# shiinamiyuki/akari_render

Hardware: AMD Instinct MI355X
Metric: Msamples/s (whole node), 1080p path tracer, C2 (higher is better)
Workload: dtype f32

## Files before the change

akari_render_amd/capi.py:

```python
from __future__ import annotations

import ctypes as C
import os
from typing import Optional

import numpy as np

from . import abi
from .build import LIB, build

AKR_OK = 0
FILM_PLANE_RGB, FILM_PLANE_SPLAT, FILM_PLANE_WEIGHT, FILM_PLANES_PT, FILM_PLANES_ALL = 1, 2, 4, 5, 7
ERR_INVALID_ARGUMENT, ERR_HIP, ERR_NO_DEVICE, ERR_IO, ERR_PARSE, ERR_UNSUPPORTED, ERR_OOM, ERR_RENDER = -1, -2, -3, -4, -5, -6, -7, -8

(ARRAY_WOOP, ARRAY_TRI_GID, ARRAY_SHADE, ARRAY_INSTANCES, ARRAY_MATERIALS, ARRAY_BVH_NODES, ARRAY_LIGHT_ENTRIES,
 ARRAY_LIGHT_PDF, ARRAY_AREA_ENTRIES, ARRAY_AREA_PDF, ARRAY_INST_TRI_OFFSET, ARRAY_R2C, ARRAY_C2W,
 ARRAY_TEX_NODES, ARRAY_TEX_IMAGES, ARRAY_TEX_TEXELS, ARRAY_MAT_INPUTS,
 ARRAY_INST_LEAVES, ARRAY_MESH_TRIS, ARRAY_MESH_POS, ARRAY_MESH_META, ARRAY_MESH_NORMALS,
 ARRAY_ENV_MARGINAL_ENTRIES, ARRAY_ENV_MARGINAL_PDF, ARRAY_ENV_CONDITIONAL_ENTRIES, ARRAY_ENV_CONDITIONAL_PDF, ARRAY_ENV_TEXELS,
 ARRAY_PUNCTUAL_LIGHTS, ARRAY_LIGHT_TREE) = range(29)
ENV_LIGHT_INSTANCE = 0xFFFFFFFF
PUNCTUAL_LIGHT_INSTANCE = 0xFFFFFFFE
LIGHT_TREE_INSTANCE = 0xFFFFFFFD

EXPORTS = [
    "akr_last_error", "akr_version", "akr_struct_size", "akr_option_set", "akr_option_get", "akr_context_create",
    "akr_context_destroy", "akr_context_synchronize", "akr_context_device_info", "akr_scene_create", "akr_scene_load",
    "akr_scene_destroy", "akr_scene_set_resolution", "akr_scene_get_info", "akr_scene_get_light", "akr_scene_get_ggx_table",
    "akr_scene_get_desc_counts", "akr_scene_get_mesh", "akr_scene_get_instance", "akr_scene_get_material", "akr_scene_get_camera",
    "akr_scene_get_array", "akr_scene_get_image_count", "akr_scene_get_image", "akr_scene_get_material_graph", "akr_film_create",
    "akr_film_wrap", "akr_film_destroy", "akr_film_clear", "akr_film_read", "akr_film_write", "akr_film_resolve",
    "akr_film_device_ptr", "akr_pt_config_default", "akr_pt_config_from_json", "akr_pt_render", "akr_pt_begin", "akr_pt_passes",
    "akr_pt_begin_features", "akr_pt_render_features",
    "akr_pt_end", "akr_pt_get_stats", "akr_render_task", "akr_image_write", "akr_aov_config_default", "akr_aov_render",
    "akr_gpt_config_default", "akr_gpt_render", "akr_gpt_begin", "akr_gpt_sample", "akr_gpt_sums", "akr_gpt_sums_read",
    "akr_gpt_sums_write", "akr_gpt_finish", "akr_gpt_abort", "akr_gpt_reduce", "akr_mcmc_config_default", "akr_mcmc_render",
    "akr_film_set_splat_scale", "akr_film_get_splat_scale", "akr_pt_read_sampler_states", "akr_context_device_ordinal",
    "akr_device_count", "akr_comm_unique_id", "akr_comm_create", "akr_comm_wrap", "akr_comm_destroy", "akr_film_reduce",
    "akr_pt_kernel_info", "akr_scene_spec_source", "akr_host_spec_compile", "akr_host_spec_compile_text",
    "akr_film_reduce_planes", "akr_mcmc_render_shard", "akr_mcmc_combine_host", "akr_mcmc_combine",
    "akr_scene_set_environment", "akr_scene_get_environment", "akr_scene_set_lens", "akr_scene_get_lens",
    "akr_denoise_config_default", "akr_denoise", "akr_denoise_variance",
    "akr_pt_set_active_tiles", "akr_film_tile_error", "akr_adaptive_config_default", "akr_pt_adaptive_render",
    "akr_display_config_default", "akr_film_luminance_histogram", "akr_display_exposure", "akr_display_transform",
    "akr_scene_add_punctual_light", "akr_scene_clear_punctual_lights", "akr_scene_punctual_light_count", "akr_scene_get_punctual_light",
    "akr_scene_set_light_tree", "akr_scene_get_light_tree",
]
TEST_EXPORTS = [
    "akr_probe_material_inputs_host", "akr_host_stdrng_u64", "akr_host_chacha_block", "akr_host_pcg32_states",
    "akr_host_pcg_start", "akr_host_alias_table", "akr_probe_math", "akr_probe_bsdf", "akr_probe_intersect",
    "akr_probe_surface_interaction", "akr_probe_material_inputs", "akr_host_decode_png", "akr_host_decode_jpeg",
    "akr_host_decode_exr", "akr_host_decode_tiff", "akr_host_decode_dds", "akr_host_pmj02bn_tables",
    "akr_probe_material_folded_host", "akr_host_sobol_dim1", "akr_host_fastmod", "akr_host_tri_pretest",
    "akr_probe_env_sample", "akr_probe_env_pdf", "akr_host_lens_ray", "akr_probe_camera_rays",
    "akr_probe_div", "akr_probe_intersect_pair", "akr_probe_math2", "akr_host_denoise", "akr_probe_denoise_times",
    "akr_host_pt_launch_plan", "akr_host_denoise_variance", "akr_probe_denoise_variance_times",
    "akr_host_tile_error", "akr_host_half_bracket", "akr_probe_adapt_times",
    "akr_host_display_transform", "akr_host_luminance_histogram", "akr_probe_display_times",
    "akr_host_pt_features_plan", "akr_host_pcg_end_pass", "akr_probe_pcg_end_pass",
    "akr_host_light_sample", "akr_probe_light_sample", "akr_host_light_sample_soft", "akr_probe_light_sample_soft",
    "akr_host_light_tree_sample", "akr_probe_light_tree_sample", "akr_host_option_info",
    "akr_probe_pt_cost_order", "akr_probe_pt_cost_order_mode",
]


class OptionInfo(C.Structure):
    _fields_ = [("name", C.c_char_p), ("env", C.c_char_p), ("default_value", C.c_int32), ("ranged", C.c_int32), ("lo", C.c_int32), ("hi", C.c_int32)]


class RenderSession(C.Structure):

    _fields_ = [("save_intermediate", C.c_int32), ("save_stats", C.c_int32), ("name", C.c_char_p),
                ("override_sampler_independent", C.c_int32), ("verbose", C.c_int32)]


class AkariError(RuntimeError):
    def __init__(self, code: int, msg: str):
        super().__init__(f"akari_hip error {code}: {msg}")
        self.code = code


_lib: Optional[C.CDLL] = None


def lib() -> C.CDLL:
    global _lib
    if _lib is not None:
        return _lib
    if not os.path.exists(LIB):
        build()
    L = C.CDLL(os.environ.get("AKR_HIP_LIB") or LIB)
    vp, u32, u64, i32, f32 = C.c_void_p, C.c_uint32, C.c_uint64, C.c_int32, C.c_float
    fp, up, u64p, vpp = C.POINTER(C.c_float), C.POINTER(C.c_uint32), C.POINTER(C.c_uint64), C.POINTER(C.c_void_p)
    L.akr_last_error.restype = C.c_char_p
    L.akr_version.restype = C.c_char_p
    L.akr_struct_size.restype = C.c_uint32
    L.akr_struct_size.argtypes = [C.c_int32]
    for sid, cls in enumerate((abi.MeshDesc, abi.InstanceDesc, abi.MaterialDesc, abi.CameraDesc, abi.SceneDesc, abi.PtConfig, abi.PtStats, abi.SceneInfo,
                               abi.KernelInfo, abi.AovConfig, abi.GptConfig, abi.McmcConfig, abi.McmcResult, abi.McmcPartial,
                               abi.EnvironmentDesc, abi.LensDesc, abi.DenoiseConfig), start=1):
        if L.akr_struct_size(sid) != C.sizeof(cls):
            raise ImportError("libakari_hip.so and akari_render_amd/abi.py disagree on sizeof(%s): %d vs %d" % (cls.__name__, L.akr_struct_size(sid), C.sizeof(cls)))
    for sid, cls in ((19, abi.AdaptiveConfig), (20, abi.AdaptiveStats), (22, abi.DisplayConfig), (24, abi.PunctualLightDesc)):
        if L.akr_struct_size(sid) != C.sizeof(cls):
            raise ImportError("libakari_hip.so and akari_render_amd/abi.py disagree on sizeof(%s): %d vs %d" % (cls.__name__, L.akr_struct_size(sid), C.sizeof(cls)))

    def proto(name, *args):
        if name in TEST_EXPORTS and not hasattr(L, name):
            return
        fn = getattr(L, name)
        fn.restype = i32
        fn.argtypes = list(args)

    proto("akr_context_create", i32, vpp)
    proto("akr_context_destroy", vp)
    proto("akr_context_synchronize", vp)
    proto("akr_context_device_info", vp, C.c_char_p, u32, up, u64p)
    proto("akr_scene_create", vp, C.POINTER(abi.SceneDesc), vpp)
    proto("akr_scene_load", vp, C.c_char_p, u32, u32, vpp)
    proto("akr_scene_destroy", vp)
    proto("akr_scene_set_resolution", vp, u32, u32)
    proto("akr_scene_get_info", vp, C.POINTER(abi.SceneInfo))
    proto("akr_scene_get_light", vp, u32, up, fp, fp)
    proto("akr_scene_set_environment", vp, C.POINTER(abi.EnvironmentDesc))
    proto("akr_scene_get_environment", vp, C.POINTER(abi.EnvironmentDesc))
    proto("akr_scene_set_lens", vp, C.POINTER(abi.LensDesc))
    proto("akr_scene_get_lens", vp, C.POINTER(abi.LensDesc))
    proto("akr_scene_add_punctual_light", vp, C.POINTER(abi.PunctualLightDesc))
    proto("akr_scene_clear_punctual_lights", vp)
    proto("akr_scene_punctual_light_count", vp, up)
    proto("akr_scene_get_punctual_light", vp, u32, C.POINTER(abi.PunctualLightDesc))
    proto("akr_host_light_sample", vp, u32, fp, fp, up)
    proto("akr_probe_light_sample", vp, vp, u32, fp, fp, up)
    proto("akr_host_light_sample_soft", vp, u32, fp, fp, up)
    proto("akr_probe_light_sample_soft", vp, vp, u32, fp, fp, up)
    proto("akr_scene_set_light_tree", vp, u32)
    proto("akr_scene_get_light_tree", vp, up, up)
    proto("akr_host_light_tree_sample", vp, u32, fp, fp, up, up)
    proto("akr_probe_light_tree_sample", vp, vp, u32, fp, fp, up, up)
    proto("akr_host_lens_ray", vp, u32, f32, u32, up, fp, fp)
    proto("akr_probe_camera_rays", vp, vp, u32, f32, u32, up, fp, fp)
    proto("akr_host_pt_launch_plan", vp, C.POINTER(abi.PtConfig), i32, i32, i32, i32, C.POINTER(abi.PtLaunchPlan))
    proto("akr_host_pt_features_plan", vp, C.POINTER(abi.PtConfig), i32, i32, i32, i32, i32, i32, i32, C.POINTER(abi.PtFeaturesPlan))
    proto("akr_probe_env_sample", vp, vp, u32, fp, fp)
    proto("akr_probe_env_pdf", vp, vp, u32, fp, fp)
    proto("akr_scene_get_ggx_table", vp, fp)
    proto("akr_scene_get_desc_counts", vp, up, up, up)
    proto("akr_scene_get_mesh", vp, u32, C.POINTER(abi.MeshDesc))
    proto("akr_scene_get_instance", vp, u32, C.POINTER(abi.InstanceDesc))
    proto("akr_scene_get_material", vp, u32, C.POINTER(abi.MaterialDesc))
    proto("akr_scene_get_camera", vp, C.POINTER(abi.CameraDesc))
    proto("akr_scene_get_array", vp, i32, vpp, u64p)
    proto("akr_scene_get_image_count", vp, up)
    proto("akr_scene_get_image", vp, u32, C.POINTER(abi.ImageDesc))
    proto("akr_scene_get_material_graph", vp, u32, C.POINTER(abi.MaterialGraph))
    proto("akr_film_create", vp, u32, u32, vpp)
    proto("akr_film_wrap", vp, u32, u32, vp, vpp)
    proto("akr_film_destroy", vp)
    proto("akr_film_clear", vp)
    proto("akr_film_read", vp, fp)
    proto("akr_film_write", vp, fp)
    proto("akr_film_resolve", vp, fp)
    proto("akr_film_device_ptr", vp, vpp, u64p)
    proto("akr_pt_kernel_info", vp, C.POINTER(abi.KernelInfo))
    proto("akr_scene_spec_source", vp, C.c_char_p, u64, u64p)
    proto("akr_host_spec_compile", vp, u32, u32, C.c_char_p, u64p, C.c_char_p, u32)
    proto("akr_probe_material_folded_host", vp, u32, u32, fp, up, fp, fp)
    proto("akr_host_sobol_dim1", u32, up, up, up)
    proto("akr_host_fastmod", u32, up, up, up)
    proto("akr_host_tri_pretest", u32, fp, fp, f32, up, up, fp)
    proto("akr_host_spec_compile_text", C.c_char_p, u32, u32, C.c_char_p, C.c_char_p)
    proto("akr_context_device_ordinal", vp, C.POINTER(C.c_int32))
    proto("akr_device_count", C.POINTER(C.c_int32))
    proto("akr_option_set", C.c_char_p, i32)
    proto("akr_option_get", C.c_char_p, C.POINTER(C.c_int32))
    proto("akr_host_option_info", u32, C.POINTER(OptionInfo))
    proto("akr_probe_pt_cost_order", vp, up, up, up, u32, up, fp)
    proto("akr_probe_pt_cost_order_mode", i32, C.POINTER(C.c_int32))
    proto("akr_comm_unique_id", C.POINTER(C.c_uint8))
    proto("akr_comm_create", vp, C.POINTER(C.c_uint8), i32, i32, vpp)
    proto("akr_comm_wrap", vp, vp, i32, i32, vpp)
    proto("akr_comm_destroy", vp)
    proto("akr_film_reduce", vp, vp, i32, i32)
    proto("akr_film_reduce_planes", vp, vp, i32, i32, u32)
    proto("akr_mcmc_render_shard", vp, vp, C.POINTER(abi.McmcConfig), u32, u32, vp, C.POINTER(abi.McmcPartial), up, C.POINTER(abi.PtStats))
    proto("akr_mcmc_combine_host", vp, C.POINTER(abi.McmcPartial), u32, C.POINTER(abi.McmcResult))
    proto("akr_mcmc_combine", vp, vp, i32, C.POINTER(abi.McmcPartial), C.POINTER(abi.McmcResult))
    proto("akr_pt_config_default", C.POINTER(abi.PtConfig))
    proto("akr_aov_config_default", C.POINTER(abi.AovConfig))
    proto("akr_aov_render", vp, vp, C.POINTER(abi.AovConfig), vp, C.POINTER(abi.PtStats))
    proto("akr_gpt_config_default", C.POINTER(abi.GptConfig))
    proto("akr_gpt_render", vp, vp, C.POINTER(abi.GptConfig), vp, fp, C.POINTER(abi.PtStats))
    proto("akr_gpt_begin", vp, vp, C.POINTER(abi.GptConfig), vp, vp, vpp)
    proto("akr_gpt_sample", vp, u32, i32)
    proto("akr_gpt_sums", vp, C.POINTER(fp), u64p)
    proto("akr_gpt_sums_read", vp, fp)
    proto("akr_gpt_sums_write", vp, fp)
    proto("akr_gpt_finish", vp, fp, C.POINTER(abi.PtStats))
    proto("akr_gpt_abort", vp, C.POINTER(abi.PtStats))
    proto("akr_gpt_reduce", vp, vp, i32, i32)
    proto("akr_mcmc_config_default", C.POINTER(abi.McmcConfig))
    proto("akr_mcmc_render", vp, vp, C.POINTER(abi.McmcConfig), vp, C.POINTER(abi.McmcResult), up, C.POINTER(abi.PtStats))
    proto("akr_film_set_splat_scale", vp, C.c_float)
    proto("akr_film_get_splat_scale", vp, fp)
    proto("akr_pt_config_from_json", C.c_char_p, C.POINTER(abi.PtConfig), C.c_char_p, u32)
    proto("akr_pt_render", vp, vp, C.POINTER(abi.PtConfig), vp, C.POINTER(abi.PtStats))
    proto("akr_pt_begin", vp, vp, C.POINTER(abi.PtConfig), vp, vpp)
    proto("akr_pt_passes", vp, u32, i32, up)
    proto("akr_pt_begin_features", vp, vp, C.POINTER(abi.PtConfig), vp, vp, vp, vpp)
    proto("akr_pt_render_features", vp, vp, C.POINTER(abi.PtConfig), vp, vp, vp, C.POINTER(abi.PtStats))
    proto("akr_pt_end", vp, C.POINTER(abi.PtStats))
    proto("akr_pt_get_stats", vp, C.POINTER(abi.PtStats))
    proto("akr_render_task", vp, vp, C.c_char_p, C.POINTER(RenderSession), C.POINTER(abi.PtStats))
    proto("akr_image_write", C.c_char_p, fp, u32, u32)
    proto("akr_pt_read_sampler_states", vp, u64p)
    proto("akr_host_stdrng_u64", u64, u32, u64p)
    proto("akr_host_chacha_block", up, u64, u64, i32, up)
    proto("akr_host_pcg32_states", u64, u64, u64p)
    proto("akr_host_pcg_start", u64p, u64)
    proto("akr_host_pcg_end_pass", u64p, u64, u32)
    proto("akr_probe_pcg_end_pass", vp, u32, u64p, u64p, up, u64p, u64p)
    proto("akr_host_alias_table", fp, u32, up, fp, fp)
    proto("akr_probe_math", vp, u32, fp, fp, fp, fp)
    proto("akr_probe_math2", vp, u32, fp, fp)
    proto("akr_probe_bsdf", vp, C.POINTER(abi.MaterialDesc), fp, i32, fp, u32, fp, fp)
    proto("akr_probe_intersect", vp, vp, u32, fp, up, fp)
    proto("akr_probe_div", vp, u32, fp, fp, fp, fp)
    proto("akr_probe_intersect_pair", vp, vp, u32, fp, up, up, fp)
    proto("akr_probe_surface_interaction", vp, vp, u32, up, fp, fp)
    proto("akr_probe_material_inputs", vp, vp, u32, u32, fp, fp)
    proto("akr_probe_material_inputs_host", vp, u32, u32, u32, fp, fp)
    proto("akr_host_decode_png", C.c_char_p, u64, up, up, C.POINTER(C.c_uint8), u64)
    proto("akr_host_decode_jpeg", C.c_char_p, u64, up, up, C.POINTER(C.c_uint8), u64)
    proto("akr_host_decode_exr", C.c_char_p, u64, up, up, fp, u64)
    proto("akr_host_decode_tiff", C.c_char_p, u64, up, up, C.POINTER(C.c_uint8), u64)
    proto("akr_host_decode_dds", C.c_char_p, u64, up, up, C.POINTER(C.c_uint8), u64)
    proto("akr_host_pmj02bn_tables", up, C.POINTER(C.c_uint16))
    proto("akr_denoise_config_default", C.POINTER(abi.DenoiseConfig))
    proto("akr_denoise", vp, C.POINTER(abi.DenoiseConfig), vp, vp, vp, vp)
    proto("akr_host_denoise", C.POINTER(abi.DenoiseConfig), u32, u32, fp, f32, fp, f32, fp, f32, fp)
    proto("akr_probe_denoise_times", vp, C.POINTER(abi.DenoiseConfig), vp, vp, vp, vp, i32, fp)
    proto("akr_denoise_variance", vp, C.POINTER(abi.DenoiseConfig), vp, vp, vp, vp, vp)
    proto("akr_host_denoise_variance", C.POINTER(abi.DenoiseConfig), u32, u32, fp, f32, fp, fp, f32, fp, f32, fp)
    proto("akr_probe_denoise_variance_times", vp, C.POINTER(abi.DenoiseConfig), vp, vp, vp, vp, vp, i32, fp)
    proto("akr_pt_set_active_tiles", vp, up, u32)
    proto("akr_film_tile_error", vp, vp, vp, u32, u32, up, u32, fp)
    proto("akr_adaptive_config_default", C.POINTER(abi.AdaptiveConfig))
    proto("akr_display_config_default", C.POINTER(abi.DisplayConfig))
    proto("akr_film_luminance_histogram", vp, vp, up, up)
    proto("akr_display_exposure", C.POINTER(abi.DisplayConfig), up, fp)
    proto("akr_display_transform", vp, C.POINTER(abi.DisplayConfig), vp, vp, fp)
    proto("akr_host_display_transform", C.POINTER(abi.DisplayConfig), u32, u32, fp, f32, fp, fp)
    proto("akr_host_luminance_histogram", u32, u32, fp, f32, up, up)
    proto("akr_probe_display_times", vp, C.POINTER(abi.DisplayConfig), vp, vp, i32, fp)
    proto("akr_pt_adaptive_render", vp, vp, C.POINTER(abi.PtConfig), C.POINTER(abi.AdaptiveConfig), vp, vp, up, C.POINTER(abi.AdaptiveStats))
    proto("akr_host_tile_error", u32, u32, fp, fp, u32, u32, up, u32, fp)
    proto("akr_host_half_bracket", u32, u32, fp, fp, u32, u32, up, u32, i32)
    proto("akr_probe_adapt_times", vp, vp, vp, u32, u32, up, u32, fp)
    _lib = L
    return L


def check(rc: int) -> None:
    if rc != AKR_OK:
        raise AkariError(rc, lib().akr_last_error().decode("utf-8", "replace"))


def _fp(a: np.ndarray):
    return a.ctypes.data_as(C.POINTER(C.c_float))


def _up(a: np.ndarray):
    return a.ctypes.data_as(C.POINTER(C.c_uint32))


class Context:

    def __init__(self, device: int = 0):
        self.h = C.c_void_p()
        check(lib().akr_context_create(device, C.byref(self.h)))

    def close(self):
        if self.h:
            lib().akr_context_destroy(self.h)
            self.h = C.c_void_p()

    def __del__(self):
        try:
            self.close()
        except Exception:
            pass

    def synchronize(self):
        check(lib().akr_context_synchronize(self.h))

    def device_info(self):
        name = C.create_string_buffer(256)
        cus, mem = C.c_uint32(), C.c_uint64()
        check(lib().akr_context_device_info(self.h, name, 256, C.byref(cus), C.byref(mem)))
        return {"name": name.value.decode(), "compute_units": cus.value, "hbm_bytes": mem.value}


class Scene:

    def __init__(self, ctx: Optional[Context], source, width: int = 0, height: int = 0):
        self.ctx = ctx
        self.h = C.c_void_p()
        ch = ctx.h if ctx is not None else C.c_void_p()
        if isinstance(source, (str, os.PathLike)):
            check(lib().akr_scene_load(ch, os.fspath(source).encode(), width, height, C.byref(self.h)))
        else:
            desc, keep = source.to_desc()
            if width and height:
                desc.camera.width, desc.camera.height = width, height
            check(lib().akr_scene_create(ch, C.byref(desc), C.byref(self.h)))
            del keep
            env = getattr(source, "environment", None)
            if env is not None:
                self._set_environment_data(env)
            lens = getattr(source, "lens", None)
            if lens is not None:
                self.set_lens(lens.radius, lens.focal_distance)
            for light in getattr(source, "lights", None) or ():
                self.add_punctual_light(light)

    def close(self):
        if self.h:
            lib().akr_scene_destroy(self.h)
            self.h = C.c_void_p()

    def __del__(self):
        try:
            self.close()
        except Exception:
            pass

    def info(self) -> abi.SceneInfo:
        i = abi.SceneInfo()
        check(lib().akr_scene_get_info(self.h, C.byref(i)))
        return i

    def spec_source(self) -> str:
        n = C.c_uint64()
        check(lib().akr_scene_spec_source(self.h, None, 0, C.byref(n)))
        buf = C.create_string_buffer(n.value + 1)
        check(lib().akr_scene_spec_source(self.h, buf, n.value + 1, C.byref(n)))
        return buf.value.decode()

    def spec_compile(self, bvh: bool = False, pmj: bool = False, stage: bool = True, defer: bool = False, min_waves: int = 3, arch: str = "gfx950", inst: bool = False,
                     env: bool = False, lens: bool = False) -> int:
        nbytes = C.c_uint64()
        log = C.create_string_buffer(4096)
        flags = (1 if bvh else 0) | (2 if pmj else 0) | (4 if stage else 0) | (8 if defer else 0) | (16 if inst else 0) | (32 if env else 0) | (64 if lens else 0)
        check(lib().akr_host_spec_compile(self.h, flags, min_waves, arch.encode(), C.byref(nbytes), log, 4096))
        return nbytes.value

    def launch_plan(self, cfg: abi.PtConfig, defer_metal: int = -1, simple_kernels: int = 1, defer_on: int = 0, spec_waves: int = 0) -> dict:
        out = abi.PtLaunchPlan()
        check(lib().akr_host_pt_launch_plan(self.h, C.byref(cfg), defer_metal, simple_kernels, defer_on, spec_waves, C.byref(out)))
        return out.as_dict()

    def features_plan(self, cfg: abi.PtConfig, feat: bool = True, defer_metal: int = -1, simple_kernels: int = 1, defer_on: int = 0, spec_waves: int = 0,
                      wavefront: int = -1, arith: int = 0) -> dict:
        out = abi.PtFeaturesPlan()
        check(lib().akr_host_pt_features_plan(self.h, C.byref(cfg), defer_metal, simple_kernels, defer_on, spec_waves, 1 if feat else 0, wavefront, arith, C.byref(out)))
        return out.as_dict()

    def material_folded_host(self, material: int, uv: np.ndarray):
        uv = np.ascontiguousarray(uv, dtype=np.float32).reshape(-1, 2)
        n = uv.shape[0]
        out, alpha, em = np.zeros((n, 64), np.uint32), np.zeros(n, np.float32), np.zeros((n, 3), np.float32)
        check(lib().akr_probe_material_folded_host(self.h, material, n, _fp(uv), out.ctypes.data_as(C.POINTER(C.c_uint32)), _fp(alpha), _fp(em)))
        return out, alpha, em

    def _set_environment_data(self, env: Optional[abi.EnvironmentData]):
        if env is None:
            check(lib().akr_scene_set_environment(self.h, None))
            return
        d, keep = env.to_desc()
        check(lib().akr_scene_set_environment(self.h, C.byref(d)))
        del keep

    def set_environment(self, image=None, color=None, strength: float = 1.0, rotation=None, filter: int = abi.TEX_FILTER_LINEAR):
        if image is None and color is None:
            self._set_environment_data(None)
        else:
            self._set_environment_data(abi.EnvironmentData(image=image, color=color, strength=strength, rotation=rotation, filter=filter))

    def environment(self) -> Optional[abi.EnvironmentData]:
        d = abi.EnvironmentDesc()
        check(lib().akr_scene_get_environment(self.h, C.byref(d)))
        if d.strength == 0.0:
            return None
        rot = np.array(list(d.rotation), dtype=np.float32).reshape(3, 3)
        if d.width:
            n = d.width * d.height * 4
            im = np.ctypeslib.as_array(d.texels, shape=(n,)).astype(np.float32, copy=True).reshape(d.height, d.width, 4)
            return abi.EnvironmentData(image=im, strength=float(d.strength), rotation=rot, filter=int(d.filter))
        return abi.EnvironmentData(color=tuple(float(c) for c in d.color), strength=float(d.strength), rotation=rot)

    def add_punctual_light(self, light: Optional[abi.PunctualLightData] = None, **fields):
        if light is None:
            light = abi.PunctualLightData(**fields)
        d = light.to_desc()
        check(lib().akr_scene_add_punctual_light(self.h, C.byref(d)))

    def clear_punctual_lights(self):
        check(lib().akr_scene_clear_punctual_lights(self.h))

    def punctual_lights(self) -> list:
        n = C.c_uint32()
        check(lib().akr_scene_punctual_light_count(self.h, C.byref(n)))
        out = []
        for i in range(n.value):
            d = abi.PunctualLightDesc()
            check(lib().akr_scene_get_punctual_light(self.h, i, C.byref(d)))
            out.append(abi.PunctualLightData.from_desc(d))
        return out

    def _light_sample(self, fn, head, rows, cols=7):
        rows = np.ascontiguousarray(rows, dtype=np.float32).reshape(-1, cols)
        n = rows.shape[0]
        out, light = np.zeros((n, 13), np.float32), np.zeros(n, np.uint32)
        check(fn(*head, n, _fp(rows), _fp(out), _up(light)))
        return out, light

    def host_light_sample(self, rows):
        return self._light_sample(lib().akr_host_light_sample, (self.h,), rows)

    def probe_light_sample(self, rows):
        return self._light_sample(lib().akr_probe_light_sample, (self.ctx.h, self.h), rows)

    def host_light_sample_soft(self, rows):
        return self._light_sample(lib().akr_host_light_sample_soft, (self.h,), rows, 9)

    def probe_light_sample_soft(self, rows):
        return self._light_sample(lib().akr_probe_light_sample_soft, (self.ctx.h, self.h), rows, 9)

    def set_light_tree(self, on):
        check(lib().akr_scene_set_light_tree(self.h, 1 if on else 0))

    def light_tree(self):
        on, n = C.c_uint32(), C.c_uint32()
        check(lib().akr_scene_get_light_tree(self.h, C.byref(on), C.byref(n)))
        return on.value, n.value

    def _light_tree_sample(self, fn, head, rows):
        rows = np.ascontiguousarray(rows, dtype=np.float32).reshape(-1, 9)
        n = rows.shape[0]
        out, light, record = np.zeros((n, 13), np.float32), np.zeros(n, np.uint32), np.zeros(n, np.uint32)
        check(fn(*head, n, _fp(rows), _fp(out), _up(light), _up(record)))
        return out, light, record

    def host_light_tree_sample(self, rows):
        return self._light_tree_sample(lib().akr_host_light_tree_sample, (self.h,), rows)

    def probe_light_tree_sample(self, rows):
        return self._light_tree_sample(lib().akr_probe_light_tree_sample, (self.ctx.h, self.h), rows)

    def set_lens(self, radius: Optional[float] = None, focal_distance: float = 0.0):
        if radius is None:
            check(lib().akr_scene_set_lens(self.h, None))
            return
        d = abi.LensDesc(float(radius), float(focal_distance))
        check(lib().akr_scene_set_lens(self.h, C.byref(d)))

    def lens(self) -> Optional[abi.LensData]:
        d = abi.LensDesc()
        check(lib().akr_scene_get_lens(self.h, C.byref(d)))
        return abi.LensData(float(d.radius), float(d.focal_distance)) if d.radius > 0.0 else None

    def _camera_rays(self, fn, head, pixels, u_filter, u_lens, filter_type, filter_radius):
        px = np.ascontiguousarray(pixels, dtype=np.uint32).reshape(-1, 2)
        n = px.shape[0]
        u = np.ascontiguousarray(np.concatenate([np.asarray(u_filter, np.float32).reshape(n, 2), np.asarray(u_lens, np.float32).reshape(n, 2)], axis=1))
        out = np.zeros((n, 6), np.float32)
        check(fn(*head, int(filter_type), float(filter_radius), n, px.ctypes.data_as(C.POINTER(C.c_uint32)), _fp(u), _fp(out)))
        return out

    def host_lens_ray(self, pixels, u_filter, u_lens, filter_type: int = 0, filter_radius: float = 0.5) -> np.ndarray:
        return self._camera_rays(lib().akr_host_lens_ray, (self.h,), pixels, u_filter, u_lens, filter_type, filter_radius)

    def probe_camera_rays(self, pixels, u_filter, u_lens, filter_type: int = 0, filter_radius: float = 0.5) -> np.ndarray:
        return self._camera_rays(lib().akr_probe_camera_rays, (self.ctx.h, self.h), pixels, u_filter, u_lens, filter_type, filter_radius)

    def probe_env_sample(self, u: np.ndarray) -> np.ndarray:
        u = np.ascontiguousarray(u, dtype=np.float32).reshape(-1, 2)
        out = np.zeros((u.shape[0], 5), np.float32)
        check(lib().akr_probe_env_sample(self.ctx.h, self.h, u.shape[0], _fp(u), _fp(out)))
        return out

    def probe_env_pdf(self, d: np.ndarray) -> np.ndarray:
        d = np.ascontiguousarray(d, dtype=np.float32).reshape(-1, 3)
        out = np.zeros((d.shape[0], 4), np.float32)
        check(lib().akr_probe_env_pdf(self.ctx.h, self.h, d.shape[0], _fp(d), _fp(out)))
        return out

    def set_resolution(self, w: int, h: int):
        check(lib().akr_scene_set_resolution(self.h, w, h))

    def light(self, i: int):
        inst, power, pdf = C.c_uint32(), C.c_float(), C.c_float()
        check(lib().akr_scene_get_light(self.h, i, C.byref(inst), C.byref(power), C.byref(pdf)))
        return inst.value, power.value, pdf.value

    def ggx_table(self) -> np.ndarray:
        t = np.zeros(4096, dtype=np.float32)
        check(lib().akr_scene_get_ggx_table(self.h, _fp(t)))
# ... 284 lines not shown
        except Exception:
            pass


def pt_render(ctx: Context, scene: Scene, cfg: abi.PtConfig, film: Film) -> dict:
    st = abi.PtStats()
    c = cfg.copy()
    check(lib().akr_pt_render(ctx.h, scene.h, C.byref(c), film.h, C.byref(st)))
    return st.as_dict()


def pt_render_features(ctx: Context, scene: Scene, cfg: abi.PtConfig, film: Film, albedo: Film, normal: Film) -> dict:
    st = abi.PtStats()
    c = cfg.copy()
    check(lib().akr_pt_render_features(ctx.h if ctx is not None else None, scene.h, C.byref(c), film.h if film is not None else None,
                                       albedo.h if albedo is not None else None, normal.h if normal is not None else None, C.byref(st)))
    return st.as_dict()


def render_task(ctx: Context, scene: Scene, method_json: str, name: Optional[str] = None, save_intermediate: bool = False,
                save_stats: bool = False, override_sampler_independent: bool = False, verbose: bool = False) -> dict:
    ses = RenderSession(1 if save_intermediate else 0, 1 if save_stats else 0, name.encode() if name else None,
                        1 if override_sampler_independent else 0, 1 if verbose else 0)
    st = abi.PtStats()
    check(lib().akr_render_task(ctx.h, scene.h, method_json.encode(), C.byref(ses), C.byref(st)))
    return st.as_dict()


def image_write(path: str, rgb: np.ndarray) -> None:
    rgb = np.ascontiguousarray(rgb, dtype=np.float32)
    h, w = rgb.shape[0], rgb.shape[1]
    check(lib().akr_image_write(os.fspath(path).encode(), _fp(rgb), w, h))


def config_from_json(text: str):
    cfg = abi.PtConfig()
    out = C.create_string_buffer(1024)
    check(lib().akr_pt_config_from_json(text.encode(), C.byref(cfg), out, 1024))
    return cfg, out.value.decode()


def host_stdrng_u64(seed: int, n: int) -> np.ndarray:
    out = np.zeros(n, dtype=np.uint64)
    check(lib().akr_host_stdrng_u64(seed, n, out.ctypes.data_as(C.POINTER(C.c_uint64))))
    return out


def host_chacha_block(key, counter: int, stream: int, rounds: int) -> np.ndarray:
    key = np.ascontiguousarray(key, dtype=np.uint32)
    out = np.zeros(16, dtype=np.uint32)
    check(lib().akr_host_chacha_block(_up(key), counter, stream, rounds, _up(out)))
    return out


def host_pcg32_states(seed: int, n: int) -> np.ndarray:
    out = np.zeros(2 * n, dtype=np.uint64)
    check(lib().akr_host_pcg32_states(seed, n, out.ctypes.data_as(C.POINTER(C.c_uint64))))
    return out


def host_pcg_start(state: int, inc: int) -> int:
    s = C.c_uint64(state)
    check(lib().akr_host_pcg_start(C.byref(s), inc))
    return s.value


def host_pcg_end_pass(state: int, inc: int, dim: int) -> int:
    s = C.c_uint64(state)
    check(lib().akr_host_pcg_end_pass(C.byref(s), inc, dim))
    return s.value


def host_tri_pretest(rays8: np.ndarray, tris9: np.ndarray, plane_shift: float = 0.0):
    rays8 = np.ascontiguousarray(rays8, dtype=np.float32).reshape(-1, 8)
    tris9 = np.ascontiguousarray(tris9, dtype=np.float32).reshape(-1, 9)
    n = rays8.shape[0]
    may, exact, t = np.zeros(n, dtype=np.uint32), np.zeros(n, dtype=np.uint32), np.zeros(n, dtype=np.float32)
    check(lib().akr_host_tri_pretest(n, _fp(rays8), _fp(tris9), C.c_float(plane_shift), _up(may), _up(exact), _fp(t)))
    return may.astype(bool), exact.astype(bool), t


def host_alias_table(weights):
    w = np.ascontiguousarray(weights, dtype=np.float32)
    j = np.zeros(w.size, dtype=np.uint32)
    t = np.zeros(w.size, dtype=np.float32)
    pdf = np.zeros(w.size, dtype=np.float32)
    check(lib().akr_host_alias_table(_fp(w), w.size, _up(j), _fp(t), _fp(pdf)))
    return j, t, pdf


def probe_math(ctx: Context, x: np.ndarray):
    x = np.ascontiguousarray(x, dtype=np.float32)
    s, c, l = (np.zeros_like(x) for _ in range(3))
    check(lib().akr_probe_math(ctx.h, x.size, _fp(x), _fp(s), _fp(c), _fp(l)))
    return s, c, l


def probe_math2(ctx: Context, x: np.ndarray, y: np.ndarray) -> np.ndarray:
    xy = np.ascontiguousarray(np.stack([np.asarray(x, dtype=np.float32), np.asarray(y, dtype=np.float32)], axis=1))
    out = np.zeros((xy.shape[0], 6), dtype=np.float32)
    check(lib().akr_probe_math2(ctx.h, xy.shape[0], _fp(xy), _fp(out)))
    return out


def probe_div(ctx: Context, a: np.ndarray, b: np.ndarray):
    a = np.ascontiguousarray(a, dtype=np.float32)
    b = np.ascontiguousarray(b, dtype=np.float32)
    assert a.shape == b.shape
    fast, ieee = np.zeros_like(a), np.zeros_like(a)
    check(lib().akr_probe_div(ctx.h, a.size, _fp(a), _fp(b), _fp(fast), _fp(ieee)))
    return fast, ieee


def probe_pcg_end_pass(ctx: Context, state: np.ndarray, inc: np.ndarray, dim: np.ndarray):
    state = np.ascontiguousarray(state, dtype=np.uint64)
    inc = np.ascontiguousarray(inc, dtype=np.uint64)
    dim = np.ascontiguousarray(dim, dtype=np.uint32)
    assert state.shape == inc.shape == dim.shape
    closed, loop = np.zeros_like(state), np.zeros_like(state)
    u64p = C.POINTER(C.c_uint64)
    check(lib().akr_probe_pcg_end_pass(ctx.h, state.size, state.ctypes.data_as(u64p), inc.ctypes.data_as(u64p), _up(dim),
                                       closed.ctypes.data_as(u64p), loop.ctypes.data_as(u64p)))
    return closed, loop


def probe_bsdf(ctx: Context, m: abi.MaterialData, mode: int, wo, data: np.ndarray, table: Optional[np.ndarray] = None) -> np.ndarray:
    ms = m.to_struct()
    wo = np.ascontiguousarray(wo, dtype=np.float32)
    data = np.ascontiguousarray(data, dtype=np.float32).reshape(-1, 3)
    out = np.zeros((data.shape[0], 4 if mode == 0 else 8), dtype=np.float32)
    tp = _fp(np.ascontiguousarray(table, dtype=np.float32)) if table is not None else C.POINTER(C.c_float)()
    check(lib().akr_probe_bsdf(ctx.h, C.byref(ms), tp, mode, _fp(wo), data.shape[0], _fp(data), _fp(out)))
    return out


def probe_intersect(ctx: Context, scene: Scene, rays: np.ndarray):
    rays = np.ascontiguousarray(rays, dtype=np.float32).reshape(-1, 8)
    out = np.zeros((rays.shape[0], 3), dtype=np.uint32)
    bary = np.zeros((rays.shape[0], 2), dtype=np.float32)
    check(lib().akr_probe_intersect(ctx.h, scene.h, rays.shape[0], _fp(rays), _up(out), _fp(bary)))
    return out, bary


def probe_intersect_pair(ctx: Context, scene: Scene, rays: np.ndarray, excl: np.ndarray):
    rays = np.ascontiguousarray(rays, dtype=np.float32).reshape(-1, 16)
    excl = np.ascontiguousarray(excl, dtype=np.uint32).reshape(-1, 3)
    assert rays.shape[0] == excl.shape[0]
    out = np.zeros((rays.shape[0], 4), dtype=np.uint32)
    tuv = np.zeros((rays.shape[0], 3), dtype=np.float32)
    check(lib().akr_probe_intersect_pair(ctx.h, scene.h, rays.shape[0], _fp(rays), _up(excl), _up(out), _fp(tuv)))
    return out, tuv


def probe_surface_interaction(ctx: Context, scene: Scene, inst_prim: np.ndarray, bary: np.ndarray) -> np.ndarray:
    ip = np.ascontiguousarray(inst_prim, dtype=np.uint32).reshape(-1, 2)
    b = np.ascontiguousarray(bary, dtype=np.float32).reshape(-1, 2)
    out = np.zeros((ip.shape[0], 19), dtype=np.float32)
    check(lib().akr_probe_surface_interaction(ctx.h, scene.h, ip.shape[0], _up(ip), _fp(b), _fp(out)))
    return out


def probe_material_inputs(ctx: Optional[Context], scene: Scene, material: int, uv: np.ndarray) -> np.ndarray:
    u = np.ascontiguousarray(uv, dtype=np.float32).reshape(-1, 2)
    out = np.zeros((u.shape[0], 26), dtype=np.float32)
    check(lib().akr_probe_material_inputs(ctx.h if ctx is not None else C.c_void_p(), scene.h, material, u.shape[0], _fp(u), _fp(out)))
    return out


def probe_material_inputs_host(scene: Scene, material: int, uv: np.ndarray, color: int = 0) -> np.ndarray:
    u = np.ascontiguousarray(uv, dtype=np.float32).reshape(-1, 2)
    out = np.zeros((u.shape[0], 26), dtype=np.float32)
    check(lib().akr_probe_material_inputs_host(scene.h, material, color, u.shape[0], _fp(u), _fp(out)))
    return out


def _host_decode(fn, data: bytes) -> np.ndarray:
    w, h = C.c_uint32(), C.c_uint32()
    check(fn(data, len(data), C.byref(w), C.byref(h), None, 0))
    out = np.zeros((h.value, w.value, 4), dtype=np.uint8)
    check(fn(data, len(data), C.byref(w), C.byref(h), out.ctypes.data_as(C.POINTER(C.c_uint8)), out.size))
    return out


def host_decode_png(data: bytes) -> np.ndarray:
    return _host_decode(lib().akr_host_decode_png, data)


def host_decode_jpeg(data: bytes) -> np.ndarray:
    return _host_decode(lib().akr_host_decode_jpeg, data)


def host_decode_tiff(data: bytes) -> np.ndarray:
    return _host_decode(lib().akr_host_decode_tiff, data)


def host_decode_dds(data: bytes) -> np.ndarray:
    return _host_decode(lib().akr_host_decode_dds, data)


def aov_render(ctx: Context, scene: Scene, cfg: abi.AovConfig, film: Film) -> dict:
    st = abi.PtStats()
    check(lib().akr_aov_render(ctx.h, scene.h, C.byref(cfg), film.h, C.byref(st)))
    return st.as_dict()


def denoise(ctx: Context, color: Film, albedo: Optional[Film], normal: Optional[Film], out: Film, cfg: Optional[abi.DenoiseConfig] = None) -> None:
    c = cfg if cfg is not None else abi.DenoiseConfig.default()
    check(lib().akr_denoise(ctx.h, C.byref(c), color.h, albedo.h if albedo is not None else None, normal.h if normal is not None else None, out.h))


def denoise_times(ctx: Context, color: Film, albedo: Optional[Film], normal: Optional[Film], out: Film, kernel: int, cfg: Optional[abi.DenoiseConfig] = None) -> dict:
    c = cfg if cfg is not None else abi.DenoiseConfig.default()
    t = np.zeros(11, dtype=np.float32)
    check(lib().akr_probe_denoise_times(ctx.h, C.byref(c), color.h, albedo.h if albedo is not None else None, normal.h if normal is not None else None, out.h, kernel, _fp(t)))
    return {"prepare": float(t[0]), "levels": [float(v) for v in t[1:1 + c.iterations]], "finish": float(t[9]), "total": float(t[10])}


def host_denoise(width: int, height: int, color: np.ndarray, albedo: Optional[np.ndarray] = None, normal: Optional[np.ndarray] = None,
                 cfg: Optional[abi.DenoiseConfig] = None, splat_scales=(1.0, 1.0, 1.0)) -> np.ndarray:
    c = cfg if cfg is not None else abi.DenoiseConfig.default()
    films = []
    for f in (color, albedo, normal):
        if f is not None:
            f = np.ascontiguousarray(f, dtype=np.float32).reshape(-1)
            assert f.size == 7 * width * height
        films.append(f)
    out = np.zeros(3 * width * height, dtype=np.float32)
    ptr = [_fp(f) if f is not None else None for f in films]
    check(lib().akr_host_denoise(C.byref(c), width, height, ptr[0], splat_scales[0], ptr[1], splat_scales[1], ptr[2], splat_scales[2], _fp(out)))
    return out.reshape(height, width, 3)


def denoise_variance(ctx: Context, color: Film, half: Film, albedo: Optional[Film], normal: Optional[Film], out: Film, cfg: Optional[abi.DenoiseConfig] = None) -> None:
    c = cfg if cfg is not None else abi.DenoiseConfig.default()
    check(lib().akr_denoise_variance(ctx.h, C.byref(c), color.h, half.h if half is not None else None, albedo.h if albedo is not None else None,
                                     normal.h if normal is not None else None, out.h))


def denoise_variance_times(ctx: Context, color: Film, half: Film, albedo: Optional[Film], normal: Optional[Film], out: Film, kernel: int,
                           cfg: Optional[abi.DenoiseConfig] = None) -> dict:
    c = cfg if cfg is not None else abi.DenoiseConfig.default()
    t = np.zeros(11, dtype=np.float32)
    check(lib().akr_probe_denoise_variance_times(ctx.h, C.byref(c), color.h, half.h, albedo.h if albedo is not None else None,
                                                 normal.h if normal is not None else None, out.h, kernel, _fp(t)))
    return {"prepare": float(t[0]), "levels": [float(v) for v in t[1:1 + c.iterations]], "finish": float(t[9]), "total": float(t[10])}


def host_denoise_variance(width: int, height: int, color: np.ndarray, half: np.ndarray, albedo: Optional[np.ndarray] = None, normal: Optional[np.ndarray] = None,
                          cfg: Optional[abi.DenoiseConfig] = None, splat_scales=(1.0, 1.0, 1.0)) -> np.ndarray:
    c = cfg if cfg is not None else abi.DenoiseConfig.default()
    films = []
    for f in (color, half, albedo, normal):
        if f is not None:
            f = np.ascontiguousarray(f, dtype=np.float32).reshape(-1)
            assert f.size == 7 * width * height
        films.append(f)
    out = np.zeros(3 * width * height, dtype=np.float32)
    ptr = [_fp(f) if f is not None else None for f in films]
    check(lib().akr_host_denoise_variance(C.byref(c), width, height, ptr[0], splat_scales[0], ptr[1], ptr[2], splat_scales[1], ptr[3], splat_scales[2], _fp(out)))
    return out.reshape(height, width, 3)


def film_tile_error(ctx: Context, film: Film, half: Film, tile_w: int, tile_h: int, tiles) -> np.ndarray:
    t = np.ascontiguousarray(tiles, dtype=np.uint32).reshape(-1)
    err = np.zeros(t.size, dtype=np.float32)
    check(lib().akr_film_tile_error(ctx.h, film.h, half.h if half is not None else None, tile_w, tile_h, _up(t), t.size, _fp(err)))
    return err


def host_tile_error(width: int, height: int, film: np.ndarray, half: np.ndarray, tile_w: int, tile_h: int, tiles) -> np.ndarray:
    film, half = np.ascontiguousarray(film, dtype=np.float32), np.ascontiguousarray(half, dtype=np.float32)
    assert film.size == half.size == 7 * width * height
    t = np.ascontiguousarray(tiles, dtype=np.uint32).reshape(-1)
    err = np.zeros(t.size, dtype=np.float32)
    check(lib().akr_host_tile_error(width, height, _fp(film), _fp(half), tile_w, tile_h, _up(t), t.size, _fp(err)))
    return err


def host_half_bracket(width: int, height: int, film: np.ndarray, half: np.ndarray, tile_w: int, tile_h: int, tiles, close: bool) -> np.ndarray:
    film = np.ascontiguousarray(film, dtype=np.float32)
    out = np.array(half, dtype=np.float32, copy=True)
    assert film.size == out.size == 7 * width * height
    t = np.ascontiguousarray(tiles, dtype=np.uint32).reshape(-1)
    check(lib().akr_host_half_bracket(width, height, _fp(film), _fp(out), tile_w, tile_h, _up(t), t.size, 1 if close else 0))
    return out


def adapt_times(ctx: Context, film: Film, half: Film, tile_w: int, tile_h: int, tiles) -> dict:
    t = np.ascontiguousarray(tiles, dtype=np.uint32).reshape(-1)
    ms = np.zeros(3, dtype=np.float32)
    check(lib().akr_probe_adapt_times(ctx.h, film.h, half.h, tile_w, tile_h, _up(t), t.size, _fp(ms)))
    return {"tile_error": float(ms[0]), "half_open": float(ms[1]), "half_close": float(ms[2])}


def pt_adaptive_render(ctx: Context, scene: Scene, cfg: abi.PtConfig, film: Film, acfg: Optional[abi.AdaptiveConfig] = None, half: Optional[Film] = None,
                       want_tile_spp: bool = True):
    c, a = cfg.copy(), (acfg if acfg is not None else abi.AdaptiveConfig.default())
    tw, th = c.tile_w or 32, c.tile_h or 32
    tiles_x, tiles_y = (film.width + tw - 1) // tw, (film.height + th - 1) // th
    tile_spp = np.zeros(tiles_x * tiles_y, dtype=np.uint32) if want_tile_spp else None
    st = abi.AdaptiveStats()
    check(lib().akr_pt_adaptive_render(ctx.h, scene.h, C.byref(c), C.byref(a), film.h, half.h if half is not None else None,
                                       _up(tile_spp) if tile_spp is not None else None, C.byref(st)))
    return st.as_dict(), (tile_spp.reshape(tiles_y, tiles_x) if tile_spp is not None else None)


# ... 148 lines not shown
```

akari_render_amd/csrc/device/disect.h:

```cpp
#pragma once
#include "drng.h"
#include "dscene.h"
#include "../kernels.h"

namespace akr {

template <bool V>
struct BoolTag {
    static constexpr bool value = V;
};

struct Hit {
    float t, u, v;
    uint32_t gid;
};

struct PlaneHit {
    float t, px, py, pz;
};
AKR_HD PlaneHit tri_plane(vec3 o, vec3 d, float4 r2) {
    float dz = __builtin_fmaf(r2.x, d.x, __builtin_fmaf(r2.y, d.y, r2.z * d.z));
    float oz = __builtin_fmaf(r2.x, o.x, __builtin_fmaf(r2.y, o.y, __builtin_fmaf(r2.z, o.z, r2.w)));
    PlaneHit h;
    h.t = div_f(-oz, dz);
    h.px = __builtin_fmaf(h.t, d.x, o.x);
    h.py = __builtin_fmaf(h.t, d.y, o.y);
    h.pz = __builtin_fmaf(h.t, d.z, o.z);
    return h;
}
AKR_HD void tri_uv(const PlaneHit& h, float4 r0, float4 r1, float& u, float& v) {
    u = __builtin_fmaf(r0.x, h.px, __builtin_fmaf(r0.y, h.py, __builtin_fmaf(r0.z, h.pz, r0.w)));
    v = __builtin_fmaf(r1.x, h.px, __builtin_fmaf(r1.y, h.py, __builtin_fmaf(r1.z, h.pz, r1.w)));
}
AKR_HD bool tri_test(vec3 o, vec3 d, float4 r0, float4 r1, float4 r2, float tmin, float tmax, float& t_out, float& u_out,
                     float& v_out) {
    PlaneHit h = tri_plane(o, d, r2);
    float u, v;
    tri_uv(h, r0, r1, u, v);
    t_out = h.t;
    u_out = u;
    v_out = v;
    return (h.t >= tmin) & (h.t <= tmax) & (u >= 0.0f) & (v >= 0.0f) & (u + v <= 1.0f);
}

AKR_D float textured_alpha(const DScene& sc, const float4* r, uint32_t material, float u, float v) {
    float w = 1.0f - u - v;
    vec2 uv = mk2((r[0].w * w + r[2].w * u) + r[4].w * v, (r[1].w * w + r[3].w * u) + r[5].w * v);
    return material_alpha_at(sc.tex, sc.materials[material], material, uv);
}
template <bool TEX>
AKR_D bool alpha_test(const DScene& sc, uint32_t gid, float u, float v) {
    const float4* r = sc.shade + (size_t)gid * SHADE_ROWS;
    float4 q6 = r[6];
    const DMaterial& m = sc.materials[f2u(q6.y)];
    float alpha = (m.kind == MAT_PRINCIPLED || m.kind == MAT_DIFFUSE) ? m.base_alpha : 1.0f;
    if (TEX) {
        if (m.flags & MF_ALPHA_TEXTURED)
            alpha = textured_alpha(sc, r, f2u(q6.y), u, v);
    }
    if (alpha >= 1.0f) return true;
    uint32_t inst = f2u(q6.z);
    uint32_t prim = gid - sc.inst_tri_offset[inst];
    float h = (float)xxhash32_4(inst, prim, f2u(u), f2u(v)) * 2.3283064365386963e-10f;
    return alpha > h;
}

AKR_D float next_up(float x) {
    uint32_t b = f2u(x);
    return x > 0.0f ? u2f(b + 1u) : (x < 0.0f ? u2f(b - 1u) : u2f(1u));
}
AKR_D float hit_margin(float t, float u, float v, float tmax) {
    return __builtin_fminf(__builtin_fminf(__builtin_fminf(u, v), 1.0f - (u + v)), __builtin_fminf(t, tmax - t));
}

template <bool ANY_HIT, bool TEX = false>
AKR_D bool trace_exhaustive(const DScene& sc, vec3 o, vec3 d, float tmin, float tmax, uint32_t ex0, uint32_t ex1, Hit& hit) {
    float best_t = next_up(tmax);
    uint32_t best = kInvalid;
    float best_u = 0.0f, best_v = 0.0f;
    const uint32_t n = sc.n_tris;
    typedef const float __attribute__((address_space(4))) * ConstF;
    ConstF recs = (ConstF)(uintptr_t)sc.woop;
    auto load_rec = [&](uint32_t k, float4& a, float4& b, float4& c) {
        ConstF r = recs + 12 * (size_t)k;
        a = make_float4(r[0], r[1], r[2], r[3]);
        b = make_float4(r[4], r[5], r[6], r[7]);
        c = make_float4(r[8], r[9], r[10], r[11]);
    };
    float4 n0, n1, n2;
    load_rec(0, n0, n1, n2);
    PlaneHit ph{0.0f, 0.0f, 0.0f, 0.0f};
    for (uint32_t k = 0; k < n; k++) {
        const float4 r0 = n0, r1 = n1, r2 = n2;
        load_rec(k + 1, n0, n1, n2);
        if (!((sc.plane_share_mask >> k) & 1ull)) ph = tri_plane(o, d, r2);
        float u, v;
        const float t = ph.t;
        tri_uv(ph, r0, r1, u, v);
        float m = __builtin_fminf(hit_margin(t, u, v, tmax), t - tmin);
        m = (k == ex0) ? -1.0f : m;
        m = (k == ex1) ? -1.0f : m;
        if (sc.has_alpha) {
            if (m >= 0.0f && !alpha_test<TEX>(sc, k, u, v)) m = -1.0f;
        }
        if (ANY_HIT) {
            if (m >= 0.0f) best = k;
            if (__builtin_amdgcn_ballot_w64(best == kInvalid) == 0) break;
        } else {
            const float tc = (m >= 0.0f) ? t : __builtin_inff();
            const bool better = tc < best_t;
            best_t = better ? tc : best_t;
            best_u = better ? u : best_u;
            best_v = better ? v : best_v;
            best = better ? k : best;
        }
    }
    hit.t = best != kInvalid ? best_t : tmax;
    hit.u = best_u;
    hit.v = best_v;
    hit.gid = best;
    return best != kInvalid;
}

typedef float v2f __attribute__((ext_vector_type(2)));
typedef float v4f __attribute__((ext_vector_type(4)));
AKR_D float min_raw(float a, float b) {
    float r;
    asm("v_min_f32 %0, %1, %2" : "=v"(r) : "v"(a), "v"(b));
    return r;
}
AKR_D float max_raw(float a, float b) {
    float r;
    asm("v_max_f32 %0, %1, %2" : "=v"(r) : "v"(a), "v"(b));
    return r;
}
AKR_D float min_abs_raw(float a, float b) {
    float r;
    asm("v_min_f32 %0, %1, |%2|" : "=v"(r) : "v"(a), "v"(b));
    return r;
}
AKR_D float max3_abs_raw(float a, float b, float c) {
    float r;
    asm("v_max3_f32 %0, |%1|, |%2|, |%3|" : "=v"(r) : "v"(a), "v"(b), "v"(c));
    return r;
}
AKR_D PlaneHit tri_plane_unscaled(vec3 o, vec3 d, float4 r2, float& lo) {
    float dz = __builtin_fmaf(r2.x, d.x, __builtin_fmaf(r2.y, d.y, r2.z * d.z));
    float oz = __builtin_fmaf(r2.x, o.x, __builtin_fmaf(r2.y, o.y, __builtin_fmaf(r2.z, o.z, r2.w)));
    lo = min_abs_raw(lo, oz);
    PlaneHit h;
    h.t = div_f_unscaled(-oz, dz);
    h.px = __builtin_fmaf(h.t, d.x, o.x);
    h.py = __builtin_fmaf(h.t, d.y, o.y);
    h.pz = __builtin_fmaf(h.t, d.z, o.z);
    return h;
}

template <bool DIV>
struct WalkOpt {
    static constexpr bool unscaled_div = DIV;
};
template <int V>
struct IntTag {
    static constexpr int value = V;
};

template <bool TEX = false, class OPT = WalkOpt<true>>
AKR_D void trace_pair_exhaustive(const DScene& sc, vec3 o, vec3 d, float tmax, uint32_t ex0, vec3 so, vec3 sd, float stmax,
                                 uint32_t sex0, uint32_t sex1, Hit& hit, bool& found, bool& occluded, const float4* lds_recs, uint32_t* took_ieee_walk = nullptr) {
    constexpr bool UNSCALED = OPT::unscaled_div && !AKR_RX;
    float best_t = next_up(tmax);
    uint32_t best = kInvalid;
    float best_u = 0.0f, best_v = 0.0f;
    float occ_margin = -1.0f;
    const uint32_t n = sc.n_tris;
    const v4f* lrec = (const v4f*)lds_recs;
    const bool has_alpha = __builtin_amdgcn_readfirstlane((int)sc.has_alpha) != 0;
    v2f T2 = {0.0f, 0.0f}, hx2 = {0.0f, 0.0f}, hy2 = {0.0f, 0.0f}, hz2 = {0.0f, 0.0f};
    float lo = __builtin_inff(), slo = __builtin_inff();
    auto record = [&](auto alpha_tag, auto div_tag, uint32_t k, const v4f& q0, const v4f& q1, const v4f& q2) {
        constexpr int ALPHA = decltype(alpha_tag)::value;
        constexpr bool FAST = decltype(div_tag)::value;
        if (!((sc.plane_share_mask >> k) & 1ull)) {
            const float4 r2 = make_float4(q2.x, q2.y, q2.z, q2.w);
            const PlaneHit a = FAST ? tri_plane_unscaled(o, d, r2, lo) : tri_plane(o, d, r2), b = FAST ? tri_plane_unscaled(so, sd, r2, slo) : tri_plane(so, sd, r2);
            T2 = (v2f){a.t, b.t};
            hx2 = (v2f){a.px, b.px}; hy2 = (v2f){a.py, b.py}; hz2 = (v2f){a.pz, b.pz};
        }
        float u, v, su, sv;
        tri_uv(PlaneHit{T2.x, hx2.x, hy2.x, hz2.x}, make_float4(q0.x, q0.y, q0.z, q0.w), make_float4(q1.x, q1.y, q1.z, q1.w), u, v);
        tri_uv(PlaneHit{T2.y, hx2.y, hy2.y, hz2.y}, make_float4(q0.x, q0.y, q0.z, q0.w), make_float4(q1.x, q1.y, q1.z, q1.w), su, sv);
        const v2f u2 = {u, su}, v2 = {v, sv};
        const v2f s2 = {1.0f - (u2.x + v2.x), 1.0f - (u2.y + v2.y)};
        const v2f w2 = {tmax - T2.x, stmax - T2.y};
        float m = min_raw(min_raw(min_raw(u2.x, v2.x), s2.x), min_raw(T2.x, w2.x));
        float sm = min_raw(min_raw(min_raw(u2.y, v2.y), s2.y), min_raw(T2.y, w2.y));
        m = (k == ex0) ? -1.0f : m;
        sm = (k == sex0) ? -1.0f : sm;
        sm = (k == sex1) ? -1.0f : sm;
        if (ALPHA == 1 || (ALPHA == 2 && has_alpha)) {
            const uint32_t ka = __builtin_amdgcn_readfirstlane(k);
            if (m >= 0.0f && !alpha_test<TEX>(sc, ka, u2.x, v2.x)) m = -1.0f;
            if (sm >= 0.0f && !alpha_test<TEX>(sc, ka, u2.y, v2.y)) sm = -1.0f;
        }
        const float tc = (m >= 0.0f) ? T2.x : __builtin_inff();
        const bool better = tc < best_t;
        best_t = better ? tc : best_t;
        best = better ? k : best;
        occ_margin = max_raw(occ_margin, sm);
    };
    auto walk = [&](auto alpha_tag) {
        const BoolTag<UNSCALED> div_tag{};
        v4f a0 = lrec[0], a1 = lrec[1], a2 = lrec[2], b0, b1, b2;
        uint32_t k = 0;
        for (; k + 1 < n; k += 2) {
            b0 = lrec[3 * (k + 1)]; b1 = lrec[3 * (k + 1) + 1]; b2 = lrec[3 * (k + 1) + 2];
            record(alpha_tag, div_tag, k, a0, a1, a2);
            a0 = lrec[3 * (k + 2)]; a1 = lrec[3 * (k + 2) + 1]; a2 = lrec[3 * (k + 2) + 2];
            record(alpha_tag, div_tag, k + 1, b0, b1, b2);
        }
        if (k < n) record(alpha_tag, div_tag, k, a0, a1, a2);
    };
    auto walk_ieee = [&] {
        best_t = next_up(tmax); best = kInvalid; occ_margin = -1.0f;
#pragma clang loop unroll(disable)
        for (uint32_t k = 0; k < n; k++) {
            record(IntTag<2>{}, BoolTag<false>{}, k, lrec[3 * k], lrec[3 * k + 1], lrec[3 * k + 2]);
        }
    };
    if (UNSCALED) {
        const float ob = lds_recs[3u * (n + 1u) + 2u].w;
        const bool pre_bad = ((tmax >= 0.0f) & !((max3_abs_raw(o.x, o.y, o.z) <= ob) & (max3_abs_raw(d.x, d.y, d.z) <= 2.0f) & (tmax <= 1e20f))) |
                             ((stmax >= 0.0f) & !((max3_abs_raw(so.x, so.y, so.z) <= ob) & (max3_abs_raw(sd.x, sd.y, sd.z) <= 2.0f) & (stmax <= 1e20f)));
        bool redo = __builtin_amdgcn_ballot_w64(pre_bad) != 0;
        if (!redo) {
            if (has_alpha) walk(IntTag<1>{});
            else walk(IntTag<0>{});
            const bool bad = ((tmax >= 0.0f) & (lo < 0x1p-47f)) | ((stmax >= 0.0f) & (slo < 0x1p-47f));
            redo = __builtin_amdgcn_ballot_w64(bad) != 0;
        }
        if (redo) walk_ieee();
        if (took_ieee_walk) *took_ieee_walk = redo ? 1u : 0u;
    } else {
        if (has_alpha) walk(IntTag<1>{});
        else walk(IntTag<0>{});
        if (took_ieee_walk) *took_ieee_walk = 0u;
    }
    if (best != kInvalid) {
        const v4f q0 = lrec[3 * best], q1 = lrec[3 * best + 1];
        const float px = __builtin_fmaf(best_t, d.x, o.x), py = __builtin_fmaf(best_t, d.y, o.y), pz = __builtin_fmaf(best_t, d.z, o.z);
        best_u = __builtin_fmaf(q0.x, px, __builtin_fmaf(q0.y, py, __builtin_fmaf(q0.z, pz, q0.w)));
        best_v = __builtin_fmaf(q1.x, px, __builtin_fmaf(q1.y, py, __builtin_fmaf(q1.z, pz, q1.w)));
    }
    found = best != kInvalid;
    hit.t = found ? best_t : tmax;
    hit.u = best_u;
    hit.v = best_v;
    hit.gid = best;
    occluded = occ_margin >= 0.0f;
}

constexpr uint32_t kBvhDone = 0xfffffffeu;

struct TraceCounters {
    uint32_t nodes, tris, overflow;
};

AKR_D float safe_inv(float d) {
    float a = abs_f(d) < 1e-20f ? __builtin_copysignf(1e-20f, d) : d;
    return __builtin_amdgcn_rcpf(a);
}
AKR_D uint32_t byte_of(uint32_t w, int i) { return (w >> (8 * i)) & 0xffu; }

struct Trav {
    vec3 o, d, inv, noi;
    float tmin, tmax, best_t, best_u, best_v;
    uint32_t ex0, ex1, best;
    uint32_t G, T, tbase, sp, octinv4;
    bool active;
};
AKR_D void trav_begin(Trav& s, vec3 o, vec3 d, float tmin, float tmax, uint32_t ex0, uint32_t ex1) {
    s.o = o; s.d = d;
    s.inv = mk3(safe_inv(d.x), safe_inv(d.y), safe_inv(d.z));
    s.noi = mk3(-o.x * s.inv.x, -o.y * s.inv.y, -o.z * s.inv.z);
    s.tmin = tmin; s.tmax = tmax;
    s.best_t = tmax; s.best_u = 0.0f; s.best_v = 0.0f; s.best = kInvalid;
    s.ex0 = ex0; s.ex1 = ex1;
    const uint32_t oi = (s.inv.x >= 0.0f ? 1u : 0u) | (s.inv.y >= 0.0f ? 2u : 0u) | (s.inv.z >= 0.0f ? 4u : 0u);
    s.octinv4 = oi * 0x01010101u;
    s.G = 1u << (24u + oi);
    s.T = 0; s.tbase = 0; s.sp = 0;
    s.active = tmax >= tmin;
}

AKR_D uint32_t node_pop(Trav& s, uint32_t* __restrict__ stack, uint32_t depth, TraceCounters& cnt) {
    const uint32_t j = 31u - (uint32_t)__builtin_clz(s.G);
    s.G &= ~(1u << j);
    if ((s.G >> 24) != 0) {
        if (s.sp < depth) {
            stack[s.sp * 256u] = s.G;
            s.sp++;
        } else {
            cnt.overflow = 1;
        }
    }
    const uint32_t slot = (j - 24u) ^ (s.octinv4 & 7u);
    return (s.G & 0xffffffu) + slot;
}
AKR_D void hit_commit(Trav& s, bool any_hit, uint32_t gid, float t, float u, float v) {
    if (any_hit) {
        s.best = gid;
        s.T = 0; s.G = 0; s.sp = 0;
    } else {
        const bool better = (s.best == kInvalid) | (t < s.best_t) | ((t == s.best_t) & (gid < s.best));
        if (better) { s.best_t = t; s.best_u = u; s.best_v = v; s.best = gid; }
    }
}
template <bool TEX>
AKR_D void hit_accept(const DScene& sc, Trav& s, bool any_hit, uint32_t gid, float t, float u, float v) {
    bool h = (gid != s.ex0) & (gid != s.ex1);
    if (h && sc.has_alpha) h = alpha_test<TEX>(sc, gid, u, v);
    if (h) hit_commit(s, any_hit, gid, t, u, v);
}

template <int MODE, bool TEX, bool TILE = false>
AKR_D void trav_step_staged(const DScene& sc, Trav& s, uint32_t* __restrict__ stack, TraceCounters& cnt, bool any_rt = false, const uint4* tile = nullptr) {
    const bool any_hit = MODE == 2 ? any_rt : (MODE == 1);
    if (s.T == 0) {
        if ((s.G >> 24) == 0) {
            s.sp--;
            s.G = stack[s.sp * 256u];
        }
        const uint32_t idx = node_pop(s, stack, sc.bvh_stack_depth, cnt);
        const uint4* p = sc.bvh_nodes + (size_t)idx * (kBvhNodeWords / 4);
        uint4 w0, w1, w2, w3;
        if (TILE && idx < sc.bvh_tile_nodes) {
            typedef const volatile uint32_t __attribute__((address_space(3))) * LdsW;
            typedef uint32_t u32x4 __attribute__((ext_vector_type(4)));
            typedef const volatile u32x4 __attribute__((address_space(3))) * LdsU4;
            LdsU4 pt = (LdsU4)((LdsW)(const uint32_t*)tile + idx * kBvhNodeWords);
            const u32x4 t0 = pt[0], t1 = pt[1], t2 = pt[2], t3 = pt[3];
            w0 = make_uint4(t0.x, t0.y, t0.z, t0.w); w1 = make_uint4(t1.x, t1.y, t1.z, t1.w); w2 = make_uint4(t2.x, t2.y, t2.z, t2.w);
            w3 = make_uint4(t3.x, t3.y, t3.z, t3.w);
        } else {
            w0 = p[0]; w1 = p[1]; w2 = p[2]; w3 = p[3];
        }
        cnt.nodes++;
        const float limit = s.best_t;
        const float bx = u2f((w0.w & 0xffu) << 23) * s.inv.x, by = u2f(((w0.w >> 8) & 0xffu) << 23) * s.inv.y, bz = u2f(((w0.w >> 16) & 0xffu) << 23) * s.inv.z;
        const float ax = __builtin_fmaf(u2f(w0.x), s.inv.x, s.noi.x), ay = __builtin_fmaf(u2f(w0.y), s.inv.y, s.noi.y), az = __builtin_fmaf(u2f(w0.z), s.inv.z, s.noi.z);
        const bool nx = s.inv.x < 0.0f, ny = s.inv.y < 0.0f, nz = s.inv.z < 0.0f;
        const uint32_t xb = nx ? ((w3.y >> 16) | (w3.y << 16)) : w3.y, yb = ny ? ((w3.z >> 16) | (w3.z << 16)) : w3.z, zb = nz ? ((w3.w >> 16) | (w3.w << 16)) : w3.w;
        const uint32_t qnx[2] = {nx ? w2.z : w1.w, xb}, qfx[2] = {nx ? w1.w : w2.z, xb >> 16};
        const uint32_t qny[2] = {ny ? w2.w : w2.x, yb}, qfy[2] = {ny ? w2.x : w2.w, yb >> 16};
        const uint32_t qnz[2] = {nz ? w3.x : w2.y, zb}, qfz[2] = {nz ? w2.y : w3.x, zb >> 16};
        uint32_t hitmask = 0;
#pragma unroll
        for (int h = 0; h < 2; h++) {
            const uint32_t meta4 = h ? (w1.x >> 16) : w1.y;
            const uint32_t is_inner4 = (meta4 & (meta4 << 1)) & 0x10101010u;
            const uint32_t inner_mask4 = (is_inner4 >> 4) * 0xffu;
            const uint32_t bit_index4 = (meta4 ^ (s.octinv4 & inner_mask4)) & 0x1f1f1f1fu;
            const uint32_t child_bits4 = (meta4 >> 5) & 0x07070707u;
#pragma unroll
            for (int i = 0; i < (h ? 2 : 4); i++) {
                const float tnx = __builtin_fmaf((float)byte_of(qnx[h], i), bx, ax), tfx = __builtin_fmaf((float)byte_of(qfx[h], i), bx, ax);
                const float tny = __builtin_fmaf((float)byte_of(qny[h], i), by, ay), tfy = __builtin_fmaf((float)byte_of(qfy[h], i), by, ay);
                const float tnz = __builtin_fmaf((float)byte_of(qnz[h], i), bz, az), tfz = __builtin_fmaf((float)byte_of(qfz[h], i), bz, az);
                const float tn = __builtin_fmaxf(__builtin_fmaxf(tnx, tny), __builtin_fmaxf(tnz, s.tmin));
                const float tf = __builtin_fminf(__builtin_fminf(tfx, tfy), __builtin_fminf(tfz, limit));
                if (tn <= tf) hitmask |= byte_of(child_bits4, i) << byte_of(bit_index4, i);
            }
        }
        s.G = ((w0.w >> 24) | ((w1.x & 0xffffu) << 8)) | (hitmask & 0xff000000u);
        s.T = hitmask & 0x00ffffffu;
        s.tbase = w1.z;
    }
    if (s.T != 0) {
        const uint32_t b = (uint32_t)__builtin_ctz(s.T);
        s.T &= s.T - 1u;
        const uint4* p = (const uint4*)sc.woop + (size_t)(s.tbase + b) * (kBvhTriWords / 4);
        const uint4 w0 = p[0], w1 = p[1], w2 = p[2], w3 = p[3];
        cnt.tris++;
        float t, u, v;
        bool h = tri_test(s.o, s.d, make_float4(u2f(w0.x), u2f(w0.y), u2f(w0.z), u2f(w0.w)), make_float4(u2f(w1.x), u2f(w1.y), u2f(w1.z), u2f(w1.w)),
                          make_float4(u2f(w2.x), u2f(w2.y), u2f(w2.z), u2f(w2.w)), s.tmin, s.tmax, t, u, v);
        if (h) hit_accept<TEX>(sc, s, any_hit, w3.x, t, u, v);
    }
    s.active = (s.T != 0) | ((s.G >> 24) != 0) | (s.sp != 0);
}
template <int MODE, bool TEX, bool TILE = false>
AKR_D void trav_step(const DScene& sc, Trav& s, uint32_t* __restrict__ stack, TraceCounters& cnt, bool any_rt = false, const uint4* tile = nullptr) {
    if constexpr (TEX) {
        trav_step_staged<MODE, TEX, TILE>(sc, s, stack, cnt, any_rt, tile);
        return;
    }
    const bool any_hit = MODE == 2 ? any_rt : (MODE == 1);
    const bool do_tri = s.T != 0;
    const uint4* p;
    bool in_tile = false;
    uint32_t tile_idx = 0;
    if (do_tri) {
        const uint32_t b = (uint32_t)__builtin_ctz(s.T);
        s.T &= s.T - 1u;
        p = (const uint4*)sc.woop + (size_t)(s.tbase + b) * (kBvhTriWords / 4);
    } else {
        if ((s.G >> 24) == 0) {
            s.sp--;
            s.G = stack[s.sp * 256u];
        }
        const uint32_t idx = node_pop(s, stack, sc.bvh_stack_depth, cnt);
        p = sc.bvh_nodes + (size_t)idx * (kBvhNodeWords / 4);
// ... 93 lines not shown
```

akari_render_amd/csrc/device/dscene.h:

```cpp
#pragma once
#include "dtex.h"

namespace akr {

constexpr uint32_t kInvalid = 0xffffffffu;

constexpr uint32_t kBvhNodeWords = 16;
constexpr uint32_t kBvhTriWords = 16;
constexpr uint32_t kBvhStackDepth = 24;
AKR_HD uint32_t walk_bound_word(uint32_t n_tris) { return 12u * (n_tris + 1u) + 11u; }

enum : uint32_t { SHADE_ROWS = 8, INST_ROWS = 8 };
enum : uint32_t { TRI_HAS_NORMALS = 1u, TRI_HAS_TANGENTS = 2u };

struct LightRec {
    uint32_t tri_offset, n_tris, first_gid, inst;
};

constexpr uint32_t kMeshPrimMask = 0x7fffffffu, kMeshTriShares = 0x80000000u;
struct DInst {
    const uint4* __restrict__ tlas_leaves;
    const float4* __restrict__ mesh_tris;
    const uint32_t* __restrict__ mesh_pos;
    const uint32_t* __restrict__ mesh_meta;
    const float4* __restrict__ mesh_normals;
    const uint32_t* __restrict__ inst_mats;
    const uint32_t* __restrict__ share_bits;
    uint32_t on, n_instances;
};

struct DEnv {
    const float4* __restrict__ texels;
    const AliasPacked* __restrict__ marginal;
    const AliasPacked* __restrict__ conditional;
    float rot[9];
    uint32_t w, h, filter, light;
};

enum : uint32_t { PUNCT_POINT = 0, PUNCT_SPOT = 1, PUNCT_SUN = 2 };
constexpr uint32_t kPunctInst = 0xfffffffeu;
constexpr uint32_t kPunctTreeInst = 0xfffffffdu;
struct DPunct {
    vec3 q;       uint32_t kind;
    vec3 a;       float cos_o;
    vec3 c;       float cos_i;
    float inv_span;
    float radius;
    float cos_max;
    float k;
};
static_assert(sizeof(DPunct) == 64, "DPunct layout");
constexpr uint32_t kPunctSoftBit = 0x80000000u;

struct DScene {
    const float4* __restrict__ woop;
    const uint32_t* __restrict__ tri_gid;
    const float4* __restrict__ shade;
    const float4* __restrict__ normals;
    const float4* __restrict__ inst;
    const DMaterial* __restrict__ materials;
    const float* __restrict__ ggx_table;
    const AliasEntry* __restrict__ light_entries;
    const float* __restrict__ light_pdf;
    const uint32_t* __restrict__ light_inst;
    const uint32_t* __restrict__ light_tri_offset;
    const DEnv* __restrict__ env;
    const AliasEntry* __restrict__ area_entries;
    const float* __restrict__ area_pdf;
    const uint32_t* __restrict__ inst_tri_offset;
    const AliasPacked* __restrict__ light_alias;
    const AliasPacked* __restrict__ area_alias;
    const LightRec* __restrict__ lights;
    const uint4* __restrict__ bvh_nodes;
    uint32_t n_tris, n_lights, n_nodes, has_alpha;
    uint32_t bvh_stack_depth;
    uint32_t bvh_tile_nodes;
    uint64_t plane_share_mask;
    TexScene tex;
    DInst in2;
    const DPunct* __restrict__ punct;
    uint32_t n_punct, punct_tree;
};

struct SurfacePoint {
    Frame frame;
    vec3 p, ng;
    float prim_area;
    uint32_t material;
    int32_t light;
    uint32_t inst;
    vec2 uv;
};

AKR_HD vec3 xyz(float4 v) { return mk3(v.x, v.y, v.z); }
AKR_HD vec3 interp3(vec2 b, vec3 a0, vec3 a1, vec3 a2) {
    float w = 1.0f - b.x - b.y;
    return (a0 * w + a1 * b.x) + a2 * b.y;
}
AKR_HD vec3 xf_point(vec3 c0, vec3 c1, vec3 c2, vec3 t, vec3 p) { return ((c0 * p.x + c1 * p.y) + c2 * p.z) + t; }
AKR_HD vec3 xf_vector(vec3 c0, vec3 c1, vec3 c2, vec3 v) { return (c0 * v.x + c1 * v.y) + c2 * v.z; }

AKR_D SurfacePoint surface_interaction_rows(const float4* m, float4 q0, float4 q1, float4 q2, float4 q3, float4 q4, float4 q5, float4 q6, float4 q7, bool has_normals,
                                            const float4* nr, vec2 bary) {
    SurfacePoint s;
    s.prim_area = q6.x;
    s.material = f2u(q6.y);
    s.inst = f2u(q6.z);
    s.light = (int32_t)f2u(q6.w);
    float4 c0 = m[0], c1 = m[1], c2 = m[2], t = m[3];
    vec3 p_local = interp3(bary, xyz(q0), xyz(q1), xyz(q2));
    s.p = xf_point(xyz(c0), xyz(c1), xyz(c2), xyz(t), p_local);
    s.ng = xyz(q3);
    s.frame = Frame{s.ng, xyz(q4), xyz(q5)};
    {
        float w = 1.0f - bary.x - bary.y;
        s.uv = mk2((q0.w * w + q2.w * bary.x) + q4.w * bary.y, (q1.w * w + q3.w * bary.x) + q5.w * bary.y);
    }
    if (has_normals) {
        const uint32_t tf = f2u(q7.w);
        if (tf & (TRI_HAS_NORMALS | TRI_HAS_TANGENTS)) {
            vec3 ns = s.ng;
            if (tf & TRI_HAS_NORMALS) {
                vec3 ns_local = interp3(bary, xyz(nr[0]), xyz(nr[1]), xyz(nr[2]));
                float4 k0 = m[4], k1 = m[5], k2 = m[6];
                vec3 rr = (xyz(k0) * ns_local.x + xyz(k1) * ns_local.y) + xyz(k2) * ns_local.z;
                ns = normalize(rr * k0.w);
            }
            vec3 tt = xyz(q7);
            if (tf & TRI_HAS_TANGENTS) {
                vec3 tt_local = normalize(interp3(bary, xyz(nr[3]), xyz(nr[4]), xyz(nr[5])));
                tt = xf_vector(xyz(c0), xyz(c1), xyz(c2), tt_local);
            }
            s.frame = (tt.x != 0.0f || tt.y != 0.0f || tt.z != 0.0f) ? frame_from_n_t(ns, tt) : frame_from_n(ns);
        }
    }
    return s;
}
AKR_D SurfacePoint surface_interaction(const DScene& sc, uint32_t gid, vec2 bary) {
    const float4* r = sc.shade + (size_t)gid * SHADE_ROWS;
    float4 q0 = r[0], q1 = r[1], q2 = r[2], q3 = r[3], q4 = r[4], q5 = r[5], q6 = r[6];
    const float4* m = sc.inst + (size_t)f2u(q6.z) * INST_ROWS;
    const bool has_normals = sc.normals != nullptr;
    float4 q7 = make_float4(0, 0, 0, 0);
    if (has_normals) q7 = r[7];
    return surface_interaction_rows(m, q0, q1, q2, q3, q4, q5, q6, q7, has_normals, has_normals ? sc.normals + (size_t)gid * 6 : nullptr, bary);
}

}
```

akari_render_amd/csrc/device/pt_pass.h:

```cpp
#pragma once
#include "dpath.h"

namespace akr {

#ifndef AKR_PT_MIN_WAVES
#define AKR_PT_MIN_WAVES 4
#endif
#ifndef AKR_PT_MIN_WAVES_BVH
#define AKR_PT_MIN_WAVES_BVH 4
#endif
#ifndef AKR_PT_MIN_WAVES_FD
#define AKR_PT_MIN_WAVES_FD 4
#endif
#ifndef AKR_PT_MIN_WAVES_TEX
#define AKR_PT_MIN_WAVES_TEX 3
#endif
#ifndef AKR_PT_MIN_WAVES_BVH_TEX
#define AKR_PT_MIN_WAVES_BVH_TEX 3
#endif
template <bool TEX>
using PairWalkOpt = WalkOpt<!TEX>;
template <bool BVH, bool FD, bool TEX, bool PMJ, bool STAGE, bool DEFER, uint32_t ABSENT = 0, bool INST = false, bool ENV = false, bool LENS = false, bool FEAT = false, bool PUNCT = false, bool LTREE = false>
AKR_D void pt_pass_body(const PtParams& p) {
    extern __shared__ __attribute__((aligned(16))) uint32_t lds_stack[];
    TraceCtx tc;
    tc.stack = lds_stack + threadIdx.x;
    tc.cnt = TraceCounters{0, 0, 0};
    PtParams staged = p;
    if (STAGE) stage_scene_tables<BVH, TEX, !BVH && !FD && TEX>(p, lds_stack, staged);
    const PtParams& q = STAGE ? staged : p;
    const DScene& sc = q.sc;
    constexpr bool TILE = BVH && !TEX && !INST;
    constexpr uint32_t STRAG = BVH ? (INST ? AKR_PT_STRAGGLERS_INST : (TEX ? AKR_PT_STRAGGLERS_TEX : AKR_PT_STRAGGLERS)) : 0;
    const uint4* tile = (const uint4*)(lds_stack + p.tile_offset);
    if (TILE) {
        uint32_t* l = lds_stack + p.tile_offset;
        const uint32_t* g = (const uint32_t*)p.sc.bvh_nodes;
        for (uint32_t i = threadIdx.x; i < p.sc.bvh_tile_nodes * kBvhNodeWords; i += 256u) l[i] = g[i];
        __syncthreads();
    }
    const float4* lds_recs = nullptr;
    if (!BVH) {
        uint32_t* l = lds_stack + (p.stage_total >> 2);
        const uint32_t* g = (const uint32_t*)p.sc.woop;
        for (uint32_t i = threadIdx.x; i < (p.sc.n_tris + 2u) * 12u; i += 256u) l[i] = g[i];
        __syncthreads();
        lds_recs = (const float4*)l;
    }
    const uint32_t item = blockIdx.x * 256u + threadIdx.x;
    uint32_t px = 0, py = 0;
    bool in_frame;
    if (p.item_pixels != nullptr) {
        const uint32_t t = p.item_pixels[item];
        in_frame = t != kInvalid;
        if (in_frame) { py = t / p.width; px = t - py * p.width; }
    } else {
        in_frame = item < p.n_items && item_to_pixel(p, item, px, py);
    }
    const uint32_t pix = px + py * p.width;
    uint32_t sx, sy;
    shifted_pixel(p, px, py, sx, sy);
    if (PMJ && p.bn_offset != 0) pmj_bluenoise_stage(p, px, py);
    PathRegs r;
    path_regs_init<PMJ, LENS, FEAT>(r, q, in_frame, pix, sx, sy);
    constexpr bool PARK = !FD && TEX;
    uint32_t* park = lds_stack + p.park_offset + threadIdx.x;
    if (PARK) {
        park_put(park, PK_PIX, pix);
        park_put(park, PK_SX, sx);
        park_put(park, PK_SY, sy);
        if (FEAT) {
            park_put(park, PK_FEAT_A + 0, f2u(r.feat_a.x)); park_put(park, PK_FEAT_A + 1, f2u(r.feat_a.y)); park_put(park, PK_FEAT_A + 2, f2u(r.feat_a.z));
            park_put(park, PK_FEAT_N + 0, f2u(r.feat_n.x)); park_put(park, PK_FEAT_N + 1, f2u(r.feat_n.y)); park_put(park, PK_FEAT_N + 2, f2u(r.feat_n.z));
        }
    }

    uint32_t iteration = 0;
    while (__builtin_amdgcn_ballot_w64(r.active) != 0) {
        iteration++;
        if (r.active) {
            Hit hit;
            bool found = false, occluded = false;
            if (!(STRAG > 0 && r.carry)) {
                r.c_closest += r.has_ray ? 1u : 0u;
                r.c_shadow += r.has_shadow ? 1u : 0u;
            }
            if (BVH && INST) {
                trace_pair_inst<TEX, STRAG>(sc, r.has_ray, r.ro, r.rd, r.ray_ex0, r.has_shadow, r.s_o, r.s_d, r.s_tmax, r.s_ex0, r.s_ex1, r.carry, hit, found, occluded, tc.stack,
                                            lds_stack + p.carry_offset + threadIdx.x, tc.cnt);
            } else if (BVH && STRAG > 0) {
                uint32_t* cy = lds_stack + p.carry_offset + threadIdx.x;
                Trav s;
                uint32_t phase;
                hit.t = 1e20f; hit.u = 0.0f; hit.v = 0.0f; hit.gid = kInvalid;
                if (!r.carry) {
                    phase = r.has_ray ? 0u : (r.has_shadow ? 1u : 2u);
                    if (phase == 0) trav_begin(s, r.ro, r.rd, 0.0f, 1e20f, r.ray_ex0, kInvalid);
                    else trav_begin(s, r.s_o, r.s_d, 0.0f, phase == 1 ? r.s_tmax : -1.0f, r.s_ex0, r.s_ex1);
                } else {
                    phase = cy[CY_PHASE * 256];
                    if (phase == 0) trav_begin(s, r.ro, r.rd, 0.0f, 1e20f, r.ray_ex0, kInvalid);
                    else {
                        trav_begin(s, r.s_o, r.s_d, 0.0f, r.s_tmax, r.s_ex0, r.s_ex1);
                        hit.t = u2f(cy[CY_HIT_T * 256]); hit.u = u2f(cy[CY_HIT_U * 256]); hit.v = u2f(cy[CY_HIT_V * 256]); hit.gid = cy[CY_HIT_GID * 256];
                        found = hit.gid != kInvalid;
                    }
                    s.best_t = u2f(cy[CY_BEST_T * 256]); s.best_u = u2f(cy[CY_BEST_U * 256]); s.best_v = u2f(cy[CY_BEST_V * 256]); s.best = cy[CY_BEST * 256];
                    s.G = cy[CY_G * 256]; s.T = cy[CY_T * 256]; s.tbase = cy[CY_TBASE * 256]; s.sp = cy[CY_SP * 256];
                    s.active = true;
                }
                const uint32_t n_in = (uint32_t)__builtin_popcountll(__builtin_amdgcn_ballot_w64(phase != 2u));
                const uint32_t n_leave = n_in / (STRAG > 0 ? STRAG : 1u);
                while (true) {
                    const uint32_t n_now = (uint32_t)__builtin_popcountll(__builtin_amdgcn_ballot_w64(phase != 2u));
                    if (n_now <= n_leave) break;
                    if (phase != 2u) {
                        if (s.active) trav_step<2, TEX, TILE>(sc, s, tc.stack, tc.cnt, phase == 1u, tile);
                        if (!s.active) {
                            if (phase == 0u) {
                                found = s.best != kInvalid;
                                hit.t = s.best_t; hit.u = s.best_u; hit.v = s.best_v; hit.gid = s.best;
                                phase = r.has_shadow ? 1u : 2u;
                                if (r.has_shadow) trav_begin(s, r.s_o, r.s_d, 0.0f, r.s_tmax, r.s_ex0, r.s_ex1);
                            } else {
                                occluded = s.best != kInvalid;
                                phase = 2u;
                            }
                        }
                    }
                }
                r.carry = phase != 2u;
                if (r.carry) {
                    cy[CY_BEST_T * 256] = f2u(s.best_t); cy[CY_BEST_U * 256] = f2u(s.best_u); cy[CY_BEST_V * 256] = f2u(s.best_v); cy[CY_BEST * 256] = s.best;
                    cy[CY_G * 256] = s.G; cy[CY_T * 256] = s.T; cy[CY_TBASE * 256] = s.tbase; cy[CY_SP * 256] = s.sp;
                    cy[CY_PHASE * 256] = phase;
                    if (phase == 1u) { cy[CY_HIT_T * 256] = f2u(hit.t); cy[CY_HIT_U * 256] = f2u(hit.u); cy[CY_HIT_V * 256] = f2u(hit.v); cy[CY_HIT_GID * 256] = hit.gid; }
                }
            } else if (BVH) {
                Trav s;
                uint32_t phase = r.has_ray ? 0u : (r.has_shadow ? 1u : 2u);
                if (phase == 0) trav_begin(s, r.ro, r.rd, 0.0f, 1e20f, r.ray_ex0, kInvalid);
                else trav_begin(s, r.s_o, r.s_d, 0.0f, phase == 1 ? r.s_tmax : -1.0f, r.s_ex0, r.s_ex1);
                hit.t = 1e20f; hit.u = 0.0f; hit.v = 0.0f; hit.gid = kInvalid;
                while (phase != 2u) {
                    if (s.active) trav_step<2, TEX, TILE>(sc, s, tc.stack, tc.cnt, phase == 1u, tile);
                    if (!s.active) {
                        if (phase == 0u) {
                            found = s.best != kInvalid;
                            hit.t = s.best_t; hit.u = s.best_u; hit.v = s.best_v; hit.gid = s.best;
                            phase = r.has_shadow ? 1u : 2u;
                            if (r.has_shadow) trav_begin(s, r.s_o, r.s_d, 0.0f, r.s_tmax, r.s_ex0, r.s_ex1);
                        } else {
                            occluded = s.best != kInvalid;
                            phase = 2u;
                        }
                    }
                }
            } else {
                trace_pair_exhaustive<TEX, PairWalkOpt<TEX>>(sc, r.ro, r.rd, r.has_ray ? 1e20f : -1.0f, r.ray_ex0, r.s_o, r.s_d, r.has_shadow ? r.s_tmax : -1.0f, r.s_ex0, r.s_ex1, hit, found,
                                           occluded, lds_recs);
            }
            if (DEFER) {
                if (r.deferred) {
                    hit.gid = r.d_gid; hit.u = r.d_u; hit.v = r.d_v; hit.t = 0.0f;
                    found = true;
                    r.has_ray = true;
                    r.deferred = false;
                } else if (r.has_ray && found && (iteration & q.defer_metal)) {
                    const uint32_t mat = f2u(sc.shade[(size_t)hit.gid * SHADE_ROWS + 6].y);
                    if (sc.materials[mat].flags & q.defer_flags) {
                        r.d_gid = hit.gid; r.d_u = hit.u; r.d_v = hit.v;
                        r.deferred = true;
                        r.has_ray = false;
                    }
// ... 17 lines not shown
```

akari_render_amd/csrc/host/api_probe.cpp:

```cpp
#if defined(AKR_TEST_HOOKS) && AKR_TEST_HOOKS
#include "api_internal.h"
#include "../../../include/akari_hip_test.h"
#include "../device/dinst.h"
#include "../device/disect.h"
#include "../device/dpath.h"

extern "C" {

AKR_TEST_API int32_t akr_host_stdrng_u64(uint64_t seed, uint32_t n, uint64_t* out) {
    if (!out) return fail(AKR_ERR_INVALID_ARGUMENT, "out is NULL");
    StdRng rng(seed);
    for (uint32_t i = 0; i < n; i++) out[i] = rng.next_u64();
    return AKR_OK;
}
AKR_TEST_API int32_t akr_host_chacha_block(const uint32_t* key8, uint64_t counter, uint64_t stream, int32_t rounds, uint32_t* out16) {
    if (!key8 || !out16) return fail(AKR_ERR_INVALID_ARGUMENT, "NULL argument");
    StdRng::chacha_block(key8, counter, stream, rounds, out16);
    return AKR_OK;
}
AKR_TEST_API int32_t akr_host_pcg32_states(uint64_t seed, uint64_t n, uint64_t* out2n) {
    if (!out2n) return fail(AKR_ERR_INVALID_ARGUMENT, "out is NULL");
    StdRng rng(seed);
    for (uint64_t i = 0; i < n; i++) {
        Pcg32 p = pcg_new_seq_offset(i, rng.next_u64());
// ... 31 lines not shown
        out[k] = fastmod_u32(a[k], fastmod_magic(d[k]), d[k]);
    }
    return AKR_OK;
}
AKR_TEST_API int32_t akr_host_tri_pretest(uint32_t n, const float* rays8, const float* tris9, float plane_shift, uint32_t* may, uint32_t* exact, float* out_t) {
    if (!rays8 || !tris9 || !may || !exact) return fail(AKR_ERR_INVALID_ARGUMENT, "akr_host_tri_pretest: NULL argument");
    for (uint32_t k = 0; k < n; k++) {
        const float* r = rays8 + 8ull * k;
        const float* t = tris9 + 9ull * k;
        const vec3 o = mk3(r[0], r[1], r[2]), d = mk3(r[3], r[4], r[5]), A = mk3(t[0], t[1], t[2]), B = mk3(t[3], t[4], t[5]), C = mk3(t[6], t[7], t[8]);
        may[k] = tri_may_hit(o, d, A, B, C, r[6], r[7], plane_shift) ? 1u : 0u;
        float w[12], tt, u, v;
        woop_precompute(A, B, C, w);
        exact[k] = tri_test(o, d, make_float4(w[0], w[1], w[2], w[3]), make_float4(w[4], w[5], w[6], w[7]), make_float4(w[8], w[9], w[10], w[11]), r[6], r[7], tt, u, v) ? 1u : 0u;
        if (out_t) out_t[k] = tt;
    }
    return AKR_OK;
}
AKR_TEST_API int32_t akr_host_alias_table(const float* weights, uint32_t n, uint32_t* j, float* t, float* pdf) {
    if (!weights || !j || !t || !pdf || n == 0) return fail(AKR_ERR_INVALID_ARGUMENT, "akr_host_alias_table: bad argument");
    return guarded([&] {
        std::vector<float> w(weights, weights + n), p;
        std::vector<AliasEntry> e;
        build_alias_table(w, e, p);
        for (uint32_t i = 0; i < n; i++) { j[i] = e[i].j; t[i] = e[i].t; pdf[i] = p[i]; }
    });
}

AKR_TEST_API int32_t akr_probe_math(akr_context* ctx, uint32_t n, const float* x, float* s, float* c, float* l) {
    if (!ctx || !x || !s || !c || !l) return fail(AKR_ERR_INVALID_ARGUMENT, "akr_probe_math: NULL argument");
    return guarded([&] {
        ctx->bind();
        DevBuf dx, ds, dc, dl;
        std::vector<float> xv(x, x + n);
        dx.upload(xv);
        ds.alloc(n * 4); dc.alloc(n * 4); dl.alloc(n * 4);
        if (n) HIP_CHECK(launch_probe_math(n, dx.as<float>(), ds.as<float>(), dc.as<float>(), dl.as<float>(), ctx->stream));
        HIP_CHECK(hipStreamSynchronize(ctx->stream));
        if (n) {
            HIP_CHECK(hipMemcpy(s, ds.p, n * 4, hipMemcpyDeviceToHost));
            HIP_CHECK(hipMemcpy(c, dc.p, n * 4, hipMemcpyDeviceToHost));
            HIP_CHECK(hipMemcpy(l, dl.p, n * 4, hipMemcpyDeviceToHost));
        }
    });
}
AKR_TEST_API int32_t akr_probe_math2(akr_context* ctx, uint32_t n, const float* xy, float* out6) {
    if (!ctx || !xy || !out6) return fail(AKR_ERR_INVALID_ARGUMENT, "akr_probe_math2: NULL argument");
    return guarded([&] {
        ctx->bind();
        DevBuf dxy, dout;
        dxy.upload(std::vector<float>(xy, xy + 2ull * n));
        dout.alloc(6ull * n * 4);
        if (n) HIP_CHECK(launch_probe_math2(n, dxy.as<float>(), dout.as<float>(), ctx->stream));
        HIP_CHECK(hipStreamSynchronize(ctx->stream));
        if (n) HIP_CHECK(hipMemcpy(out6, dout.p, 6ull * n * 4, hipMemcpyDeviceToHost));
    });
}
AKR_TEST_API int32_t akr_probe_div(akr_context* ctx, uint32_t n, const float* a, const float* b, float* out_fast, float* out_ieee) {
    if (!ctx || !a || !b || !out_fast || !out_ieee) return fail(AKR_ERR_INVALID_ARGUMENT, "akr_probe_div: NULL argument");
    return guarded([&] {
        ctx->bind();
        DevBuf da, db, df, di;
        da.upload(std::vector<float>(a, a + n));
        db.upload(std::vector<float>(b, b + n));
        df.alloc((size_t)n * 4); di.alloc((size_t)n * 4);
        if (n) HIP_CHECK(launch_probe_div(n, da.as<float>(), db.as<float>(), df.as<float>(), di.as<float>(), ctx->stream));
        HIP_CHECK(hipStreamSynchronize(ctx->stream));
        if (n) {
            HIP_CHECK(hipMemcpy(out_fast, df.p, (size_t)n * 4, hipMemcpyDeviceToHost));
            HIP_CHECK(hipMemcpy(out_ieee, di.p, (size_t)n * 4, hipMemcpyDeviceToHost));
        }
    });
}
AKR_TEST_API int32_t akr_probe_pcg_end_pass(akr_context* ctx, uint32_t n, const uint64_t* state, const uint64_t* inc, const uint32_t* dim, uint64_t* out_closed, uint64_t* out_loop) {
    if (!ctx || !state || !inc || !dim || !out_closed || !out_loop) return fail(AKR_ERR_INVALID_ARGUMENT, "akr_probe_pcg_end_pass: NULL argument");
    return guarded([&] {
        ctx->bind();
        DevBuf ds, di, dd, dc, dl;
        ds.upload(std::vector<uint64_t>(state, state + n));
        di.upload(std::vector<uint64_t>(inc, inc + n));
        dd.upload(std::vector<uint32_t>(dim, dim + n));
        dc.alloc((size_t)n * 8); dl.alloc((size_t)n * 8);
        if (n) HIP_CHECK(launch_probe_pcg_end_pass(n, ds.as<uint64_t>(), di.as<uint64_t>(), dd.as<uint32_t>(), dc.as<uint64_t>(), dl.as<uint64_t>(), ctx->stream));
        HIP_CHECK(hipStreamSynchronize(ctx->stream));
        if (n) {
            HIP_CHECK(hipMemcpy(out_closed, dc.p, (size_t)n * 8, hipMemcpyDeviceToHost));
            HIP_CHECK(hipMemcpy(out_loop, dl.p, (size_t)n * 8, hipMemcpyDeviceToHost));
        }
    });
}
AKR_TEST_API int32_t akr_probe_bsdf(akr_context* ctx, const akr_material_desc* m, const float* table, int32_t mode, const float* wo, uint32_t n,
                               const float* in, float* out) {
    if (!ctx || !m || !wo || !in || !out) return fail(AKR_ERR_INVALID_ARGUMENT, "akr_probe_bsdf: NULL argument");
    return guarded([&] {
        ctx->bind();
        std::vector<DMaterial> dm(1, fold_material(*m));
        DevBuf dmat, dtab, din, dout;
        dmat.upload(dm);
        std::vector<float> tab(4096, 0.0f);
        if (table) tab.assign(table, table + 4096);
        dtab.upload(tab);
        std::vector<float> inv(in, in + 3ull * n);
        din.upload(inv);
        size_t out_n = (mode == 0 ? 4ull : 8ull) * n;
        dout.alloc(out_n * 4);
        if (n) HIP_CHECK(launch_probe_bsdf(dmat.as<DMaterial>(), dtab.as<float>(), mode, wo, n, din.as<float>(), dout.as<float>(), ctx->stream));
        HIP_CHECK(hipStreamSynchronize(ctx->stream));
        if (n) HIP_CHECK(hipMemcpy(out, dout.p, out_n * 4, hipMemcpyDeviceToHost));
    });
}
static PtParams probe_params(akr_scene* s) {
    PtParams p;
    std::memset(&p, 0, sizeof p);
    p.sc = s->dscene;
    p.tex_slots = s->cs.has_textures ? s->cs.tex_slots : 0;
    return p;
}
AKR_TEST_API int32_t akr_probe_intersect(akr_context* ctx, akr_scene* scene, uint32_t n, const float* rays, uint32_t* hit_inst_prim, float* bary) {
    if (!ctx || !scene || !rays || !hit_inst_prim || !bary) return fail(AKR_ERR_INVALID_ARGUMENT, "akr_probe_intersect: NULL argument");
    return guarded([&] {
        ctx->bind();
        DevBuf dr, dout, db;
        std::vector<float> rv(rays, rays + 8ull * n);
        dr.upload(rv);
        dout.alloc(3ull * n * 4);
        db.alloc(2ull * n * 4);
        if (n) HIP_CHECK(launch_probe_intersect(probe_params(scene), n, dr.as<float>(), dout.as<uint32_t>(), db.as<float>(), ctx->stream));
        HIP_CHECK(hipStreamSynchronize(ctx->stream));
        if (n) {
            HIP_CHECK(hipMemcpy(hit_inst_prim, dout.p, 3ull * n * 4, hipMemcpyDeviceToHost));
            HIP_CHECK(hipMemcpy(bary, db.p, 2ull * n * 4, hipMemcpyDeviceToHost));
        }
    });
}
AKR_TEST_API int32_t akr_probe_intersect_pair(akr_context* ctx, akr_scene* scene, uint32_t n, const float* rays16, const uint32_t* excl3, uint32_t* out4, float* tuv3) {
    if (!ctx || !scene || !rays16 || !excl3 || !out4 || !tuv3) return fail(AKR_ERR_INVALID_ARGUMENT, "akr_probe_intersect_pair: NULL argument");
    if (scene->ctx != ctx) return fail(AKR_ERR_INVALID_ARGUMENT, "akr_probe_intersect_pair: scene belongs to another context");
    if (scene->dscene.bvh_nodes || scene->dscene.in2.on || scene->dscene.n_tris > 64)
        return fail(AKR_ERR_INVALID_ARGUMENT, "akr_probe_intersect_pair: the pair walk serves scenes of at most 64 triangles");
    return guarded([&] {
        ctx->bind();
        DevBuf dr, de, dout, dt;
        dr.upload(std::vector<float>(rays16, rays16 + 16ull * n));
        de.upload(std::vector<uint32_t>(excl3, excl3 + 3ull * n));
        dout.alloc(4ull * n * 4);
        dt.alloc(3ull * n * 4);
        if (n) HIP_CHECK(launch_probe_intersect_pair(probe_params(scene), n, dr.as<float>(), de.as<uint32_t>(), dout.as<uint32_t>(), dt.as<float>(), ctx->stream));
        HIP_CHECK(hipStreamSynchronize(ctx->stream));
        if (n) {
            HIP_CHECK(hipMemcpy(out4, dout.p, 4ull * n * 4, hipMemcpyDeviceToHost));
            HIP_CHECK(hipMemcpy(tuv3, dt.p, 3ull * n * 4, hipMemcpyDeviceToHost));
        }
    });
}
static int32_t probe_env(akr_context* ctx, akr_scene* scene, uint32_t mode, uint32_t n, const float* in, float* out, const char* name) {
    if (!ctx || !scene || !in || !out) return fail(AKR_ERR_INVALID_ARGUMENT, std::string(name) + ": NULL argument");
    if (scene->ctx != ctx || !scene->cs.env.on) return fail(AKR_ERR_INVALID_ARGUMENT, std::string(name) + ": the scene has no environment light on this context");
    return guarded([&] {
        ctx->bind();
        const size_t n_in = (mode == 0 ? 2ull : 3ull) * n, n_out = (mode == 0 ? 5ull : 4ull) * n;
        DevBuf din, dout;
        din.upload(std::vector<float>(in, in + n_in));
        dout.alloc(n_out * 4);
        if (n) HIP_CHECK(launch_probe_env(probe_params(scene), mode, n, din.as<float>(), dout.as<float>(), ctx->stream));
        HIP_CHECK(hipStreamSynchronize(ctx->stream));
        if (n) HIP_CHECK(hipMemcpy(out, dout.p, n_out * 4, hipMemcpyDeviceToHost));
    });
}
AKR_TEST_API int32_t akr_probe_env_sample(akr_context* ctx, akr_scene* scene, uint32_t n, const float* u2, float* out5) {
    return probe_env(ctx, scene, 0, n, u2, out5, "akr_probe_env_sample");
}
AKR_TEST_API int32_t akr_probe_env_pdf(akr_context* ctx, akr_scene* scene, uint32_t n, const float* dirs3, float* out4) {
    return probe_env(ctx, scene, 1, n, dirs3, out4, "akr_probe_env_pdf");
}
static std::vector<float> rows9_of_rows7(uint32_t n, const float* rows7) {
    std::vector<float> r(9ull * n);
    for (uint32_t i = 0; i < n; i++) {
        for (int k = 0; k < 7; k++) r[9ull * i + k] = rows7[7ull * i + k];
        r[9ull * i + 7] = r[9ull * i + 8] = 0.5f;
    }
    return r;
}
AKR_TEST_API int32_t akr_host_light_sample_soft(const akr_scene* scene, uint32_t n, const float* rows9, float* out13, uint32_t* light) {
    if (!scene || !rows9 || !out13 || !light) return fail(AKR_ERR_INVALID_ARGUMENT, "akr_host_light_sample_soft: NULL argument");
    return guarded([&] {
        std::vector<AliasPacked> la, aa;
        std::vector<LightRec> lr;
        packed_light_tables(scene->cs, la, aa, lr);
        for (uint32_t i = 0; i < n; i++) punct_probe_row(la.data(), lr.data(), scene->cs.punct.data(), scene->cs.n_lights, rows9 + 9ull * i, out13 + 13ull * i, light + i);
    });
}
AKR_TEST_API int32_t akr_host_light_sample(const akr_scene* scene, uint32_t n, const float* rows7, float* out13, uint32_t* light) {
    if (!scene || !rows7 || !out13 || !light) return fail(AKR_ERR_INVALID_ARGUMENT, "akr_host_light_sample: NULL argument");
    return akr_host_light_sample_soft(scene, n, rows9_of_rows7(n, rows7).data(), out13, light);
}
AKR_TEST_API int32_t akr_probe_light_sample_soft(akr_context* ctx, akr_scene* scene, uint32_t n, const float* rows9, float* out13, uint32_t* light) {
    if (!ctx || !scene || !rows9 || !out13 || !light) return fail(AKR_ERR_INVALID_ARGUMENT, "akr_probe_light_sample_soft: NULL argument");
    if (scene->ctx != ctx) return fail(AKR_ERR_INVALID_ARGUMENT, "akr_probe_light_sample_soft: the scene was not created on this context");
    return guarded([&] {
        ctx->bind();
        DevBuf din, dout, dl;
        din.upload(std::vector<float>(rows9, rows9 + 9ull * n));
        dout.alloc(13ull * n * 4);
        dl.alloc(4ull * n);
        if (n) HIP_CHECK(launch_probe_light_sample(probe_params(scene), n, din.as<float>(), dout.as<float>(), dl.as<uint32_t>(), ctx->stream));
        HIP_CHECK(hipStreamSynchronize(ctx->stream));
        if (n) {
            HIP_CHECK(hipMemcpy(out13, dout.p, 13ull * n * 4, hipMemcpyDeviceToHost));
            HIP_CHECK(hipMemcpy(light, dl.p, 4ull * n, hipMemcpyDeviceToHost));
        }
    });
}
AKR_TEST_API int32_t akr_probe_light_sample(akr_context* ctx, akr_scene* scene, uint32_t n, const float* rows7, float* out13, uint32_t* light) {
    if (!ctx || !scene || !rows7 || !out13 || !light) return fail(AKR_ERR_INVALID_ARGUMENT, "akr_probe_light_sample: NULL argument");
    return akr_probe_light_sample_soft(ctx, scene, n, rows9_of_rows7(n, rows7).data(), out13, light);
}
AKR_TEST_API int32_t akr_host_light_tree_sample(const akr_scene* scene, uint32_t n, const float* rows9, float* out13, uint32_t* light, uint32_t* record) {
    if (!scene || !rows9 || !out13 || !light || !record) return fail(AKR_ERR_INVALID_ARGUMENT, "akr_host_light_tree_sample: NULL argument");
    return guarded([&] {
        std::vector<AliasPacked> la, aa;
        std::vector<LightRec> lr;
        packed_light_tables(scene->cs, la, aa, lr);
        const std::vector<DPunct> recs = punctual_device_records(scene->cs.punct, scene->cs.punct_tree);
        const uint32_t tree = scene->cs.punct_tree.empty() ? 0u : (uint32_t)scene->cs.punct.size();
        for (uint32_t i = 0; i < n; i++) light_tree_probe_row(la.data(), lr.data(), recs.data(), tree, scene->cs.n_lights, rows9 + 9ull * i, out13 + 13ull * i, light + i, record + i);
    });
}
AKR_TEST_API int32_t akr_probe_light_tree_sample(akr_context* ctx, akr_scene* scene, uint32_t n, const float* rows9, float* out13, uint32_t* light, uint32_t* record) {
    if (!ctx || !scene || !rows9 || !out13 || !light || !record) return fail(AKR_ERR_INVALID_ARGUMENT, "akr_probe_light_tree_sample: NULL argument");
    if (scene->ctx != ctx) return fail(AKR_ERR_INVALID_ARGUMENT, "akr_probe_light_tree_sample: the scene was not created on this context");
    return guarded([&] {
        ctx->bind();
        DevBuf din, dout, dl, dr;
        din.upload(std::vector<float>(rows9, rows9 + 9ull * n));
        dout.alloc(13ull * n * 4);
        dl.alloc(4ull * n);
        dr.alloc(4ull * n);
        if (n) HIP_CHECK(launch_probe_light_tree_sample(probe_params(scene), n, din.as<float>(), dout.as<float>(), dl.as<uint32_t>(), dr.as<uint32_t>(), ctx->stream));
        HIP_CHECK(hipStreamSynchronize(ctx->stream));
        if (n) {
            HIP_CHECK(hipMemcpy(out13, dout.p, 13ull * n * 4, hipMemcpyDeviceToHost));
            HIP_CHECK(hipMemcpy(light, dl.p, 4ull * n, hipMemcpyDeviceToHost));
            HIP_CHECK(hipMemcpy(record, dr.p, 4ull * n, hipMemcpyDeviceToHost));
        }
    });
}
static PtParams probe_camera_params(const akr_scene* s, uint32_t filter_type, float filter_radius) {
    PtParams p;
    std::memset(&p, 0, sizeof p);
    camera_params(p, s, filter_type, filter_radius);
    return p;
}
AKR_TEST_API int32_t akr_host_lens_ray(const akr_scene* scene, uint32_t filter_type, float filter_radius, uint32_t n, const uint32_t* pixels2, const float* u4, float* out6) {
    if (!scene || !pixels2 || !u4 || !out6) return fail(AKR_ERR_INVALID_ARGUMENT, "akr_host_lens_ray: NULL argument");
    if (filter_type > AKR_FILTER_GAUSSIAN) return fail(AKR_ERR_INVALID_ARGUMENT, "akr_host_lens_ray: unknown filter_type");
    const PtParams p = probe_camera_params(scene, filter_type, filter_radius);
    for (uint32_t i = 0; i < n; i++) {
        const float* u = u4 + 4ull * i;
        vec3 o, d;
        if (p.lens_radius > 0.0f) generate_ray_lens_from(p, pixels2[2ull * i], pixels2[2ull * i + 1], mk2(u[0], u[1]), mk2(u[2], u[3]), o, d);
        else generate_ray_from(p, pixels2[2ull * i], pixels2[2ull * i + 1], mk2(u[0], u[1]), o, d);
        float* r = out6 + 6ull * i;
        r[0] = o.x; r[1] = o.y; r[2] = o.z; r[3] = d.x; r[4] = d.y; r[5] = d.z;
    }
    return AKR_OK;
}
static std::pair<PtVariant, PtLdsLayout> fill_launch_plan(akr_scene* scene, const akr_pt_config* cfg, const TuningOptions& opt, bool feat, akr_pt_launch_plan* out) {
        const CompiledScene& cs = scene->cs;
        const TileGrid grid = tile_grid(cfg->tile_w, cfg->tile_h, scene->flat.camera.width, scene->flat.camera.height, cfg->shard_rank, cfg->shard_count);
        const PtRoute route = pt_route(scene, *cfg, opt, grid, feat, 1);
        if (!route.refusal.empty()) throw Unsupported(route.refusal);
        const PtPlan& pl = route.plan;
        const PtVariant& v = pl.v;
        const PtLdsSizes sizes{scene_stack_depth(cs), cs.n_tris, scene_n_nodes(cs), pl.tex_slots, pl.stage_total, cfg->sampler_type == AKR_SAMPLER_PMJ02BN};
        const PtLdsLayout L = pt_lds_layout(v, sizes);
        std::memset(out, 0, sizeof *out);
        const bool flags[10] = {v.bvh, v.fd, v.tex, v.pmj, v.stage, v.defer, v.simple, v.inst, v.env, v.lens};
        for (int i = 0; i < 10; i++) out->variant[i] = flags[i] ? 1u : 0u;
        out->simple_scene = pl.simple_scene; out->defer_metal = pl.defer_metal; out->defer_flags = pl.defer_flags;
        std::memcpy(out->stage_bytes, pl.stage_bytes, sizeof out->stage_bytes);
        out->stage_total = pl.stage_total;
        out->tile_offset = L.tile_offset; out->bvh_tile_nodes = L.tile_nodes; out->park_offset = L.park_offset; out->carry_offset = L.carry_offset;
        out->bn_offset = L.bn_offset; out->val_offset_words = L.val_offset_words;
        out->lds_bytes = (uint32_t)L.total_bytes;
        out->blocks = (grid.n_items + 255u) / 256u;
        out->specialised = route.spec ? 1u : 0u;
        out->punct = v.punct ? 1u : 0u;
        if (route.spec) std::snprintf(out->wrapper, sizeof out->wrapper, "%s", spec_wrapper_source(v, route.spec_waves).c_str());
        return {v, L};
}
static TuningOptions plan_options(int32_t defer_metal, int32_t simple_kernels, int32_t defer_on, int32_t spec_waves) {
    TuningOptions t;
    t.defer_metal = defer_metal;
    t.simple_kernels = simple_kernels;
    t.defer_on = defer_on;
    t.specialise = spec_waves != 0 ? 1 : 0;
    t.specialise_waves = spec_waves;
    return t;
}
AKR_TEST_API int32_t akr_host_pt_launch_plan(akr_scene* scene, const akr_pt_config* cfg, int32_t defer_metal, int32_t simple_kernels, int32_t defer_on, int32_t spec_waves,
                                             akr_pt_launch_plan* out) {
    if (!scene || !cfg || !out) return fail(AKR_ERR_INVALID_ARGUMENT, "akr_host_pt_launch_plan: NULL argument");
    return guarded([&] { fill_launch_plan(scene, cfg, plan_options(defer_metal, simple_kernels, defer_on, spec_waves), false, out); });
}
AKR_TEST_API int32_t akr_host_pt_features_plan(akr_scene* scene, const akr_pt_config* cfg, int32_t defer_metal, int32_t simple_kernels, int32_t defer_on, int32_t spec_waves, int32_t feat,
                                               int32_t wavefront, int32_t arith, akr_pt_features_plan* out) {
// ... 237 lines not shown
```

akari_render_amd/csrc/host/api_scene.cpp:

```cpp
#include "api_internal.h"

static void ensure_ggx_table(akr_scene* s) {
    akr_context* ctx = s->ctx;
    if (!s->flat.ggx_table.empty()) {
        s->ggx_host = s->flat.ggx_table;
    } else if (s->cs.needs_ggx_table) {
        std::lock_guard<std::mutex> lock(ctx->ggx_mutex);
        if (!ctx->ggx_cache.empty()) {
            s->ggx_host = ctx->ggx_cache;
            s->ggx_table.upload(s->ggx_host);
            return;
        }
        std::vector<uint64_t> seeds(4096);
        StdRng rng(0);
        for (auto& v : seeds) v = rng.next_u64();
        DevBuf dseeds;
        dseeds.upload(seeds);
        s->ggx_table.alloc(4096 * sizeof(float));
        HIP_CHECK(launch_ggx_table(dseeds.as<uint64_t>(), s->ggx_table.as<float>(), 1u << 20, ctx->stream));
        HIP_CHECK(hipStreamSynchronize(ctx->stream));
        s->ggx_host.resize(4096);
        HIP_CHECK(hipMemcpy(s->ggx_host.data(), s->ggx_table.p, 4096 * sizeof(float), hipMemcpyDeviceToHost));
        ctx->ggx_cache = s->ggx_host;
        return;
// ... 63 lines not shown
            DEnv rec;
            std::memset(&rec, 0, sizeof rec);
            rec.texels = s->env_texels.as<float4>();
            rec.marginal = s->env_marginal.as<AliasPacked>();
            rec.conditional = s->env_conditional.as<AliasPacked>();
            for (int k = 0; k < 9; k++) rec.rot[k] = cs.env.rot_t[k];
            rec.w = cs.env.w;
            rec.h = cs.env.h;
            rec.filter = cs.env.filter;
            rec.light = cs.n_lights - 1;
            s->env_rec.alloc(sizeof rec);
            HIP_CHECK(hipMemcpy(s->env_rec.p, &rec, sizeof rec, hipMemcpyHostToDevice));
        } else {
            s->env_texels.release();
            s->env_marginal.release();
            s->env_conditional.release();
            s->env_rec.release();
        }
    }
    DScene& d = s->dscene;
    d.light_entries = s->light_entries.as<AliasEntry>();
    d.light_pdf = s->light_pdf.as<float>();
    d.light_inst = s->light_inst.as<uint32_t>();
    d.light_tri_offset = s->light_tri_offset.as<uint32_t>();
    d.light_alias = s->light_alias.as<AliasPacked>();
    d.area_alias = s->area_alias.as<AliasPacked>();
    d.lights = s->lights.as<LightRec>();
    d.n_lights = cs.n_lights;
    d.env = cs.env.on ? s->env_rec.as<DEnv>() : nullptr;
    d.punct = s->punct.as<DPunct>();
    d.n_punct = (uint32_t)cs.punct.size();
    for (const DPunct& r : cs.punct)
        if (r.radius != 0.0f || r.cos_max != 0.0f) d.n_punct |= kPunctSoftBit;
    d.punct_tree = cs.punct_tree.empty() ? 0u : (uint32_t)cs.punct.size();
}
static void count_device_bytes(akr_scene* s) {
    s->device_bytes = 0;
    for (const DevBuf* b : {&s->woop, &s->tri_gid, &s->shade, &s->normals, &s->inst, &s->materials, &s->ggx_table, &s->light_entries,
                            &s->light_pdf, &s->light_inst, &s->light_tri_offset, &s->light_n_tris, &s->area_entries, &s->area_pdf,
                            &s->inst_tri_offset, &s->light_alias, &s->area_alias, &s->lights, &s->bvh_nodes, &s->tex_nodes, &s->tex_images, &s->tex_texels, &s->tex_mat_inputs,
                            &s->in2_tlas_leaves, &s->in2_mesh_tris, &s->in2_mesh_pos, &s->in2_mesh_meta, &s->in2_mesh_normals, &s->in2_inst_mats, &s->in2_share_bits,
                            &s->env_texels, &s->env_marginal, &s->env_conditional, &s->env_rec, &s->punct})
        s->device_bytes += b->bytes;
}

static float walk_origin_bound(const std::vector<float>& woop, uint32_t n) {
    double s_max = 0.0, w_max = 0.0;
    for (uint32_t k = 0; k < n; k++) {
        const float* r = &woop[12ull * k + 8];
        if (!(std::isfinite(r[0]) && std::isfinite(r[1]) && std::isfinite(r[2]) && std::isfinite(r[3]))) return -1.0f;
        s_max = std::max(s_max, std::fabs((double)r[0]) + std::fabs((double)r[1]) + std::fabs((double)r[2]));
        w_max = std::max(w_max, std::fabs((double)r[3]));
    }
    const double limit = 0x1p45;
    if (!(2.0 * s_max <= limit && w_max < limit)) return -1.0f;
    double b = 0x1p40;
    while (b >= 0x1p-40 && s_max * b + w_max > limit) b *= 0.5;
    return b >= 0x1p-40 ? (float)b : -1.0f;
}

static void check_lens_reach(const akr_scene* s, const HostLens& lens) {
    const CompiledScene& cs = s->cs;
    if (lens.radius == 0.0f || (cs.bvh_nodes.empty() && !cs.instanced.on)) return;
    const float* c2w = s->flat.camera.c2w;
    float bound[3], moved[16];
    lens_origin_bound(c2w, lens.radius, bound);
    std::memcpy(moved, c2w, sizeof moved);
    bool inside = true;
    for (int a = 0; a < 3; a++) {
        const float m = std::max(std::max(std::fabs(cs.scene_lo[a]), std::fabs(cs.scene_hi[a])), std::fabs(c2w[12 + a]));
        if (bound[a] > m) inside = false;
        moved[12 + a] = bound[a];
    }
    if (inside || (!cs.instanced.on && bvh_box_padding(cs.scene_lo, cs.scene_hi, moved) == bvh_box_padding(cs.scene_lo, cs.scene_hi, c2w))) return;
    char msg[320];
    std::snprintf(msg, sizeof msg, "lens: a lens of radius %g puts ray origins at coordinates up to (%g, %g, %g), beyond the magnitude the scene's acceleration "
                  "structure was padded for (its box and the camera position); use a smaller radius", lens.radius, bound[0], bound[1], bound[2]);
    throw std::invalid_argument(msg);
}

void akr_api::scene_finish(akr_scene* s, const TuningOptions& opt) {
    akr_context* ctx = s->ctx;
    compile_scene(s->flat, opt, s->cs);
    compile_punctual(s->flat, s->cs);
    compile_environment(s->flat, s->cs);
    check_lens_reach(s, s->flat.lens);
    CompiledScene& cs = s->cs;
    camera_matrices(s->flat.camera, s->r2c, s->c2w, &s->c2w_identity);
    if (!ctx) {
        s->ggx_host = s->flat.ggx_table.empty() ? std::vector<float>(4096, 0.0f) : s->flat.ggx_table;
        std::memset(&s->dscene, 0, sizeof s->dscene);
        return;
    }
    ctx->bind();
    if (cs.bvh_nodes.empty() && !cs.instanced.on && cs.woop.size() > walk_bound_word(cs.n_tris))
        cs.woop[walk_bound_word(cs.n_tris)] = walk_origin_bound(cs.woop, cs.n_tris);
    s->woop.upload(cs.woop);
    s->tri_gid.upload(cs.tri_gid);
    s->shade.upload(cs.shade);
    s->normals.upload(cs.normals);
    s->inst.upload(cs.inst);
    s->materials.upload(cs.materials);
    s->area_entries.upload(cs.area_entries);
    s->area_pdf.upload(cs.area_pdf);
    s->inst_tri_offset.upload(cs.inst_tri_offset);
    s->bvh_nodes.upload(cs.instanced.on ? cs.instanced.nodes : cs.bvh_nodes);
    if (cs.instanced.on) {
        s->in2_tlas_leaves.upload(cs.instanced.tlas_leaves);
        s->in2_mesh_tris.upload(cs.instanced.mesh_tris);
        s->in2_mesh_pos.upload(cs.instanced.mesh_pos);
        s->in2_mesh_meta.upload(cs.instanced.mesh_meta);
        s->in2_mesh_normals.upload(cs.instanced.mesh_normals);
        s->in2_inst_mats.upload(cs.instanced.inst_mats);
    }
    if (cs.has_textures) {
        s->tex_nodes.upload(cs.tex_nodes);
        s->tex_images.upload(cs.images);
        s->tex_texels.upload(cs.texels);
        s->tex_mat_inputs.upload(cs.mat_inputs);
    }
    ensure_ggx_table(s);
    DScene& d = s->dscene;
    std::memset(&d, 0, sizeof d);
    d.woop = s->woop.as<float4>();
    d.tri_gid = s->tri_gid.as<uint32_t>();
    d.shade = s->shade.as<float4>();
    d.normals = s->normals.as<float4>();
    d.inst = s->inst.as<float4>();
    d.materials = s->materials.as<DMaterial>();
    d.ggx_table = s->ggx_table.as<float>();
    d.area_entries = s->area_entries.as<AliasEntry>();
    d.area_pdf = s->area_pdf.as<float>();
    d.inst_tri_offset = s->inst_tri_offset.as<uint32_t>();
    upload_lights(s);
    d.bvh_nodes = s->bvh_nodes.as<uint4>();
    d.n_tris = cs.n_tris;
    d.n_nodes = scene_n_nodes(cs);
    d.has_alpha = cs.has_alpha ? 1u : 0u;
    d.bvh_stack_depth = scene_stack_depth(cs);
    if (cs.instanced.on) {
        d.in2.tlas_leaves = s->in2_tlas_leaves.as<uint4>();
        d.in2.mesh_tris = s->in2_mesh_tris.as<float4>();
        d.in2.mesh_pos = s->in2_mesh_pos.as<uint32_t>();
        d.in2.mesh_meta = s->in2_mesh_meta.as<uint32_t>();
        d.in2.mesh_normals = s->in2_mesh_normals.as<float4>();
        d.in2.inst_mats = s->in2_inst_mats.as<uint32_t>();
        d.in2.on = 1u;
        d.in2.n_instances = (uint32_t)s->flat.instances.size();
    }
    d.plane_share_mask = 0;
    if (cs.bvh_nodes.empty() && !cs.instanced.on)
        for (uint32_t k = 1; k < d.n_tris && k < 64; k++)
            if (std::memcmp(&cs.woop[12ull * k + 8], &cs.woop[12ull * (k - 1) + 8], 16) == 0) d.plane_share_mask |= 1ull << k;
    if (cs.has_textures) {
        d.tex.nodes = s->tex_nodes.as<DNode>();
        d.tex.images = s->tex_images.as<DImage>();
        d.tex.texels = s->tex_texels.as<uint32_t>();
        d.tex.mat_inputs = s->tex_mat_inputs.as<MatInputs>();
    }
    if (cs.instanced.on) {
        const size_t words = ((size_t)cs.n_tris + 31u) / 32u;
        s->in2_share_bits.alloc(std::max<size_t>(words, 1u) * 4u);
        HIP_CHECK(hipMemsetAsync(s->in2_share_bits.p, 0, s->in2_share_bits.bytes, ctx->stream));
        HIP_CHECK(launch_inst_share_bits(d, s->in2_share_bits.as<uint32_t>(), s->in2_mesh_tris.as<uint32_t>(), ctx->stream));
        HIP_CHECK(hipStreamSynchronize(ctx->stream));
        d.in2.share_bits = s->in2_share_bits.as<uint32_t>();
    }
    count_device_bytes(s);
}

static uint64_t compiled_scene_bytes(const CompiledScene& cs) {
    auto b = [](const auto& v) { return (uint64_t)v.size() * sizeof(v[0]); };
    uint64_t n = b(cs.woop) + b(cs.tri_gid) + b(cs.shade) + b(cs.normals) + b(cs.inst) + b(cs.materials) + b(cs.light_entries) + b(cs.light_pdf) +
                 b(cs.light_inst) + b(cs.light_tri_offset) + b(cs.light_n_tris) + b(cs.area_entries) + b(cs.area_pdf) + b(cs.inst_tri_offset) +
                 16ull * (cs.light_entries.size() + cs.area_entries.size() + cs.n_lights) + b(cs.bvh_nodes) + b(cs.tex_nodes) + b(cs.images) + b(cs.texels) +
                 b(cs.mat_inputs);
    n += (uint64_t)punctual_device_records(cs.punct, cs.punct_tree).size() * sizeof(DPunct);
    n += b(cs.env.texels) + 16ull * (cs.env.marginal_entries.size() + cs.env.conditional_entries.size()) + (cs.env.on ? sizeof(DEnv) : 0u);
    const CompiledScene::Instanced& is = cs.instanced;
    return n + b(is.nodes) + b(is.tlas_leaves) + b(is.mesh_tris) + b(is.mesh_pos) + b(is.mesh_meta) + b(is.mesh_normals) + b(is.inst_mats) + (is.on ? std::max<uint64_t>(((uint64_t)cs.n_tris + 31u) / 32u, 1u) * 4u : 0u);
}

extern "C" {

AKR_API int32_t akr_scene_create(akr_context* ctx, const akr_scene_desc* desc, akr_scene** out) {
    if (!desc || !out) return fail(AKR_ERR_INVALID_ARGUMENT, "akr_scene_create: NULL argument");
    *out = nullptr;
    return guarded([&] {
        auto s = std::make_unique<akr_scene>();
        s->ctx = ctx;
        const TuningOptions opt = tuning();
        s->flat = FlatScene::from_desc(*desc);
        s->flat.light_tree = opt.light_tree;
        scene_finish(s.get(), opt);
        *out = s.release();
    });
}
AKR_API int32_t akr_scene_load(akr_context* ctx, const char* path, uint32_t width, uint32_t height, akr_scene** out) {
    if (!path || !out) return fail(AKR_ERR_INVALID_ARGUMENT, "akr_scene_load: NULL argument");
    *out = nullptr;
    return guarded([&] {
        auto s = std::make_unique<akr_scene>();
        s->ctx = ctx;
        const TuningOptions opt = tuning();
        s->flat = load_scene_json(path, opt);
        s->flat.light_tree = opt.light_tree;
        if (width && height) {
            s->flat.camera.width = width;
            s->flat.camera.height = height;
        }
        scene_finish(s.get(), opt);
        *out = s.release();
    });
}
AKR_API int32_t akr_scene_destroy(akr_scene* scene) {
    if (!scene) return AKR_OK;
    return guarded([&] {
        if (scene->ctx) (void)hipSetDevice(scene->ctx->device);
        delete scene;
    });
}
AKR_API int32_t akr_scene_set_resolution(akr_scene* s, uint32_t width, uint32_t height) {
    if (!s || !width || !height) return fail(AKR_ERR_INVALID_ARGUMENT, "akr_scene_set_resolution: bad argument");
    if (s->sessions.load() != 0) return fail(AKR_ERR_INVALID_ARGUMENT, "akr_scene_set_resolution: a session holds the scene (end it first)");
    s->flat.camera.width = width;
    s->flat.camera.height = height;
    camera_matrices(s->flat.camera, s->r2c, s->c2w, &s->c2w_identity);
    return AKR_OK;
}
AKR_API int32_t akr_scene_get_info(const akr_scene* s, akr_scene_info* info) {
    if (!s || !info) return fail(AKR_ERR_INVALID_ARGUMENT, "akr_scene_get_info: NULL argument");
    info->width = s->flat.camera.width;
    info->height = s->flat.camera.height;
    info->n_instances = (uint32_t)s->flat.instances.size();
    info->n_triangles = s->cs.n_tris;
    info->n_materials = (uint32_t)s->flat.materials.size();
    info->n_lights = s->cs.n_lights;
    info->n_bvh_nodes = (uint32_t)((s->cs.instanced.on ? s->cs.instanced.nodes.size() : s->cs.bvh_nodes.size()) / kBvhNodeWords);
    info->uses_bvh = (s->cs.bvh_nodes.empty() && !s->cs.instanced.on) ? 0u : (s->cs.instanced.on ? 2u : 1u);
    info->device_bytes = s->device_bytes ? s->device_bytes : compiled_scene_bytes(s->cs);
    info->node_bytes = (s->cs.bvh_nodes.empty() && !s->cs.instanced.on) ? 0u : kBvhNodeWords * 4u;
    info->node_stride_bytes = (s->cs.bvh_nodes.empty() && !s->cs.instanced.on) ? 0u : kBvhNodeWords * 4u;
    info->tri_bytes = (s->cs.bvh_nodes.empty() && !s->cs.instanced.on) ? 48u : kBvhTriWords * 4u;
    info->bvh_depth = s->cs.bvh_depth;
    return AKR_OK;
}
AKR_API int32_t akr_scene_set_environment(akr_scene* s, const akr_environment_desc* desc) {
    if (!s) return fail(AKR_ERR_INVALID_ARGUMENT, "akr_scene_set_environment: scene is NULL");
    return guarded([&] {
        if (s->sessions.load() != 0) throw std::invalid_argument("akr_scene_set_environment: a session holds the scene (end it first)");
        HostEnvironment env;
        if (desc) env = environment_from_desc(*desc);
        std::swap(s->flat.env, env);
        try {
            compile_environment(s->flat, s->cs);
        } catch (...) {
            std::swap(s->flat.env, env);
            throw;
        }
        if (s->ctx) {
            s->ctx->bind();
            upload_lights(s);
            count_device_bytes(s);
        }
    });
}
AKR_API int32_t akr_scene_get_environment(const akr_scene* s, akr_environment_desc* out) {
    if (!s || !out) return fail(AKR_ERR_INVALID_ARGUMENT, "akr_scene_get_environment: NULL argument");
    const HostEnvironment& e = s->flat.env;
    std::memset(out, 0, sizeof *out);
    for (int k = 0; k < 9; k++) out->rotation[k] = e.rotation[k];
    if (!e.set) return AKR_OK;
    out->width = e.width;
    out->height = e.height;
    out->filter = e.filter;
    out->texels = e.texels.empty() ? nullptr : e.texels.data();
    for (int c = 0; c < 3; c++) out->color[c] = e.color[c];
    out->strength = e.strength;
    return AKR_OK;
}
static void punctual_lights_changed(akr_scene* s, std::vector<akr_punctual_light_desc>& before) {
    try {
        compile_punctual(s->flat, s->cs);
    } catch (...) {
        std::swap(s->flat.punct, before);
        throw;
    }
    if (s->ctx) {
        s->ctx->bind();
        upload_lights(s);
        count_device_bytes(s);
        std::lock_guard<std::mutex> lock(s->color_sets_mutex);
        for (auto& kv : s->color_sets) kv.second->punct.release();
    }
}
AKR_API int32_t akr_scene_add_punctual_light(akr_scene* s, const akr_punctual_light_desc* desc) {
    if (!s || !desc) return fail(AKR_ERR_INVALID_ARGUMENT, "akr_scene_add_punctual_light: NULL argument");
    return guarded([&] {
        if (s->sessions.load() != 0) throw std::invalid_argument("akr_scene_add_punctual_light: a session holds the scene (end it first)");
        akr_punctual_light_desc checked;
        if (!punctual_from_desc(*desc, checked)) return;
        std::vector<akr_punctual_light_desc> before = s->flat.punct;
        s->flat.punct.push_back(checked);
        punctual_lights_changed(s, before);
    });
}
// ... 230 lines not shown
```

akari_render_amd/csrc/host/scene_build.cpp:

```cpp
#include "scene_build.h"
#include "../device/dinst.h"
#include "host_parallel.h"

#include <chrono>
#include <cstdio>
#include <cmath>
#include <cstdlib>
#include <cstring>
#include <deque>
#include <stdexcept>

#include "../device/dgeom.h"

namespace akr {

FlatScene FlatScene::from_desc(const akr_scene_desc& d) {
    FlatScene s;
    if ((d.n_meshes && !d.meshes) || (d.n_instances && !d.instances) || (d.n_materials && !d.materials))
        throw std::invalid_argument("akr_scene_desc: null array with non-zero count");
    s.meshes.resize(d.n_meshes);
    for (uint32_t i = 0; i < d.n_meshes; i++) {
        const akr_mesh_desc& m = d.meshes[i];
        if (!m.vertices || !m.indices || m.n_triangles == 0) throw std::invalid_argument("akr_mesh_desc: empty mesh");
        HostMesh& h = s.meshes[i];
// ... 375 lines not shown
    out.tex_nodes.clear();
    out.tex_nodes_ssa.clear();
    out.shader_kinds.clear();
    out.mat_inputs.clear();
    out.has_textures = false;
    out.tex_slots = 0;
    descs = flat.materials;
    for (size_t mi = 0; mi < flat.materials.size(); mi++) {
        DMaterial d;
        if (!flat.graphs.empty() && !flat.graphs[mi].nodes.empty()) {
            compile_graph(flat.graphs[mi], flat.images, color, (uint32_t)mi, descs[mi], d, out);
        } else {
            d = fold_material(descs[mi], color);
            MatInputs in;
            std::memcpy(&in, &descs[mi], sizeof in);
            const bool fed[4] = {false, false, false, false};
            convert_color_inputs(in, descs[mi].kind, color, fed);
            in.kind = descs[mi].kind & MAT_KIND_MASK;
            std::memcpy(&descs[mi], &in, sizeof in);
        }
        const bool tex = (d.flags & MF_TEXTURED) != 0;
        if ((d.kind == MAT_PRINCIPLED || d.kind == MAT_DIFFUSE) && (d.base_alpha < 1.0f || (d.flags & MF_ALPHA_TEXTURED))) out.has_alpha = true;
        if (d.kind == MAT_PRINCIPLED && ((d.flags & (MF_SPEC | MF_COAT)) || tex)) out.needs_ggx_table = true;
        out.materials.push_back(d);
    }
    if (out.has_textures) {
        out.mat_inputs.resize(descs.size());
        std::memcpy(out.mat_inputs.data(), descs.data(), descs.size() * sizeof(MatInputs));
    }
    uint32_t absent = AB_COAT | AB_TRANSMISSION | AB_NORMAL_MAP | AB_GLASS | AB_METAL;
    for (const DMaterial& m : out.materials) {
        auto fed = [&](uint32_t k) { return (m.flags & MF_TEXTURED) && m.tex_input[k] != kNodeNone; };
        if (m.kind == MAT_GLASS) absent &= ~(uint32_t)AB_GLASS;
        if (m.kind != MAT_PRINCIPLED) continue;
        if (m.coat_weight != 0.0f || (m.flags & MF_COAT) || fed(IN_COAT_WEIGHT)) absent &= ~(uint32_t)AB_COAT;
        if (m.transmission != 0.0f || (m.flags & MF_EVAL_DIEL) || fed(IN_TRANSMISSION_WEIGHT)) absent &= ~(uint32_t)AB_TRANSMISSION;
        if ((m.flags & MF_NORMAL_MAP) || fed(IN_NORMAL)) absent &= ~(uint32_t)AB_NORMAL_MAP;
        if (m.metallic != 0.0f || (m.flags & MF_EVAL_METAL) || fed(IN_METALLIC)) absent &= ~(uint32_t)AB_METAL;
    }
    out.absent = absent;
}

float triangle_emission_power(const CompiledScene& out, const TexScene& host_tex, uint32_t material, uint32_t prim, vec2 uv0, vec2 uv1, vec2 uv2, float area) {
    const DMaterial& dm = out.materials[material];
    vec3 e = (dm.kind == MAT_PRINCIPLED || dm.kind == MAT_EMISSION) ? dm.emission : mk3(0, 0, 0);
    float acc = 0.0f;
    const bool tex_emission = (dm.flags & MF_TEXTURED) && (dm.kind == MAT_PRINCIPLED || dm.kind == MAT_EMISSION) &&
                              (dm.tex_input[IN_EMISSION_COLOR] != kNodeNone || dm.tex_input[IN_EMISSION_STRENGTH] != kNodeNone);
    if (tex_emission) {
        Pcg32 rng = pcg_new_seq((uint64_t)prim);
        for (int k = 0; k < 16; k++) {
            float u0 = pcg_next_1d(rng), u1 = pcg_next_1d(rng);
            vec2 bary = uniform_sample_triangle(mk2(u0, u1));
            (void)pcg_next_1d(rng);
            (void)pcg_next_1d(rng);
            float w = 1.0f - bary.x - bary.y;
            vec2 uv = mk2((uv0.x * w + uv1.x * bary.x) + uv2.x * bary.y, (uv0.y * w + uv1.y * bary.x) + uv2.y * bary.y);
            DMaterial at = dm;
            material_at(host_tex, material, uv, at);
            acc += max3(at.emission) * area;
        }
    } else {
        for (int k = 0; k < 16; k++) acc += max3(e) * area;
    }
    return acc / 16.0f;
}
bool instance_may_emit(const CompiledScene& out, const std::vector<akr_material_desc>& descs, const HostInstance& in) {
    bool any = false;
    for (uint32_t mi : in.materials) {
        const akr_material_desc& m = descs[mi];
        if (m.kind != AKR_MAT_PRINCIPLED && m.kind != AKR_MAT_EMISSION) { any = true; continue; }
        const DMaterial& dm = out.materials[mi];
        if ((dm.flags & MF_TEXTURED) && (dm.tex_input[IN_EMISSION_COLOR] != kNodeNone || dm.tex_input[IN_EMISSION_STRENGTH] != kNodeNone)) {
            any = true;
            continue;
        }
        float power = max_f(max_f(m.emission_color[0], m.emission_color[1]), m.emission_color[2]);
        if (!(power * m.emission_strength == 0.0f)) any = true;
    }
    return any;
}

namespace {
struct PhaseTimer {
    bool on = std::getenv("AKR_TIMING") != nullptr;
    std::chrono::steady_clock::time_point t = std::chrono::steady_clock::now();
    void lap(const char* what) {
        if (!on) return;
        auto n = std::chrono::steady_clock::now();
        std::fprintf(stderr, "[akari_hip] compile_scene: %-28s %.3f s\n", what, std::chrono::duration<double>(n - t).count());
        t = n;
    }
};
}
void compile_scene(const FlatScene& flat, const TuningOptions& tune, CompiledScene& out) {
    PhaseTimer phase;
    const size_t n_inst = flat.instances.size();
    out = CompiledScene();
    out.materials.reserve(flat.materials.size());
    if (!flat.graphs.empty() && flat.graphs.size() != flat.materials.size())
        throw std::invalid_argument("material graphs: one per material expected");
    for (const HostImage& im : flat.images) {
        while (im.format == AKR_IMAGE_RGBA32F && (out.texels.size() & 3u)) out.texels.push_back(0u);
        DImage d{};
        uint64_t off = out.texels.size();
        d.offset_lo = (uint32_t)off; d.offset_hi = (uint32_t)(off >> 32);
        d.width = im.width; d.height = im.height; d.format = im.format; d.filter = im.filter; d.address = im.address;
        out.images.push_back(d);
        out.texels.insert(out.texels.end(), im.words.begin(), im.words.end());
    }
    std::vector<akr_material_desc> descs;
    compile_materials(flat, 0, out, descs);
    const TexScene host_tex{out.tex_nodes.data(), out.images.data(), out.texels.data(), out.mat_inputs.data(), 0, 0};
    std::vector<InstXf> xf(n_inst);
    out.inst.assign(32 * n_inst, 0.0f);
    out.inst_tri_offset.resize(n_inst + 1);
    uint32_t n_tris = 0;
    bool any_normals = false;
    {
        uint64_t total = 0;
        for (const HostInstance& in : flat.instances)
            if (in.mesh < flat.meshes.size()) total += flat.meshes[in.mesh].n_triangles();
        if (total >= 0xffffffffull)
            throw std::runtime_error("unsupported: " + std::to_string(total) + " instance-triangles; global triangle ids are 32 bits");
    }
    for (size_t i = 0; i < n_inst; i++) {
        const HostInstance& in = flat.instances[i];
        xf[i] = make_xform(in.transform);
        const InstXf& x = xf[i];
        float* r = &out.inst[32 * i];
        r[0] = x.c0.x; r[1] = x.c0.y; r[2] = x.c0.z; r[3] = x.det;
        r[4] = x.c1.x; r[5] = x.c1.y; r[6] = x.c1.z;
        r[8] = x.c2.x; r[9] = x.c2.y; r[10] = x.c2.z;
        r[12] = x.t.x; r[13] = x.t.y; r[14] = x.t.z;
        r[16] = x.k0.x; r[17] = x.k0.y; r[18] = x.k0.z; r[19] = x.inv_det;
        r[20] = x.k1.x; r[21] = x.k1.y; r[22] = x.k1.z;
        r[24] = x.k2.x; r[25] = x.k2.y; r[26] = x.k2.z;
        out.inst_tri_offset[i] = n_tris;
        n_tris += flat.meshes[in.mesh].n_triangles();
        if (!flat.meshes[in.mesh].normals.empty() || !flat.meshes[in.mesh].tangents.empty()) any_normals = true;
    }
    out.inst_tri_offset[n_inst] = n_tris;
    out.n_tris = n_tris;
    if (want_instancing(flat, tune)) {
        compile_instanced_geometry(flat, tune, xf, descs, out);
        phase.lap("instanced geometry");
        return;
    }
    out.woop.assign(12ull * n_tris, 0.0f);
    out.shade.assign(32ull * n_tris, 0.0f);
    if (any_normals) out.normals.assign(24ull * n_tris, 0.0f);
    std::vector<float> bounds(6ull * n_tris);
    std::vector<float> tri_power(n_tris, 0.0f);
    std::vector<float> tri_cond(3ull * n_tris, 0.0f);
    for (int a = 0; a < 3; a++) { out.scene_lo[a] = INFINITY; out.scene_hi[a] = -INFINITY; }

    struct TriChunk { size_t inst; uint32_t first, last; float lo[3], hi[3]; std::string error; bool bad_slot = false; };
    std::vector<TriChunk> chunks;
    {
        const uint32_t kChunk = 1u << 16;
        for (size_t i = 0; i < n_inst; i++) {
            const uint32_t nt = flat.meshes[flat.instances[i].mesh].n_triangles();
            for (uint32_t f = 0; f < nt; f += kChunk) {
                TriChunk c;
                c.inst = i; c.first = f; c.last = std::min(nt, f + kChunk);
                for (int a = 0; a < 3; a++) { c.lo[a] = INFINITY; c.hi[a] = -INFINITY; }
                chunks.push_back(c);
            }
        }
    }
    parallel_chunks((unsigned)chunks.size(), n_tris > (1u << 17) ? host_threads() : 1u, [&](unsigned ci) {
        TriChunk& chunk = chunks[ci];
        const size_t i = chunk.inst;
        const HostInstance& in = flat.instances[i];
        const HostMesh& g = flat.meshes[in.mesh];
        const InstXf& x = xf[i];
        for (uint32_t prim = chunk.first; prim < chunk.last; prim++) {
            const uint32_t gid = out.inst_tri_offset[i] + prim;
            uint32_t slot = (g.slots.size() > 1) ? g.slots[prim] : 0;
            if (slot >= in.materials.size()) { chunk.bad_slot = true; return; }
            uint32_t material = in.materials[slot];
            vec3 v0 = ld3(g.vertices, g.indices[3 * prim]), v1 = ld3(g.vertices, g.indices[3 * prim + 1]), v2 = ld3(g.vertices, g.indices[3 * prim + 2]);
            vec2 uv0, uv1, uv2;
            tri_default_uvs(uv0, uv1, uv2);
            if (!g.uvs.empty()) {
                uv0 = mk2(g.uvs[6 * prim + 0], g.uvs[6 * prim + 1]);
                uv1 = mk2(g.uvs[6 * prim + 2], g.uvs[6 * prim + 3]);
                uv2 = mk2(g.uvs[6 * prim + 4], g.uvs[6 * prim + 5]);
            }
            const TriWorld tw = tri_world(x, v0, v1, v2, uv0, uv1, uv2);
            const vec3 ng_local = tw.ng_local, tt = tw.tt, ng = tw.ng;
            const float area = tw.area;
            const Frame fr = tw.frame;
            uint32_t tri_flags = 0;
            bool tangents_ok = false;
            if (!g.tangents.empty()) {
                tangents_ok = true;
                for (int k = 0; k < 9; k++) tangents_ok = tangents_ok && is_finite(g.tangents[9 * prim + k]);
            }
            if (!g.normals.empty()) tri_flags |= TRI_HAS_NORMALS;
            if (tangents_ok) tri_flags |= 2u;
            float* r = &out.shade[32ull * gid];
            r[0] = v0.x; r[1] = v0.y; r[2] = v0.z; r[3] = uv0.x;
            r[4] = v1.x; r[5] = v1.y; r[6] = v1.z; r[7] = uv0.y;
            r[8] = v2.x; r[9] = v2.y; r[10] = v2.z; r[11] = uv1.x;
            r[12] = ng.x; r[13] = ng.y; r[14] = ng.z; r[15] = uv1.y;
            r[16] = fr.t.x; r[17] = fr.t.y; r[18] = fr.t.z; r[19] = uv2.x;
            r[20] = fr.s.x; r[21] = fr.s.y; r[22] = fr.s.z; r[23] = uv2.y;
            r[24] = area; r[25] = u2f(material); r[26] = u2f((uint32_t)i); r[27] = u2f(0xffffffffu);
            r[28] = tt.x; r[29] = tt.y; r[30] = tt.z; r[31] = u2f(tri_flags);
            if (any_normals) {
                float* nr = &out.normals[24ull * gid];
                for (int k = 0; k < 3; k++) {
                    vec3 nk = g.normals.empty() ? ng_local : mk3(g.normals[9 * prim + 3 * k], g.normals[9 * prim + 3 * k + 1], g.normals[9 * prim + 3 * k + 2]);
                    nr[4 * k] = nk.x; nr[4 * k + 1] = nk.y; nr[4 * k + 2] = nk.z;
                    if (tangents_ok) {
                        nr[12 + 4 * k] = g.tangents[9 * prim + 3 * k]; nr[12 + 4 * k + 1] = g.tangents[9 * prim + 3 * k + 1];
                        nr[12 + 4 * k + 2] = g.tangents[9 * prim + 3 * k + 2];
                    }
                }
            }
            vec3 A = xf_point(x.c0, x.c1, x.c2, x.t, v0), B = xf_point(x.c0, x.c1, x.c2, x.t, v1), C = xf_point(x.c0, x.c1, x.c2, x.t, v2);
            woop_precompute(A, B, C, &out.woop[12ull * gid]);
            if (prim & 1u) {
                const vec3 vb[3] = {A, B, C};
                share_plane_row(&out.woop[12ull * (gid - 1) + 8], &out.woop[12ull * gid + 8], vb);
            }
            float* bb = &bounds[6ull * gid];
            bb[0] = min_f(min_f(A.x, B.x), C.x); bb[1] = min_f(min_f(A.y, B.y), C.y); bb[2] = min_f(min_f(A.z, B.z), C.z);
            bb[3] = max_f(max_f(A.x, B.x), C.x); bb[4] = max_f(max_f(A.y, B.y), C.y); bb[5] = max_f(max_f(A.z, B.z), C.z);
            {
                const double Ad[3] = {A.x, A.y, A.z}, Bd[3] = {B.x, B.y, B.z}, Cd[3] = {C.x, C.y, C.z};
                tri_conditioning(Ad, Bd, Cd, &tri_cond[3ull * gid]);
            }
            if (!(is_finite(A.x) && is_finite(A.y) && is_finite(A.z) && is_finite(B.x) && is_finite(B.y) && is_finite(B.z) && is_finite(C.x) &&
                  is_finite(C.y) && is_finite(C.z)))
            {
                chunk.error = "instance " + std::to_string(i) + ", triangle " + std::to_string(prim) + ": non-finite vertex position after the instance transform";
                return;
            }
            for (int a = 0; a < 3; a++) {
                chunk.lo[a] = min_f(chunk.lo[a], bb[a]);
                chunk.hi[a] = max_f(chunk.hi[a], bb[3 + a]);
            }
            tri_power[gid] = triangle_emission_power(out, host_tex, material, prim, uv0, uv1, uv2, area);
        }
    });
    for (const TriChunk& c : chunks) {
        if (c.bad_slot) throw std::invalid_argument("material slot out of range for instance");
        if (!c.error.empty()) throw std::invalid_argument(c.error);
        for (int a = 0; a < 3; a++) {
            out.scene_lo[a] = min_f(out.scene_lo[a], c.lo[a]);
            out.scene_hi[a] = max_f(out.scene_hi[a], c.hi[a]);
        }
    }
    phase.lap("triangle records");
    std::vector<float> light_weights;
    for (size_t i = 0; i < n_inst; i++) {
        const HostInstance& in = flat.instances[i];
        const bool any = instance_may_emit(out, descs, in);
        if (!any) continue;
        uint32_t first = out.inst_tri_offset[i], count = out.inst_tri_offset[i + 1] - first;
        std::vector<float> powers(tri_power.begin() + first, tri_power.begin() + first + count);
        float total = 0.0f;
        for (float pw : powers) total += pw;
        if (total > 1e-4f) {
            uint32_t light_id = (uint32_t)out.light_inst.size();
            out.light_inst.push_back((uint32_t)i);
            out.light_power.push_back(total);
            light_weights.push_back(total);
            std::vector<AliasEntry> ent;
            std::vector<float> pdf;
            build_alias_table(powers, ent, pdf);
            out.light_tri_offset.push_back((uint32_t)out.area_entries.size());
            out.light_n_tris.push_back(count);
            out.area_entries.insert(out.area_entries.end(), ent.begin(), ent.end());
            out.area_pdf.insert(out.area_pdf.end(), pdf.begin(), pdf.end());
            for (uint32_t k = 0; k < count; k++) out.shade[32ull * (first + k) + 27] = u2f(light_id);
        }
    }
    out.n_lights = (uint32_t)out.light_inst.size();
    if (out.n_lights > 0) build_alias_table(light_weights, out.light_entries, out.light_pdf);

    phase.lap("light tables");
    const uint32_t kExhaustiveMax = tune.force_bvh ? 0u : 64u;
    const size_t stage = exhaustive_stage_bytes(out, out.n_lights);
    if (n_tris > kExhaustiveMax || stage > kStageMaxBytes) {
        const float pad_scale = 0.01f * (float)tune.pad_percent;
        const float pad = pad_scale * bvh_box_padding(out.scene_lo, out.scene_hi, flat.camera.c2w);
        {
            const unsigned nc = n_tris > (1u << 17) ? host_threads() * 4 : 1;
            parallel_chunks(nc, host_threads(), [&](unsigned c) {
                const uint32_t lo = (uint32_t)((uint64_t)n_tris * c / nc), hi = (uint32_t)((uint64_t)n_tris * (c + 1) / nc);
                for (uint32_t g = lo; g < hi; g++) {
                    const float* k = &tri_cond[3ull * g];
                    float* bb = &bounds[6ull * g];
                    const float mag = box_magnitude(bb, bb + 3);
                    for (int a = 0; a < 3; a++) {
                        const float extra = pad_scale * tri_cond_extra(k[a], mag, pad / pad_scale);
                        if (extra > 0.0f) {
                            bb[a] -= extra;
                            bb[3 + a] += extra;
                        }
                    }
                }
            });
        }
        std::vector<float>().swap(tri_cond);
        std::vector<uint32_t> order;
        const bool force_balanced = tune.bvh_balanced != 0;
        build_bvh8(bounds, n_tris, pad, kBvhNodeWords, force_balanced, order, out.bvh_nodes, out.bvh_depth);
        if (out.bvh_depth > kBvhStackDepth) build_bvh8(bounds, n_tris, pad, kBvhNodeWords, true, order, out.bvh_nodes, out.bvh_depth);
        if (out.bvh_depth > kBvhStackDepth)
            throw std::runtime_error("unsupported: BVH depth " + std::to_string(out.bvh_depth) + " exceeds the traversal stack (" +
                                     std::to_string(kBvhStackDepth) + " levels)");
        phase.lap("BVH build");
        std::vector<float> rec((size_t)kBvhTriWords * n_tris, 0.0f);
        {
            const unsigned nc = n_tris > (1u << 17) ? host_threads() * 4 : 1;
            parallel_chunks(nc, host_threads(), [&](unsigned c) {
                const uint32_t lo = (uint32_t)((uint64_t)n_tris * c / nc), hi = (uint32_t)((uint64_t)n_tris * (c + 1) / nc);
                for (uint32_t k = lo; k < hi; k++) {
                    std::memcpy(&rec[(size_t)kBvhTriWords * k], &out.woop[12ull * order[k]], 48);
                    rec[(size_t)kBvhTriWords * k + 12] = u2f(order[k]);
                }
            });
        }
        out.woop.swap(rec);
        out.tri_gid = order;
        phase.lap("records in traversal order");
    }
    out.woop.resize(out.woop.size() + 32, 0.0f);
}

size_t exhaustive_stage_bytes(const CompiledScene& out, size_t n_lights) {
    size_t stage = 0;
    for (size_t b : {out.shade.size() * 4, out.normals.size() * 4, out.inst.size() * 4, out.materials.size() * sizeof(DMaterial),
                     n_lights * 32 , out.area_entries.size() * 16, n_lights * 4, out.area_pdf.size() * 4,
                     out.tex_nodes.size() * sizeof(DNode), out.images.size() * sizeof(DImage), out.mat_inputs.size() * sizeof(MatInputs)})
        stage += (b + 15) & ~(size_t)15;
    return stage;
}

}
```

akari_render_amd/csrc/host/scene_build.h:

```cpp
#pragma once
#include <cmath>
#include <stdint.h>

#include <string>
#include <vector>

#include "../../../include/akari_hip.h"
#include "../kernels.h"
#include "options.h"

namespace akr {

struct HostMesh {
    std::vector<float> vertices;
    std::vector<uint32_t> indices;
    std::vector<float> uvs;
    std::vector<float> normals;
    std::vector<float> tangents;
    std::vector<uint32_t> slots;
    uint32_t n_triangles() const { return (uint32_t)(indices.size() / 3); }
};
struct HostInstance {
    uint32_t mesh = 0;
    std::vector<uint32_t> materials;
    float transform[16];
};
struct HostImage {
    uint32_t width = 0, height = 0, format = 0, filter = 0, address = 0;
    std::vector<uint32_t> words;
};
struct HostGraph {
    std::vector<akr_shader_node> nodes;
    uint32_t input[AKR_IN_COUNT];
    HostGraph() { for (uint32_t& i : input) i = AKR_NODE_NONE; }
};
struct HostEnvironment {
    bool set = false;
    uint32_t width = 0, height = 0;
    uint32_t filter = 0;
    std::vector<float> texels;
    float color[3] = {0, 0, 0};
    float strength = 0.0f;
    float rotation[9] = {1, 0, 0, 0, 1, 0, 0, 0, 1};
};
struct HostLens {
    float radius = 0.0f, focal_distance = 0.0f;
};
inline HostLens lens_from_values(float radius, float focal_distance) {
    if (!std::isfinite(radius) || !std::isfinite(focal_distance) || radius < 0.0f || focal_distance < 0.0f)
        throw std::invalid_argument("lens: radius and focal_distance must be finite and >= 0");
    if (radius > 0.0f && !(focal_distance > 0.0f)) throw std::invalid_argument("lens: a radius > 0 needs a focal_distance > 0");
    HostLens l;
    if (radius > 0.0f) { l.radius = radius; l.focal_distance = focal_distance; }
    return l;
}
struct FlatScene {
    std::vector<HostMesh> meshes;
    std::vector<HostInstance> instances;
    std::vector<akr_material_desc> materials;
    akr_camera_desc camera;
    std::vector<float> ggx_table;
    std::vector<HostImage> images;
    std::vector<HostGraph> graphs;
    HostEnvironment env;
    std::vector<akr_punctual_light_desc> punct;
    int light_tree = 0;
    HostLens lens;
    static FlatScene from_desc(const akr_scene_desc& d);
};

struct CompiledScene {
    uint32_t n_tris = 0, n_lights = 0;
    std::vector<float> woop;
    std::vector<uint32_t> tri_gid;
    std::vector<float> shade;
    std::vector<float> normals;
    std::vector<float> inst;
    std::vector<DMaterial> materials;
    std::vector<uint32_t> inst_tri_offset;
    std::vector<AliasEntry> light_entries;
    std::vector<float> light_pdf, light_power;
    std::vector<uint32_t> light_inst, light_tri_offset, light_n_tris;
    std::vector<AliasEntry> area_entries;
    std::vector<float> area_pdf;
    std::vector<uint32_t> bvh_nodes;
    uint32_t bvh_depth = 0;
    std::vector<DNode> tex_nodes;
    std::vector<DImage> images;
    std::vector<uint32_t> texels;
    std::vector<MatInputs> mat_inputs;
    uint32_t tex_slots = 0;
    std::vector<akr_shader_node> tex_nodes_ssa;
    struct ShaderKind {
        std::string signature;
        uint32_t mat_kind = 0, n_nodes = 0;
        std::vector<uint32_t> materials;
    };
    std::vector<ShaderKind> shader_kinds;
    uint32_t absent = 0;
    struct Instanced {
        bool on = false;
        std::vector<uint32_t> nodes;
        std::vector<float> tlas_leaves;
        std::vector<float> mesh_tris;
        std::vector<uint32_t> mesh_pos;
        std::vector<uint32_t> mesh_meta;
        std::vector<float> mesh_normals;
        std::vector<uint32_t> inst_mats;
        std::vector<uint32_t> inst_light;
        uint32_t tlas_nodes = 0, tlas_depth = 0, blas_depth = 0, n_mesh_tris = 0;
        uint32_t n_padding_classes = 0;
    } instanced;
    struct Environment {
        bool on = false;
        uint32_t w = 0, h = 0, filter = 0;
        std::vector<float> texels;
        std::vector<AliasEntry> marginal_entries, conditional_entries;
        std::vector<float> marginal_pdf, conditional_pdf;
        float rot_t[9] = {1, 0, 0, 0, 1, 0, 0, 0, 1};
        float power = 0.0f;
    } env;
    std::vector<DPunct> punct;
    std::vector<uint32_t> punct_tree;
    bool has_textures = false;
    bool has_alpha = false;
    bool needs_ggx_table = false;
    float scene_lo[3], scene_hi[3];
    bool has_tree() const { return !bvh_nodes.empty() || instanced.on; }
};

inline float bvh_box_padding(const float lo[3], const float hi[3], const float* c2w ) {
    float diag2 = 0.0f, reach = 0.0f;
    for (int a = 0; a < 3; a++) {
        diag2 += (hi[a] - lo[a]) * (hi[a] - lo[a]);
        const float m = std::fabs(lo[a]) > std::fabs(hi[a]) ? std::fabs(lo[a]) : std::fabs(hi[a]);
        const float c = std::fabs(c2w[12 + a]);
        reach += m > c ? m : c;
    }
    const float diag = __builtin_sqrtf(diag2);
    return 4e-6f * (diag > reach ? diag : reach);
}
inline void lens_origin_bound(const float* c2w , float radius, float out[3]) {
    const double w = std::fabs((double)c2w[15]) > 0.0 ? std::fabs((double)c2w[15]) : 1.0;
    for (int a = 0; a < 3; a++)
        out[a] = (float)(((double)std::fabs(c2w[12 + a]) + (double)radius * std::sqrt((double)c2w[a] * c2w[a] + (double)c2w[4 + a] * c2w[4 + a])) / w * 1.000001);
}

constexpr float kTriCondEps = 10.0f * 5.9604645e-8f;
constexpr float kTriCondFree = 0.64f;
inline void tri_conditioning(const double A[3], const double B[3], const double C[3], float k[3]) {
    const double e1[3] = {B[0] - A[0], B[1] - A[1], B[2] - A[2]}, e2[3] = {C[0] - A[0], C[1] - A[1], C[2] - A[2]};
    const double n[3] = {e1[1] * e2[2] - e1[2] * e2[1], e1[2] * e2[0] - e1[0] * e2[2], e1[0] * e2[1] - e1[1] * e2[0]};
    const double nl = std::sqrt(n[0] * n[0] + n[1] * n[1] + n[2] * n[2]);
    const double l1 = std::sqrt(e1[0] * e1[0] + e1[1] * e1[1] + e1[2] * e1[2]), l2 = std::sqrt(e2[0] * e2[0] + e2[1] * e2[1] + e2[2] * e2[2]);
    for (int a = 0; a < 3; a++) {
        const double v = nl > 0.0 ? (l2 * std::fabs(e1[a]) + l1 * std::fabs(e2[a])) / nl : 0.0;
        k[a] = v < 1e30 ? (float)(v * 1.0001) : 1e30f;
    }
}
inline float tri_cond_extra(float k, float magnitude, float pad) {
    const float need = kTriCondEps * magnitude * k, have = kTriCondFree * pad;
    return need > have ? need - have : 0.0f;
}
inline float box_magnitude(const float lo[3], const float hi[3]) {
    float m2 = 0.0f;
    for (int a = 0; a < 3; a++) {
        const float m = std::fabs(lo[a]) > std::fabs(hi[a]) ? std::fabs(lo[a]) : std::fabs(hi[a]);
        m2 += m * m;
    }
    return __builtin_sqrtf(m2) * 1.0001f;
}
DMaterial fold_material(const akr_material_desc& m, uint32_t color = 0);
void compile_materials(const FlatScene& flat, uint32_t color, CompiledScene& out, std::vector<akr_material_desc>& descs);
void build_alias_table(const std::vector<float>& weights, std::vector<AliasEntry>& entries, std::vector<float>& pdf);
constexpr uint64_t kSpecAutoSamples = 1ull << 31;

void compile_scene(const FlatScene& flat, const TuningOptions& opt, CompiledScene& out);
size_t exhaustive_stage_bytes(const CompiledScene& out, size_t n_lights);
std::string punctual_light_name(const CompiledScene& cs);
constexpr uint32_t kEnvConstW = 32, kEnvConstH = 16;
void compile_environment(const FlatScene& flat, CompiledScene& out);
HostEnvironment environment_from_desc(const akr_environment_desc& d);
void rebuild_light_alias(CompiledScene& out);
bool punctual_from_desc(const akr_punctual_light_desc& d, akr_punctual_light_desc& out);
DPunct fold_punctual(const akr_punctual_light_desc& d, uint32_t color);
void compile_punctual(const FlatScene& flat, CompiledScene& out);
std::vector<uint32_t> build_light_tree(const std::vector<DPunct>& recs, const std::vector<float>& weights);
std::vector<DPunct> punctual_device_records(const std::vector<DPunct>& recs, const std::vector<uint32_t>& tree);
float triangle_emission_power(const CompiledScene& out, const TexScene& host_tex, uint32_t material, uint32_t prim, vec2 uv0, vec2 uv1, vec2 uv2, float area);
bool instance_may_emit(const CompiledScene& out, const std::vector<akr_material_desc>& descs, const HostInstance& in);
bool want_instancing(const FlatScene& flat, const TuningOptions& opt);
struct InstXf;
void compile_instanced_geometry(const FlatScene& flat, const TuningOptions& opt, const std::vector<InstXf>& xf, const std::vector<akr_material_desc>& descs, CompiledScene& out);
void camera_matrices(const akr_camera_desc& cam, float r2c[16], float c2w[16], uint32_t* c2w_identity);
PcgStartConsts pcg_start_constants();

FlatScene load_scene_json(const std::string& path, const TuningOptions& opt);
void parse_method_json(const std::string& text, akr_pt_config* cfg, std::string* film_out);
constexpr size_t kStageMaxBytes = 32 * 1024;
constexpr size_t kStageMaxBytesBvh = 12 * 1024;

struct ParsedTask {
    bool is_aov = false;
    akr_pt_config cfg;
    akr_aov_config aov;
    bool is_gpt = false;
    akr_gpt_config gpt;
    bool is_mcmc = false;
    akr_mcmc_config mcmc;
    std::string film_out;
};
std::vector<ParsedTask> parse_render_tasks(const std::string& text, bool allow_sampler_override);
void make_pmj02_sets(std::vector<uint32_t>& out);
void load_bluenoise(std::vector<uint16_t>& out);
void write_image(const std::string& path, const float* rgb, uint32_t w, uint32_t h);
void decode_png(const uint8_t* data, size_t n, uint32_t& w, uint32_t& h, std::vector<uint8_t>& rgba);
void decode_jpeg(const uint8_t* data, size_t n, uint32_t& w, uint32_t& h, std::vector<uint8_t>& rgba);
void decode_exr(const uint8_t* data, size_t n, uint32_t& w, uint32_t& h, std::vector<float>& rgba);
void decode_tiff(const uint8_t* data, size_t n, uint32_t& w, uint32_t& h, std::vector<uint8_t>& rgba);
void decode_dds(const uint8_t* data, size_t n, uint32_t& w, uint32_t& h, std::vector<uint8_t>& rgba);
std::vector<uint8_t> inflate_zlib_stream(const uint8_t* data, size_t n);

}
```

akari_render_amd/csrc/kernels.h:

```cpp
#pragma once
#if !defined(__HIPCC_RTC__)
#include <hip/hip_runtime.h>
#endif

#include "device/drng.h"
#include "device/dscene.h"

#if !defined(__HIPCC_RTC__)
#include <algorithm>
struct PtVariant {
    bool bvh = false, fd = false, tex = false, pmj = false, stage = false, defer = false, simple = false, inst = false, env = false, lens = false;
    bool feat = false;
    bool punct = false;
    bool ltree = false;
};
constexpr bool pt_variant_compiled(const PtVariant& v) {
    return (v.bvh || v.stage) && !(v.defer && (v.fd || (v.bvh && !v.tex))) && !(v.simple && (v.fd || v.tex)) && !((v.env || v.lens || v.feat || v.punct) && (v.defer || v.simple)) &&
           !(v.inst && !(v.bvh && !v.stage && !v.defer && !v.simple && !v.feat)) && !(v.punct && (v.feat || v.inst)) && !(v.ltree && !v.punct);
}
constexpr uint32_t pt_variant_bits(const PtVariant& v) {
    return (v.bvh ? 1u : 0u) | (v.pmj ? 2u : 0u) | (v.stage ? 4u : 0u) | (v.defer ? 8u : 0u) | (v.inst ? 16u : 0u) | (v.env ? 32u : 0u) | (v.lens ? 64u : 0u) |
           (v.feat ? 128u : 0u) | (v.punct ? 256u : 0u) | (v.ltree ? 512u : 0u);
}
constexpr PtVariant pt_variant_from_bits(uint32_t f) {
// ... 132 lines not shown
    uint32_t last_pass_spp;
    PcgStartConsts start;
    Pcg32* states;
    float* film;
    uint64_t* counters;
    uint32_t sampler;
    uint32_t smp_seed, smp_spp, smp_w;
    uint64_t smp_mod_magic;
    const uint32_t* pmj_sets;
    const uint16_t* bluenoise;
    uint32_t stage_bytes[13];
    uint32_t stage_total;
    uint32_t simple_scene;
    uint32_t defer_metal;
    uint32_t defer_flags;
    uint32_t tex_slots;
    uint32_t tile_offset;
    uint32_t park_offset;
    uint32_t carry_offset;
    uint32_t bn_offset;
    uint32_t wf_sort;
    float sort_lo[3], sort_scale[3];
    uint32_t n_items;
    uint32_t shard_rank, shard_count;
    uint32_t tile_w, tile_h, tiles_x, tiles_y;
    const uint32_t* owned_tiles;
    uint32_t* item_cost;
    const uint32_t* item_pixels;
    float lens_radius, lens_focal;
    float *feat_albedo, *feat_normal;
};

AKR_HD uint32_t morton_spread16(uint32_t x) {
    x &= 0xffffu;
    x = (x | (x << 8)) & 0x00ff00ffu;
    x = (x | (x << 4)) & 0x0f0f0f0fu;
    x = (x | (x << 2)) & 0x33333333u;
    x = (x | (x << 1)) & 0x55555555u;
    return x;
}
AKR_HD uint32_t tile_morton(uint32_t tx, uint32_t ty) { return morton_spread16(tx) | (morton_spread16(ty) << 1); }
AKR_HD uint32_t tile_owner(uint32_t tx, uint32_t ty, uint32_t count) { return tile_morton(tx, ty) % count; }

struct WfBuffers {
    float4 *ray_o, *ray_d;
    float4 *sh_o, *sh_d, *sh_c;
    float4* hit;
    float4 *beta, *rad, *base;
    float4* film;
    uint4 *rng, *misc;
    uint32_t* queue_closest[2];
    uint32_t* queue_shadow[2];
    uint32_t* key_closest[2];
    uint32_t* key_shadow[2];
    uint32_t* qcount;
    uint32_t* qhead;
    uint32_t* n_active;
    uint32_t* pend;
    uint32_t* carry;
    uint32_t carry_words, n_slots;
    uint32_t carry_queue;
    uint32_t carry_lanes, carry_steps;
    uint32_t slot_base, slot_end;
};

struct GptParams {
    float* own;
    float* shifted[4];
    float *acc_p, *acc_gx, *acc_gy, *sqr_p, *sqr_gx, *sqr_gy;
    uint32_t reconnect, stride, separate_weights, reconstruction;
    const uint32_t* item_pixels;
    uint32_t shard_rank, shard_count, tile_w, tile_h, tiles_x;
};

struct PssSample {
    float cur, backup;
    uint32_t last_modified, modified_backup;
};
struct MarkovState {
    uint32_t cur_pixel[2], chain_id;
    float cur_f, b;
    uint32_t b_cnt, n_accepted, n_mutations, cur_iter, last_large_iter;
};
struct McmcParams {
    PssSample* pss;
    MarkovState* states;
    float4* cur_colors;
    Pcg32* rngs;
    const Pcg32* seeds;
    float* fs;
    const uint32_t* resampled;
    float* film;
    uint32_t n_chains, n_bootstrap, dim, width, height;
    uint32_t chain_begin, chain_count;
    uint32_t exponential_mutation;
    float small_sigma, large_step_prob, image_mutation_prob, image_mutation_size;
};
#if !defined(__HIPCC_RTC__)
hipError_t launch_mcmc_bootstrap(const PtParams& p, const McmcParams& m, hipStream_t stream);
hipError_t launch_mcmc_init(const PtParams& p, const McmcParams& m, hipStream_t stream);
hipError_t launch_mcmc_advance(const PtParams& p, const McmcParams& m, uint32_t mutations_per_chain, float contribution, hipStream_t stream);
#endif

#if !defined(__HIPCC_RTC__)
inline PtLdsSizes pt_lds_sizes(const PtParams& p) {
    return PtLdsSizes{p.sc.bvh_stack_depth, p.sc.n_tris, p.sc.n_nodes, p.tex_slots, p.stage_total, p.sampler == 1u && p.bluenoise != nullptr};
}
inline PtParams pt_params_with_layout(const PtParams& p, const PtLdsLayout& L) {
    PtParams q = p;
    q.tile_offset = L.tile_offset; q.sc.bvh_tile_nodes = L.tile_nodes; q.park_offset = L.park_offset; q.carry_offset = L.carry_offset;
    q.bn_offset = L.bn_offset; q.sc.tex.val_offset_words = L.val_offset_words;
    return q;
}
#endif
inline PtParams with_tex_slots(const PtParams& p, size_t base_bytes, size_t& lds_bytes) {
    PtParams q = p;
    base_bytes = (base_bytes + 15) & ~(size_t)15;
    q.sc.tex.val_offset_words = (uint32_t)(base_bytes / 4);
    lds_bytes = base_bytes + (p.sc.tex.nodes != nullptr ? (size_t)p.tex_slots * kTexValStride * sizeof(TexVal) : 0);
    return q;
}
#if !defined(__HIPCC_RTC__)
hipError_t launch_inst_share_bits(const DScene& sc, uint32_t* bits, uint32_t* mesh_tri_words, hipStream_t stream);
hipError_t launch_probe_env(const PtParams& p, uint32_t mode, uint32_t n, const float* in, float* out, hipStream_t stream);
hipError_t launch_probe_light_sample(const PtParams& p, uint32_t n, const float* rows9, float* out13, uint32_t* light, hipStream_t stream);
hipError_t launch_probe_light_tree_sample(const PtParams& p, uint32_t n, const float* rows9, float* out13, uint32_t* light, uint32_t* record, hipStream_t stream);
hipError_t launch_probe_camera_rays(const PtParams& p, uint32_t n, const uint32_t* pixels2, const float* u4, float* out6, hipStream_t stream);
hipError_t launch_pt_pass(const PtParams& p, const PtVariant& v, hipStream_t stream, hipFunction_t spec_fn = nullptr, bool relaxed = false);
hipError_t launch_gpt_sample(const PtParams& p, const GptParams& g, hipStream_t stream);
hipError_t launch_gpt_update(const GptParams& g, uint32_t W, uint32_t H, float* film, hipStream_t stream);
hipError_t launch_gpt_recon_init(const GptParams& g, uint32_t W, uint32_t H, float* old, float spp, hipStream_t stream);
hipError_t launch_gpt_recon(const GptParams& g, uint32_t W, uint32_t H, const float* old, float* cur, float scaling, float spp, hipStream_t stream);
hipError_t launch_aov(const PtParams& p, uint32_t spp, uint32_t aov, uint32_t remap, hipStream_t stream);
hipError_t launch_wf_init(const PtParams& p, const WfBuffers& wf, hipStream_t stream);
hipError_t launch_wf_shade(const PtParams& p, const WfBuffers& wf, uint32_t q_out, hipStream_t stream);
uint32_t wf_trace_blocks_per_cu(const PtParams& p);
hipError_t launch_wf_trace(const PtParams& p, const WfBuffers& wf, uint32_t q_in, uint32_t n_blocks, hipStream_t stream);
size_t wf_sort_temp_bytes(uint32_t n);
hipError_t wf_sort_pairs(void* temp, size_t temp_bytes, const uint32_t* keys_in, uint32_t* keys_out, const uint32_t* vals_in, uint32_t* vals_out, uint32_t n, hipStream_t stream);
size_t cost_order_temp_bytes(uint32_t n_padded);
hipError_t launch_cost_order(const PtParams& p, uint32_t n_padded, uint64_t* keys, uint64_t* keys_sorted, void* temp, size_t temp_bytes, uint32_t* table, hipStream_t stream);
hipError_t launch_cost_to_pixels(const PtParams& p, const uint32_t* item_cost, uint32_t* pixel_cost, hipStream_t stream);
hipError_t launch_probe_material(const PtParams& p, uint32_t material, uint32_t n, const float* uv, uint32_t* out, hipStream_t stream);
hipError_t launch_init_pcg32(const uint64_t* seeds, void* states, uint64_t n, hipStream_t stream);
hipError_t launch_film_resolve(const float* film, uint64_t n, float splat_scale, float* rgb, hipStream_t stream);
hipError_t launch_ggx_table(const uint64_t* seeds, float* table, uint32_t samples, hipStream_t stream);
hipError_t launch_probe_math(uint32_t n, const float* x, float* s, float* c, float* l, hipStream_t stream);
hipError_t launch_probe_math2(uint32_t n, const float* xy, float* out, hipStream_t stream);
hipError_t launch_probe_bsdf(const DMaterial* m, const float* table, int mode, const float* wo, uint32_t n, const float* in, float* out,
                             hipStream_t stream);
hipError_t launch_probe_div(uint32_t n, const float* a, const float* b, float* out_fast, float* out_ieee, hipStream_t stream);
hipError_t launch_probe_pcg_end_pass(uint32_t n, const uint64_t* state, const uint64_t* inc, const uint32_t* dim, uint64_t* out_closed, uint64_t* out_loop, hipStream_t stream);
hipError_t launch_probe_intersect_pair(const PtParams& p, uint32_t n, const float* rays, const uint32_t* excl, uint32_t* out, float* out_tuv, hipStream_t stream);
hipError_t launch_probe_intersect(const PtParams& p, uint32_t n, const float* rays, uint32_t* out, float* bary, hipStream_t stream);
hipError_t launch_probe_si(const PtParams& p, uint32_t n, const uint32_t* inst_prim, const float* bary, float* out, hipStream_t stream);
#endif

}
```

akari_render_amd/csrc/probe_kernels.hip:

```cpp
#include "device/pt_pass.h"
#include "launch.h"

namespace akr {

__global__ void k_probe_math(uint32_t n, const float* __restrict__ x, float* s, float* c, float* l) {
    uint32_t i = blockIdx.x * blockDim.x + threadIdx.x;
    if (i >= n) return;
    float sv, cv;
    sincos_f(x[i], sv, cv);
    s[i] = sv;
    c[i] = cv;
    l[i] = log_f(x[i]);
}
__global__ void k_probe_math2(uint32_t n, const float* __restrict__ xy, float* __restrict__ out) {
    uint32_t i = blockIdx.x * blockDim.x + threadIdx.x;
    if (i >= n) return;
    const float x = xy[2 * (size_t)i], y = xy[2 * (size_t)i + 1];
    float* o = out + 6 * (size_t)i;
    o[0] = exp_f(x);
    o[1] = pow_f(x, y);
    o[2] = atan2_f(y, x);
    o[3] = sqrt_f(x);
    o[4] = rcp_f(x);
    o[5] = srgb_to_linear1(x);
}
__global__ void k_probe_div(uint32_t n, const float* __restrict__ a, const float* __restrict__ b, float* __restrict__ out_fast, float* __restrict__ out_ieee) {
    uint32_t i = blockIdx.x * blockDim.x + threadIdx.x;
    if (i >= n) return;
    out_fast[i] = div_f_unscaled(a[i], b[i]);
    out_ieee[i] = div_f(a[i], b[i]);
}
__global__ void k_probe_pcg_end_pass(uint32_t n, const uint64_t* __restrict__ state, const uint64_t* __restrict__ inc, const uint32_t* __restrict__ dim,
                                     uint64_t* __restrict__ out_closed, uint64_t* __restrict__ out_loop) {
    uint32_t i = blockIdx.x * blockDim.x + threadIdx.x;
    if (i >= n) return;
    Pcg32 a{state[i], inc[i]}, b = a;
    pcg_end_pass(a, dim[i]);
    pcg_advance(b, -(int64_t)dim[i]);
    out_closed[i] = a.state;
    out_loop[i] = b.state;
}
__global__ void k_probe_bsdf(const DMaterial* __restrict__ m, const float* __restrict__ table, int mode, vec3 wo, uint32_t n,
                             const float* __restrict__ in, float* __restrict__ out) {
    uint32_t i = blockIdx.x * blockDim.x + threadIdx.x;
    if (i >= n) return;
    ShadePoint sp;
    shade_point_init(sp, *m, frame_from_n(mk3(0, 0, 1)), mk3(0, 0, 1), false);
    if (mode == 0) {
        BsdfEval e = shade_evaluate(sp, *m, table, wo, mk3(in[3 * i], in[3 * i + 1], in[3 * i + 2]));
        out[4 * i + 0] = e.f.x;
        out[4 * i + 1] = e.f.y;
        out[4 * i + 2] = e.f.z;
        out[4 * i + 3] = e.pdf;
    } else {
        BsdfSample s = shade_sample(sp, *m, table, wo, in[3 * i], mk2(in[3 * i + 1], in[3 * i + 2]));
        float* o = out + 8 * (size_t)i;
        o[0] = s.wi.x; o[1] = s.wi.y; o[2] = s.wi.z;
        o[3] = s.color.x; o[4] = s.color.y; o[5] = s.color.z;
        o[6] = s.pdf;
        o[7] = s.valid ? 1.0f : 0.0f;
    }
}
template <bool BVH, bool INST = false>
__global__ __launch_bounds__(256) void k_probe_intersect(PtParams p, uint32_t n, const float* __restrict__ rays, uint32_t* __restrict__ out, float* __restrict__ bary) {
    extern __shared__ __attribute__((aligned(16))) uint32_t lds_stack[];
    TraceCtx tc;
    tc.stack = lds_stack + threadIdx.x;
    tc.cnt = TraceCounters{0, 0, 0};
    uint32_t i = blockIdx.x * blockDim.x + threadIdx.x;
    bool act = i < n;
    const float* r = rays + 8 * (size_t)(act ? i : 0);
    Hit h;
    bool found = INST ? trace_inst<false, false>(p.sc, mk3(r[0], r[1], r[2]), mk3(r[3], r[4], r[5]), r[6], r[7], kInvalid, kInvalid, h, tc.stack, tc.cnt)
                      : trace<BVH, false>(p, tc, mk3(r[0], r[1], r[2]), mk3(r[3], r[4], r[5]), r[6], r[7], kInvalid, kInvalid, h);
    if (!act) return;
    uint32_t inst = 0, prim = 0;
    if (found) {
        inst = INST ? inst_of_gid(p.sc, h.gid) : f2u(p.sc.shade[(size_t)h.gid * SHADE_ROWS + 6].z);
        prim = h.gid - p.sc.inst_tri_offset[inst];
    }
    out[3 * i + 0] = found ? 1u : 0u;
    out[3 * i + 1] = inst;
    out[3 * i + 2] = prim;
    bary[2 * i + 0] = found ? h.u : 0.0f;
    bary[2 * i + 1] = found ? h.v : 0.0f;
}
__global__ __launch_bounds__(256) void k_probe_intersect_pair(PtParams p, uint32_t n, const float* __restrict__ rays, const uint32_t* __restrict__ excl, uint32_t* __restrict__ out,
                                                              float* __restrict__ out_tuv) {
    extern __shared__ __attribute__((aligned(16))) uint32_t lds_stack[];
    const uint32_t* g = (const uint32_t*)p.sc.woop;
    for (uint32_t i = threadIdx.x; i < (p.sc.n_tris + 2u) * 12u; i += 256u) lds_stack[i] = g[i];
    __syncthreads();
    const uint32_t i = blockIdx.x * blockDim.x + threadIdx.x;
    const bool act = i < n;
    const float* r = rays + 16 * (size_t)(act ? i : 0);
    const uint32_t* e = excl + 3 * (size_t)(act ? i : 0);
    Hit h;
    bool found = false, occluded = false;
    uint32_t redo = 0;
    trace_pair_exhaustive<false>(p.sc, mk3(r[0], r[1], r[2]), mk3(r[3], r[4], r[5]), act ? r[6] : -1.0f, e[0], mk3(r[8], r[9], r[10]), mk3(r[11], r[12], r[13]),
                                 act ? r[14] : -1.0f, e[1], e[2], h, found, occluded, (const float4*)lds_stack, &redo);
    if (!act) return;
    out[4 * i + 0] = found ? 1u : 0u;
    out[4 * i + 1] = h.gid;
    out[4 * i + 2] = occluded ? 1u : 0u;
    out[4 * i + 3] = redo;
    out_tuv[3 * i + 0] = h.t;
    out_tuv[3 * i + 1] = h.u;
    out_tuv[3 * i + 2] = h.v;
}
template <bool INST>
__global__ void k_probe_si(PtParams p, uint32_t n, const uint32_t* __restrict__ inst_prim, const float* __restrict__ bary, float* __restrict__ out) {
    uint32_t i = blockIdx.x * blockDim.x + threadIdx.x;
    if (i >= n) return;
    uint32_t gid = p.sc.inst_tri_offset[inst_prim[2 * i]] + inst_prim[2 * i + 1];
    SurfacePoint s = surface_interaction_any<INST>(p.sc, gid, mk2(bary[2 * i], bary[2 * i + 1]));
    float* o = out + 19 * (size_t)i;
    o[0] = s.p.x; o[1] = s.p.y; o[2] = s.p.z;
    o[3] = s.ng.x; o[4] = s.ng.y; o[5] = s.ng.z;
    o[6] = s.frame.n.x; o[7] = s.frame.n.y; o[8] = s.frame.n.z;
    o[9] = s.frame.t.x; o[10] = s.frame.t.y; o[11] = s.frame.t.z;
    o[12] = s.frame.s.x; o[13] = s.frame.s.y; o[14] = s.frame.s.z;
    o[15] = s.uv.x;
    o[16] = s.uv.y;
    o[17] = s.prim_area;
    o[18] = (float)s.material;
}

__global__ void k_probe_material(PtParams p, uint32_t material, uint32_t n, const float* __restrict__ uv, uint32_t* __restrict__ out) {
    uint32_t i = blockIdx.x * blockDim.x + threadIdx.x;
    if (i >= n) return;
    const DMaterial& m = p.sc.materials[material];
    MatInputs in = p.sc.tex.mat_inputs[material];
    if (m.flags & MF_TEXTURED) {
        eval_material_graph(p.sc.tex, m.tex_first_node, m.tex_n_nodes & kTexCountMask, mk2(uv[2 * i], uv[2 * i + 1]), in);
    }
    const uint32_t* w = reinterpret_cast<const uint32_t*>(&in);
    for (uint32_t k = 0; k < 26; k++) out[26 * (size_t)i + k] = w[k];
}

hipError_t launch_probe_material(const PtParams& p, uint32_t material, uint32_t n, const float* uv, uint32_t* out, hipStream_t stream) {
    size_t lds;
    const PtParams q = with_tex_slots(p, 0, lds);
    hipLaunchKernelGGL(k_probe_material, dim3((n + 127) / 128), dim3(128), lds, stream, q, material, n, uv, out);
    return hipGetLastError();
}
hipError_t launch_probe_math(uint32_t n, const float* x, float* s, float* c, float* l, hipStream_t stream) {
    hipLaunchKernelGGL(k_probe_math, dim3((n + 255) / 256), dim3(256), 0, stream, n, x, s, c, l);
    return hipGetLastError();
}
hipError_t launch_probe_math2(uint32_t n, const float* xy, float* out, hipStream_t stream) {
    hipLaunchKernelGGL(k_probe_math2, dim3((n + 255) / 256), dim3(256), 0, stream, n, xy, out);
    return hipGetLastError();
}
hipError_t launch_probe_div(uint32_t n, const float* a, const float* b, float* out_fast, float* out_ieee, hipStream_t stream) {
    hipLaunchKernelGGL(k_probe_div, dim3((n + 255) / 256), dim3(256), 0, stream, n, a, b, out_fast, out_ieee);
    return hipGetLastError();
}
hipError_t launch_probe_pcg_end_pass(uint32_t n, const uint64_t* state, const uint64_t* inc, const uint32_t* dim, uint64_t* out_closed, uint64_t* out_loop, hipStream_t stream) {
    hipLaunchKernelGGL(k_probe_pcg_end_pass, dim3((n + 255) / 256), dim3(256), 0, stream, n, state, inc, dim, out_closed, out_loop);
    return hipGetLastError();
}
hipError_t launch_probe_intersect_pair(const PtParams& p, uint32_t n, const float* rays, const uint32_t* excl, uint32_t* out, float* out_tuv, hipStream_t stream) {
    launch_kernel(k_probe_intersect_pair, (n + 255) / 256, (p.sc.n_tris + 2u) * 48u, stream, p, n, rays, excl, out, out_tuv);
    return hipGetLastError();
}
hipError_t launch_probe_bsdf(const DMaterial* m, const float* table, int mode, const float* wo, uint32_t n, const float* in, float* out,
                             hipStream_t stream) {
    hipLaunchKernelGGL(k_probe_bsdf, dim3((n + 255) / 256), dim3(256), 0, stream, m, table, mode, mk3(wo[0], wo[1], wo[2]), n, in, out);
    return hipGetLastError();
}
hipError_t launch_probe_intersect(const PtParams& p, uint32_t n, const float* rays, uint32_t* out, float* bary, hipStream_t stream) {
    const bool bvh = p.sc.bvh_nodes != nullptr, inst = p.sc.in2.on != 0;
    dispatch_bools([&](auto B, auto I) {
        launch_kernel(k_probe_intersect<B() || I(), I()>, (n + 255) / 256, B() || I() ? p.sc.bvh_stack_depth * 256 * 4 : 0, stream, p, n, rays, out, bary);
    }, bvh, inst);
    return hipGetLastError();
}
hipError_t launch_probe_si(const PtParams& p, uint32_t n, const uint32_t* inst_prim, const float* bary, float* out, hipStream_t stream) {
    dispatch_bools([&](auto I) { launch_kernel(k_probe_si<I()>, (n + 255) / 256, 0, stream, p, n, inst_prim, bary, out); }, p.sc.in2.on != 0);
    return hipGetLastError();
}

__global__ void k_probe_env(const DEnv* __restrict__ env_p, uint32_t color, uint32_t mode, uint32_t n, const float* __restrict__ in, float* __restrict__ out) {
    const uint32_t i = blockIdx.x * blockDim.x + threadIdx.x;
    if (i >= n) return;
    const DEnv& env = *env_p;
    if (mode == 0) {
        vec3 wi;
        float pdf;
        const bool ok = env_sample(env, mk2(in[2 * (size_t)i], in[2 * (size_t)i + 1]), wi, pdf);
        float* o = out + 5 * (size_t)i;
        o[0] = wi.x; o[1] = wi.y; o[2] = wi.z; o[3] = pdf; o[4] = ok ? 1.0f : 0.0f;
    } else {
        const vec3 d = mk3(in[3 * (size_t)i], in[3 * (size_t)i + 1], in[3 * (size_t)i + 2]);
        const vec3 le = env_eval(env, color, d);
        float* o = out + 4 * (size_t)i;
        o[0] = env_pdf(env, d); o[1] = le.x; o[2] = le.y; o[3] = le.z;
    }
}
hipError_t launch_probe_env(const PtParams& p, uint32_t mode, uint32_t n, const float* in, float* out, hipStream_t stream) {
    if (!p.sc.env || mode > 1) return hipErrorInvalidValue;
    if (n == 0) return hipSuccess;
    hipLaunchKernelGGL(k_probe_env, dim3((n + 255) / 256), dim3(256), 0, stream, p.sc.env, p.color, mode, n, in, out);
    return hipGetLastError();
}

__global__ void k_probe_camera_rays(const PtParams p, uint32_t n, const uint32_t* __restrict__ pixels, const float* __restrict__ u, float* __restrict__ out) {
    const uint32_t i = blockIdx.x * blockDim.x + threadIdx.x;
    if (i >= n) return;
    const float* ui = u + 4 * (size_t)i;
    vec3 o, d;
    if (p.lens_radius > 0.0f) generate_ray_lens_from(p, pixels[2 * (size_t)i], pixels[2 * (size_t)i + 1], mk2(ui[0], ui[1]), mk2(ui[2], ui[3]), o, d);
    else generate_ray_from(p, pixels[2 * (size_t)i], pixels[2 * (size_t)i + 1], mk2(ui[0], ui[1]), o, d);
    float* r = out + 6 * (size_t)i;
    r[0] = o.x; r[1] = o.y; r[2] = o.z; r[3] = d.x; r[4] = d.y; r[5] = d.z;
}
hipError_t launch_probe_camera_rays(const PtParams& p, uint32_t n, const uint32_t* pixels2, const float* u4, float* out6, hipStream_t stream) {
    if (n == 0) return hipSuccess;
    hipLaunchKernelGGL(k_probe_camera_rays, dim3((n + 255) / 256), dim3(256), 0, stream, p, n, pixels2, u4, out6);
    return hipGetLastError();
}

__global__ void k_probe_light_sample(const AliasPacked* __restrict__ light_alias, const LightRec* __restrict__ lights, const DPunct* __restrict__ punct, uint32_t n_lights, uint32_t n,
                                     const float* __restrict__ rows9, float* __restrict__ out13, uint32_t* __restrict__ light) {
    const uint32_t i = blockIdx.x * blockDim.x + threadIdx.x;
    if (i >= n) return;
    punct_probe_row(light_alias, lights, punct, n_lights, rows9 + 9 * (size_t)i, out13 + 13 * (size_t)i, light + i);
}
hipError_t launch_probe_light_sample(const PtParams& p, uint32_t n, const float* rows9, float* out13, uint32_t* light, hipStream_t stream) {
    if (n == 0) return hipSuccess;
    hipLaunchKernelGGL(k_probe_light_sample, dim3((n + 255) / 256), dim3(256), 0, stream, p.sc.light_alias, p.sc.lights, p.sc.punct, p.sc.n_lights, n, rows9, out13, light);
    return hipGetLastError();
}

__global__ void k_probe_light_tree_sample(const AliasPacked* __restrict__ light_alias, const LightRec* __restrict__ lights, const DPunct* __restrict__ punct, uint32_t punct_tree,
                                          uint32_t n_lights, uint32_t n, const float* __restrict__ rows9, float* __restrict__ out13, uint32_t* __restrict__ light,
                                          uint32_t* __restrict__ record) {
    const uint32_t i = blockIdx.x * blockDim.x + threadIdx.x;
    if (i >= n) return;
    light_tree_probe_row(light_alias, lights, punct, punct_tree, n_lights, rows9 + 9 * (size_t)i, out13 + 13 * (size_t)i, light + i, record + i);
}
hipError_t launch_probe_light_tree_sample(const PtParams& p, uint32_t n, const float* rows9, float* out13, uint32_t* light, uint32_t* record, hipStream_t stream) {
    if (n == 0) return hipSuccess;
    hipLaunchKernelGGL(k_probe_light_tree_sample, dim3((n + 255) / 256), dim3(256), 0, stream, p.sc.light_alias, p.sc.lights, p.sc.punct, p.sc.punct_tree, p.sc.n_lights, n, rows9, out13,
                       light, record);
    return hipGetLastError();
}

}
```

Before: 3674.

## Skip shadow-ray triangle tests for boundary planes when whole wave is outside segment

At scene build time, mark triangle planes for which every scene vertex lies on one side (boundary planes such as the walls of a closed box). During the exhaustive pair walk, when such a plane's shadow-segment parameter is outside [0, stmax] for every lane in the wave (checked with a ballot), the shadow barycentric, alpha and occlusion work for that triangle is skipped. The shadow plane computation is also split so that hit-point components are only computed when needed. This adds a wave ballot per triangle and a per-scene mask, and relies on a tolerance-based convexity test being correct.

```diff
diff --git a/akari_render_amd/capi.py b/akari_render_amd/capi.py
--- a/akari_render_amd/capi.py
+++ b/akari_render_amd/capi.py
@@ -61,6 +61,7 @@
     "akr_host_light_sample", "akr_probe_light_sample", "akr_host_light_sample_soft", "akr_probe_light_sample_soft",
     "akr_host_light_tree_sample", "akr_probe_light_tree_sample", "akr_host_option_info",
     "akr_probe_pt_cost_order", "akr_probe_pt_cost_order_mode",
+    "akr_probe_intersect_pair_gate", "akr_host_shadow_gate_mask",
 ]
 
 
@@ -227,6 +228,8 @@
     proto("akr_probe_intersect", vp, vp, u32, fp, up, fp)
     proto("akr_probe_div", vp, u32, fp, fp, fp, fp)
     proto("akr_probe_intersect_pair", vp, vp, u32, fp, up, up, fp)
+    proto("akr_probe_intersect_pair_gate", vp, vp, i32, u32, fp, up, up, fp, C.POINTER(C.c_uint64))
+    proto("akr_host_shadow_gate_mask", vp, C.POINTER(C.c_uint64))
     proto("akr_probe_surface_interaction", vp, vp, u32, up, fp, fp)
     proto("akr_probe_material_inputs", vp, vp, u32, u32, fp, fp)
     proto("akr_probe_material_inputs_host", vp, u32, u32, u32, fp, fp)
@@ -354,6 +357,11 @@
         flags = (1 if bvh else 0) | (2 if pmj else 0) | (4 if stage else 0) | (8 if defer else 0) | (16 if inst else 0) | (32 if env else 0) | (64 if lens else 0)
         check(lib().akr_host_spec_compile(self.h, flags, min_waves, arch.encode(), C.byref(nbytes), log, 4096))
         return nbytes.value
+
+    def shadow_gate_mask(self) -> int:
+        m = C.c_uint64()
+        check(lib().akr_host_shadow_gate_mask(self.h, C.byref(m)))
+        return m.value
 
     def launch_plan(self, cfg: abi.PtConfig, defer_metal: int = -1, simple_kernels: int = 1, defer_on: int = 0, spec_waves: int = 0) -> dict:
         out = abi.PtLaunchPlan()
@@ -944,6 +952,18 @@
     return out, tuv
 
 
+def probe_intersect_pair_gate(ctx: Context, scene: Scene, rays: np.ndarray, excl: np.ndarray, gate: bool):
+    rays = np.ascontiguousarray(rays, dtype=np.float32).reshape(-1, 16)
+    excl = np.ascontiguousarray(excl, dtype=np.uint32).reshape(-1, 3)
+    assert rays.shape[0] == excl.shape[0]
+    out = np.zeros((rays.shape[0], 4), dtype=np.uint32)
+    tuv = np.zeros((rays.shape[0], 3), dtype=np.float32)
+    skipped = np.zeros(rays.shape[0], dtype=np.uint64)
+    check(lib().akr_probe_intersect_pair_gate(ctx.h, scene.h, 1 if gate else 0, rays.shape[0], _fp(rays), _up(excl), _up(out), _fp(tuv),
+                                              skipped.ctypes.data_as(C.POINTER(C.c_uint64))))
+    return out, tuv, skipped
+
+
 def probe_surface_interaction(ctx: Context, scene: Scene, inst_prim: np.ndarray, bary: np.ndarray) -> np.ndarray:
     ip = np.ascontiguousarray(inst_prim, dtype=np.uint32).reshape(-1, 2)
     b = np.ascontiguousarray(bary, dtype=np.float32).reshape(-1, 2)
diff --git a/akari_render_amd/csrc/device/disect.h b/akari_render_amd/csrc/device/disect.h
--- a/akari_render_amd/csrc/device/disect.h
+++ b/akari_render_amd/csrc/device/disect.h
@@ -144,21 +144,30 @@
     asm("v_max3_f32 %0, |%1|, |%2|, |%3|" : "=v"(r) : "v"(a), "v"(b), "v"(c));
     return r;
 }
-AKR_D PlaneHit tri_plane_unscaled(vec3 o, vec3 d, float4 r2, float& lo) {
+AKR_D float tri_plane_t_unscaled(vec3 o, vec3 d, float4 r2, float& lo) {
     float dz = __builtin_fmaf(r2.x, d.x, __builtin_fmaf(r2.y, d.y, r2.z * d.z));
     float oz = __builtin_fmaf(r2.x, o.x, __builtin_fmaf(r2.y, o.y, __builtin_fmaf(r2.z, o.z, r2.w)));
     lo = min_abs_raw(lo, oz);
+    return div_f_unscaled(-oz, dz);
+}
+AKR_HD float tri_plane_t(vec3 o, vec3 d, float4 r2) {
+    float dz = __builtin_fmaf(r2.x, d.x, __builtin_fmaf(r2.y, d.y, r2.z * d.z));
+    float oz = __builtin_fmaf(r2.x, o.x, __builtin_fmaf(r2.y, o.y, __builtin_fmaf(r2.z, o.z, r2.w)));
+    return div_f(-oz, dz);
+}
+AKR_D PlaneHit tri_plane_unscaled(vec3 o, vec3 d, float4 r2, float& lo) {
     PlaneHit h;
-    h.t = div_f_unscaled(-oz, dz);
+    h.t = tri_plane_t_unscaled(o, d, r2, lo);
     h.px = __builtin_fmaf(h.t, d.x, o.x);
     h.py = __builtin_fmaf(h.t, d.y, o.y);
     h.pz = __builtin_fmaf(h.t, d.z, o.z);
     return h;
 }
 
-template <bool DIV>
+template <bool DIV, bool GATE = false>
 struct WalkOpt {
     static constexpr bool unscaled_div = DIV;
+    static constexpr bool shadow_gate = GATE;
 };
 template <int V>
 struct IntTag {
@@ -167,8 +176,12 @@
 
 template <bool TEX = false, class OPT = WalkOpt<true>>
 AKR_D void trace_pair_exhaustive(const DScene& sc, vec3 o, vec3 d, float tmax, uint32_t ex0, vec3 so, vec3 sd, float stmax,
-                                 uint32_t sex0, uint32_t sex1, Hit& hit, bool& found, bool& occluded, const float4* lds_recs, uint32_t* took_ieee_walk = nullptr) {
+                                 uint32_t sex0, uint32_t sex1, Hit& hit, bool& found, bool& occluded, const float4* lds_recs, uint32_t* took_ieee_walk = nullptr,
+                                 uint64_t* gate_skipped = nullptr) {
     constexpr bool UNSCALED = OPT::unscaled_div && !AKR_RX;
+    constexpr bool GATE = OPT::shadow_gate;
+    uint64_t skipped = 0;
+    bool skip_shadow = false;
     float best_t = next_up(tmax);
     uint32_t best = kInvalid;
     float best_u = 0.0f, best_v = 0.0f;
@@ -177,55 +190,69 @@
     const v4f* lrec = (const v4f*)lds_recs;
     const bool has_alpha = __builtin_amdgcn_readfirstlane((int)sc.has_alpha) != 0;
     v2f T2 = {0.0f, 0.0f}, hx2 = {0.0f, 0.0f}, hy2 = {0.0f, 0.0f}, hz2 = {0.0f, 0.0f};
+    float sg = 0.0f;
     float lo = __builtin_inff(), slo = __builtin_inff();
-    auto record = [&](auto alpha_tag, auto div_tag, uint32_t k, const v4f& q0, const v4f& q1, const v4f& q2) {
+    auto record = [&](auto alpha_tag, auto div_tag, auto gate_tag, uint32_t k, const v4f& q0, const v4f& q1, const v4f& q2) {
         constexpr int ALPHA = decltype(alpha_tag)::value;
         constexpr bool FAST = decltype(div_tag)::value;
+        constexpr bool GATED = decltype(gate_tag)::value;
         if (!((sc.plane_share_mask >> k) & 1ull)) {
             const float4 r2 = make_float4(q2.x, q2.y, q2.z, q2.w);
-            const PlaneHit a = FAST ? tri_plane_unscaled(o, d, r2, lo) : tri_plane(o, d, r2), b = FAST ? tri_plane_unscaled(so, sd, r2, slo) : tri_plane(so, sd, r2);
-            T2 = (v2f){a.t, b.t};
-            hx2 = (v2f){a.px, b.px}; hy2 = (v2f){a.py, b.py}; hz2 = (v2f){a.pz, b.pz};
-        }
-        float u, v, su, sv;
+            const PlaneHit a = FAST ? tri_plane_unscaled(o, d, r2, lo) : tri_plane(o, d, r2);
+            const float st = FAST ? tri_plane_t_unscaled(so, sd, r2, slo) : tri_plane_t(so, sd, r2);
+            T2 = (v2f){a.t, st};
+            sg = min_raw(st, stmax - st);
+            hx2.x = a.px; hy2.x = a.py; hz2.x = a.pz;
+            if (GATED) {
+                skip_shadow = ((sc.shadow_gate_mask >> k) & 1ull) != 0 && __builtin_amdgcn_ballot_w64(sg >= 0.0f) == 0;
+                if (gate_skipped && skip_shadow) skipped |= 1ull << k;
+            }
+            if (!(GATED && skip_shadow)) {
+                hx2.y = __builtin_fmaf(st, sd.x, so.x); hy2.y = __builtin_fmaf(st, sd.y, so.y); hz2.y = __builtin_fmaf(st, sd.z, so.z);
+            }
+        }
+        float u, v;
         tri_uv(PlaneHit{T2.x, hx2.x, hy2.x, hz2.x}, make_float4(q0.x, q0.y, q0.z, q0.w), make_float4(q1.x, q1.y, q1.z, q1.w), u, v);
-        tri_uv(PlaneHit{T2.y, hx2.y, hy2.y, hz2.y}, make_float4(q0.x, q0.y, q0.z, q0.w), make_float4(q1.x, q1.y, q1.z, q1.w), su, sv);
-        const v2f u2 = {u, su}, v2 = {v, sv};
-        const v2f s2 = {1.0f - (u2.x + v2.x), 1.0f - (u2.y + v2.y)};
-        const v2f w2 = {tmax - T2.x, stmax - T2.y};
-        float m = min_raw(min_raw(min_raw(u2.x, v2.x), s2.x), min_raw(T2.x, w2.x));
-        float sm = min_raw(min_raw(min_raw(u2.y, v2.y), s2.y), min_raw(T2.y, w2.y));
+        float m = min_raw(min_raw(min_raw(u, v), 1.0f - (u + v)), min_raw(T2.x, tmax - T2.x));
         m = (k == ex0) ? -1.0f : m;
-        sm = (k == sex0) ? -1.0f : sm;
-        sm = (k == sex1) ? -1.0f : sm;
-        if (ALPHA == 1 || (ALPHA == 2 && has_alpha)) {
-            const uint32_t ka = __builtin_amdgcn_readfirstlane(k);
-            if (m >= 0.0f && !alpha_test<TEX>(sc, ka, u2.x, v2.x)) m = -1.0f;
-            if (sm >= 0.0f && !alpha_test<TEX>(sc, ka, u2.y, v2.y)) sm = -1.0f;
+        const bool alpha = ALPHA == 1 || (ALPHA == 2 && has_alpha);
+        if (alpha) {
+            if (m >= 0.0f && !alpha_test<TEX>(sc, __builtin_amdgcn_readfirstlane(k), u, v)) m = -1.0f;
         }
         const float tc = (m >= 0.0f) ? T2.x : __builtin_inff();
         const bool better = tc < best_t;
         best_t = better ? tc : best_t;
         best = better ? k : best;
-        occ_margin = max_raw(occ_margin, sm);
+        if (!(GATED && skip_shadow)) {
+            float su, sv;
+            tri_uv(PlaneHit{T2.y, hx2.y, hy2.y, hz2.y}, make_float4(q0.x, q0.y, q0.z, q0.w), make_float4(q1.x, q1.y, q1.z, q1.w), su, sv);
+            float sm = min_raw(min_raw(min_raw(su, sv), 1.0f - (su + sv)), sg);
+            sm = (k == sex0) ? -1.0f : sm;
+            sm = (k == sex1) ? -1.0f : sm;
+            if (alpha) {
+                if (sm >= 0.0f && !alpha_test<TEX>(sc, __builtin_amdgcn_readfirstlane(k), su, sv)) sm = -1.0f;
+            }
+            occ_margin = max_raw(occ_margin, sm);
+        }
     };
     auto walk = [&](auto alpha_tag) {
         const BoolTag<UNSCALED> div_tag{};
+        const BoolTag<GATE> gate_tag{};
         v4f a0 = lrec[0], a1 = lrec[1], a2 = lrec[2], b0, b1, b2;
         uint32_t k = 0;
         for (; k + 1 < n; k += 2) {
             b0 = lrec[3 * (k + 1)]; b1 = lrec[3 * (k + 1) + 1]; b2 = lrec[3 * (k + 1) + 2];
-            record(alpha_tag, div_tag, k, a0, a1, a2);
+            record(alpha_tag, div_tag, gate_tag, k, a0, a1, a2);
             a0 = lrec[3 * (k + 2)]; a1 = lrec[3 * (k + 2) + 1]; a2 = lrec[3 * (k + 2) + 2];
-            record(alpha_tag, div_tag, k + 1, b0, b1, b2);
-        }
-        if (k < n) record(alpha_tag, div_tag, k, a0, a1, a2);
+            record(alpha_tag, div_tag, gate_tag, k + 1, b0, b1, b2);
+        }
+        if (k < n) record(alpha_tag, div_tag, gate_tag, k, a0, a1, a2);
     };
     auto walk_ieee = [&] {
-        best_t = next_up(tmax); best = kInvalid; occ_margin = -1.0f;
+        best_t = next_up(tmax); best = kInvalid; occ_margin = -1.0f; skipped = 0;
 #pragma clang loop unroll(disable)
         for (uint32_t k = 0; k < n; k++) {
-            record(IntTag<2>{}, BoolTag<false>{}, k, lrec[3 * k], lrec[3 * k + 1], lrec[3 * k + 2]);
+            record(IntTag<2>{}, BoolTag<false>{}, BoolTag<false>{}, k, lrec[3 * k], lrec[3 * k + 1], lrec[3 * k + 2]);
         }
     };
     if (UNSCALED) {
@@ -258,6 +285,7 @@
     hit.v = best_v;
     hit.gid = best;
     occluded = occ_margin >= 0.0f;
+    if (gate_skipped) *gate_skipped = skipped;
 }
 
 constexpr uint32_t kBvhDone = 0xfffffffeu;
diff --git a/akari_render_amd/csrc/device/dscene.h b/akari_render_amd/csrc/device/dscene.h
--- a/akari_render_amd/csrc/device/dscene.h
+++ b/akari_render_amd/csrc/device/dscene.h
@@ -80,6 +80,7 @@
     DInst in2;
     const DPunct* __restrict__ punct;
     uint32_t n_punct, punct_tree;
+    uint64_t shadow_gate_mask;
 };
 
 struct SurfacePoint {
diff --git a/akari_render_amd/csrc/device/pt_pass.h b/akari_render_amd/csrc/device/pt_pass.h
--- a/akari_render_amd/csrc/device/pt_pass.h
+++ b/akari_render_amd/csrc/device/pt_pass.h
@@ -18,8 +18,11 @@
 #ifndef AKR_PT_MIN_WAVES_BVH_TEX
 #define AKR_PT_MIN_WAVES_BVH_TEX 3
 #endif
+#ifndef AKR_WALK_SHADOW_GATE
+#define AKR_WALK_SHADOW_GATE 1
+#endif
 template <bool TEX>
-using PairWalkOpt = WalkOpt<!TEX>;
+using PairWalkOpt = WalkOpt<!TEX, AKR_WALK_SHADOW_GATE == 2 || (AKR_WALK_SHADOW_GATE == 1 && !TEX)>;
 template <bool BVH, bool FD, bool TEX, bool PMJ, bool STAGE, bool DEFER, uint32_t ABSENT = 0, bool INST = false, bool ENV = false, bool LENS = false, bool FEAT = false, bool PUNCT = false, bool LTREE = false>
 AKR_D void pt_pass_body(const PtParams& p) {
     extern __shared__ __attribute__((aligned(16))) uint32_t lds_stack[];
diff --git a/akari_render_amd/csrc/host/api_probe.cpp b/akari_render_amd/csrc/host/api_probe.cpp
--- a/akari_render_amd/csrc/host/api_probe.cpp
+++ b/akari_render_amd/csrc/host/api_probe.cpp
@@ -207,6 +207,34 @@
             HIP_CHECK(hipMemcpy(tuv3, dt.p, 3ull * n * 4, hipMemcpyDeviceToHost));
         }
     });
+}
+AKR_TEST_API int32_t akr_probe_intersect_pair_gate(akr_context* ctx, akr_scene* scene, int32_t gate, uint32_t n, const float* rays16, const uint32_t* excl3, uint32_t* out4, float* tuv3,
+                                                   uint64_t* skipped) {
+    if (!ctx || !scene || !rays16 || !excl3 || !out4 || !tuv3 || !skipped) return fail(AKR_ERR_INVALID_ARGUMENT, "akr_probe_intersect_pair_gate: NULL argument");
+    if (scene->ctx != ctx) return fail(AKR_ERR_INVALID_ARGUMENT, "akr_probe_intersect_pair_gate: scene belongs to another context");
+    if (scene->dscene.bvh_nodes || scene->dscene.in2.on || scene->dscene.n_tris > 64)
+        return fail(AKR_ERR_INVALID_ARGUMENT, "akr_probe_intersect_pair_gate: the pair walk serves scenes of at most 64 triangles");
+    return guarded([&] {
+        ctx->bind();
+        DevBuf dr, de, dout, dt, ds;
+        dr.upload(std::vector<float>(rays16, rays16 + 16ull * n));
+        de.upload(std::vector<uint32_t>(excl3, excl3 + 3ull * n));
+        dout.alloc(4ull * n * 4);
+        dt.alloc(3ull * n * 4);
+        ds.alloc(8ull * n);
+        if (n) HIP_CHECK(launch_probe_intersect_pair_gate(probe_params(scene), gate != 0, n, dr.as<float>(), de.as<uint32_t>(), dout.as<uint32_t>(), dt.as<float>(), ds.as<uint64_t>(), ctx->stream));
+        HIP_CHECK(hipStreamSynchronize(ctx->stream));
+        if (n) {
+            HIP_CHECK(hipMemcpy(out4, dout.p, 4ull * n * 4, hipMemcpyDeviceToHost));
+            HIP_CHECK(hipMemcpy(tuv3, dt.p, 3ull * n * 4, hipMemcpyDeviceToHost));
+            HIP_CHECK(hipMemcpy(skipped, ds.p, 8ull * n, hipMemcpyDeviceToHost));
+        }
+    });
+}
+AKR_TEST_API int32_t akr_host_shadow_gate_mask(const akr_scene* scene, uint64_t* mask) {
+    if (!scene || !mask) return fail(AKR_ERR_INVALID_ARGUMENT, "akr_host_shadow_gate_mask: NULL argument");
+    *mask = scene->cs.shadow_gate_mask;
+    return AKR_OK;
 }
 static int32_t probe_env(akr_context* ctx, akr_scene* scene, uint32_t mode, uint32_t n, const float* in, float* out, const char* name) {
     if (!ctx || !scene || !in || !out) return fail(AKR_ERR_INVALID_ARGUMENT, std::string(name) + ": NULL argument");
diff --git a/akari_render_amd/csrc/host/api_scene.cpp b/akari_render_amd/csrc/host/api_scene.cpp
--- a/akari_render_amd/csrc/host/api_scene.cpp
+++ b/akari_render_amd/csrc/host/api_scene.cpp
@@ -239,6 +239,7 @@
     if (cs.bvh_nodes.empty() && !cs.instanced.on)
         for (uint32_t k = 1; k < d.n_tris && k < 64; k++)
             if (std::memcmp(&cs.woop[12ull * k + 8], &cs.woop[12ull * (k - 1) + 8], 16) == 0) d.plane_share_mask |= 1ull << k;
+    d.shadow_gate_mask = cs.shadow_gate_mask;
     if (cs.has_textures) {
         d.tex.nodes = s->tex_nodes.as<DNode>();
         d.tex.images = s->tex_images.as<DImage>();
diff --git a/akari_render_amd/csrc/host/scene_build.cpp b/akari_render_amd/csrc/host/scene_build.cpp
--- a/akari_render_amd/csrc/host/scene_build.cpp
+++ b/akari_render_amd/csrc/host/scene_build.cpp
@@ -551,6 +551,7 @@
     if (any_normals) out.normals.assign(24ull * n_tris, 0.0f);
     std::vector<float> bounds(6ull * n_tris);
     std::vector<float> tri_power(n_tris, 0.0f);
+    std::vector<float> world_v(n_tris <= 64u ? 9ull * n_tris : 0ull);
     std::vector<float> tri_cond(3ull * n_tris, 0.0f);
     for (int a = 0; a < 3; a++) { out.scene_lo[a] = INFINITY; out.scene_hi[a] = -INFINITY; }
 
@@ -621,6 +622,10 @@
             }
             vec3 A = xf_point(x.c0, x.c1, x.c2, x.t, v0), B = xf_point(x.c0, x.c1, x.c2, x.t, v1), C = xf_point(x.c0, x.c1, x.c2, x.t, v2);
             woop_precompute(A, B, C, &out.woop[12ull * gid]);
+            if (!world_v.empty()) {
+                const float w9[9] = {A.x, A.y, A.z, B.x, B.y, B.z, C.x, C.y, C.z};
+                std::memcpy(&world_v[9ull * gid], w9, sizeof w9);
+            }
             if (prim & 1u) {
                 const vec3 vb[3] = {A, B, C};
                 share_plane_row(&out.woop[12ull * (gid - 1) + 8], &out.woop[12ull * gid + 8], vb);
@@ -728,8 +733,31 @@
         out.woop.swap(rec);
         out.tri_gid = order;
         phase.lap("records in traversal order");
+    } else {
+        out.shadow_gate_mask = shadow_gate_planes(out.woop, world_v, n_tris);
     }
     out.woop.resize(out.woop.size() + 32, 0.0f);
+}
+
+uint64_t shadow_gate_planes(const std::vector<float>& woop, const std::vector<float>& world_v, uint32_t n_tris) {
+    if (n_tris > 64u || world_v.size() != 9ull * n_tris) return 0;
+    uint64_t mask = 0;
+    for (uint32_t k = 0; k < n_tris; k++) {
+        const float* r = &woop[12ull * k + 8];
+        if (k > 0 && std::memcmp(r, &woop[12ull * (k - 1) + 8], 16) == 0) continue;
+        double lo = 0.0, hi = 0.0, scale = 0.0;
+        for (size_t c = 0; c < 3ull * n_tris; c++) {
+            const float* p = &world_v[3 * c];
+            const double tx = (double)r[0] * p[0], ty = (double)r[1] * p[1], tz = (double)r[2] * p[2];
+            const double e = tx + ty + tz + (double)r[3];
+            lo = std::min(lo, e);
+            hi = std::max(hi, e);
+            scale = std::max(scale, std::fabs(tx) + std::fabs(ty) + std::fabs(tz) + std::fabs((double)r[3]));
+        }
+        const double tol = 1e-5 * scale;
+        if (std::isfinite(lo) && std::isfinite(hi) && scale > 0.0 && (lo >= -tol || hi <= tol)) mask |= 1ull << k;
+    }
+    return mask;
 }
 
 size_t exhaustive_stage_bytes(const CompiledScene& out, size_t n_lights) {
diff --git a/akari_render_amd/csrc/host/scene_build.h b/akari_render_amd/csrc/host/scene_build.h
--- a/akari_render_amd/csrc/host/scene_build.h
+++ b/akari_render_amd/csrc/host/scene_build.h
@@ -126,6 +126,7 @@
     bool has_alpha = false;
     bool needs_ggx_table = false;
     float scene_lo[3], scene_hi[3];
+    uint64_t shadow_gate_mask = 0;
     bool has_tree() const { return !bvh_nodes.empty() || instanced.on; }
 };
 
@@ -177,6 +178,7 @@
 
 void compile_scene(const FlatScene& flat, const TuningOptions& opt, CompiledScene& out);
 size_t exhaustive_stage_bytes(const CompiledScene& out, size_t n_lights);
+uint64_t shadow_gate_planes(const std::vector<float>& woop, const std::vector<float>& world_v, uint32_t n_tris);
 std::string punctual_light_name(const CompiledScene& cs);
 constexpr uint32_t kEnvConstW = 32, kEnvConstH = 16;
 void compile_environment(const FlatScene& flat, CompiledScene& out);
diff --git a/akari_render_amd/csrc/kernels.h b/akari_render_amd/csrc/kernels.h
--- a/akari_render_amd/csrc/kernels.h
+++ b/akari_render_amd/csrc/kernels.h
@@ -308,6 +308,7 @@
 hipError_t launch_probe_div(uint32_t n, const float* a, const float* b, float* out_fast, float* out_ieee, hipStream_t stream);
 hipError_t launch_probe_pcg_end_pass(uint32_t n, const uint64_t* state, const uint64_t* inc, const uint32_t* dim, uint64_t* out_closed, uint64_t* out_loop, hipStream_t stream);
 hipError_t launch_probe_intersect_pair(const PtParams& p, uint32_t n, const float* rays, const uint32_t* excl, uint32_t* out, float* out_tuv, hipStream_t stream);
+hipError_t launch_probe_intersect_pair_gate(const PtParams& p, bool gate, uint32_t n, const float* rays, const uint32_t* excl, uint32_t* out, float* out_tuv, uint64_t* skipped, hipStream_t stream);
 hipError_t launch_probe_intersect(const PtParams& p, uint32_t n, const float* rays, uint32_t* out, float* bary, hipStream_t stream);
 hipError_t launch_probe_si(const PtParams& p, uint32_t n, const uint32_t* inst_prim, const float* bary, float* out, hipStream_t stream);
 #endif
diff --git a/akari_render_amd/csrc/probe_kernels.hip b/akari_render_amd/csrc/probe_kernels.hip
--- a/akari_render_amd/csrc/probe_kernels.hip
+++ b/akari_render_amd/csrc/probe_kernels.hip
@@ -85,8 +85,9 @@
     bary[2 * i + 0] = found ? h.u : 0.0f;
     bary[2 * i + 1] = found ? h.v : 0.0f;
 }
+template <class OPT>
 __global__ __launch_bounds__(256) void k_probe_intersect_pair(PtParams p, uint32_t n, const float* __restrict__ rays, const uint32_t* __restrict__ excl, uint32_t* __restrict__ out,
-                                                              float* __restrict__ out_tuv) {
+                                                              float* __restrict__ out_tuv, uint64_t* __restrict__ skipped) {
     extern __shared__ __attribute__((aligned(16))) uint32_t lds_stack[];
     const uint32_t* g = (const uint32_t*)p.sc.woop;
     for (uint32_t i = threadIdx.x; i < (p.sc.n_tris + 2u) * 12u; i += 256u) lds_stack[i] = g[i];
@@ -98,9 +99,11 @@
     Hit h;
     bool found = false, occluded = false;
     uint32_t redo = 0;
-    trace_pair_exhaustive<false>(p.sc, mk3(r[0], r[1], r[2]), mk3(r[3], r[4], r[5]), act ? r[6] : -1.0f, e[0], mk3(r[8], r[9], r[10]), mk3(r[11], r[12], r[13]),
-                                 act ? r[14] : -1.0f, e[1], e[2], h, found, occluded, (const float4*)lds_stack, &redo);
+    uint64_t skip = 0;
+    trace_pair_exhaustive<false, OPT>(p.sc, mk3(r[0], r[1], r[2]), mk3(r[3], r[4], r[5]), act ? r[6] : -1.0f, e[0], mk3(r[8], r[9], r[10]), mk3(r[11], r[12], r[13]),
+                                      act ? r[14] : -1.0f, e[1], e[2], h, found, occluded, (const float4*)lds_stack, &redo, &skip);
     if (!act) return;
+    if (skipped) skipped[i] = skip;
     out[4 * i + 0] = found ? 1u : 0u;
     out[4 * i + 1] = h.gid;
     out[4 * i + 2] = occluded ? 1u : 0u;
@@ -162,7 +165,11 @@
     return hipGetLastError();
 }
 hipError_t launch_probe_intersect_pair(const PtParams& p, uint32_t n, const float* rays, const uint32_t* excl, uint32_t* out, float* out_tuv, hipStream_t stream) {
-    launch_kernel(k_probe_intersect_pair, (n + 255) / 256, (p.sc.n_tris + 2u) * 48u, stream, p, n, rays, excl, out, out_tuv);
+    launch_kernel(k_probe_intersect_pair<WalkOpt<true>>, (n + 255) / 256, (p.sc.n_tris + 2u) * 48u, stream, p, n, rays, excl, out, out_tuv, (uint64_t*)nullptr);
+    return hipGetLastError();
+}
+hipError_t launch_probe_intersect_pair_gate(const PtParams& p, bool gate, uint32_t n, const float* rays, const uint32_t* excl, uint32_t* out, float* out_tuv, uint64_t* skipped, hipStream_t stream) {
+    dispatch_bools([&](auto G) { launch_kernel(k_probe_intersect_pair<WalkOpt<true, G()>>, (n + 255) / 256, (p.sc.n_tris + 2u) * 48u, stream, p, n, rays, excl, out, out_tuv, skipped); }, gate);
     return hipGetLastError();
 }
 hipError_t launch_probe_bsdf(const DMaterial* m, const float* table, int mode, const float* wo, uint32_t n, const float* in, float* out,
```

New measurement: 3690 (median of 6 runs). Within noise of the previous version (+0.5%).
